# MilchRatchet/Luminary

Hardware: AMD Instinct MI355X
Metric: Mrays/s at 1920x1080, 8 bounces (higher is better)
Workload: dtype f32

## Files before the change

### include/lum_core.h

```cpp
#ifndef LUM_CORE_H
#define LUM_CORE_H

#include <stdint.h>

#ifdef __cplusplus
extern "C" {
#endif

typedef struct LumContext LumContext;

typedef struct LumDeviceSceneView {
  uint32_t num_meshes;
  uint32_t num_instances;
  uint32_t num_materials;
  uint32_t num_lights;
  const uint32_t* mesh_tri_offset;
  const float* vertices;
  const uint32_t* tri_tex;
  const uint32_t* instance_mesh_ids;
  const float* instance_transforms;
  const uint16_t* materials;
  const uint8_t* light_tree_root;
  const uint8_t* light_tree_nodes;
  const uint32_t* light_tri_handles;
// ... 146 lines not shown
typedef struct LumDenoiseParams {
  uint32_t iterations;
  float sigma_luminance;
  float sigma_normal;
  float sigma_depth;
  uint32_t uniform_samples;
} LumDenoiseParams;
void lumc_denoise_default_params(LumDenoiseParams* params);
int lumc_render_guides(LumContext* ctx, uint32_t num_samples, void* stream);
int lumc_download_guides(LumContext* ctx, float* albedo, float* normal, float* depth);
int lumc_has_guides(const LumContext* ctx);
int lumc_denoise(LumContext* ctx, const LumDenoiseParams* params, float* d_image, void* stream);
int lumc_denoise_host(LumContext* ctx, const LumDenoiseParams* params, float* image);
int lumc_set_denoise_form(LumContext* ctx, int lds);
int lumc_download_result_image(LumContext* ctx, float* result);
const float* lumc_result_image(LumContext* ctx);

int lumc_trace_closest(LumContext* ctx, uint32_t num_rays, const float* d_origins, const float* d_dirs, const uint32_t* d_ignore, uint32_t* d_out, void* stream);
int lumc_pixel_query(LumContext* ctx, uint32_t x, uint32_t y, uint32_t sample_id, uint32_t out[6]);
int lumc_trace_closest_host(LumContext* ctx, uint32_t num_rays, const float* origins, const float* dirs, const uint32_t* ignore, uint32_t* out);

int lumc_trace_visibility(LumContext* ctx, uint32_t num_rays, const float* d_origins, const float* d_dirs, const float* d_dist, const uint32_t* d_ids, const uint32_t* d_order,
                          float* d_out, void* stream);
int lumc_trace_visibility_host(LumContext* ctx, uint32_t num_rays, const float* origins, const float* dirs, const float* dist, const uint32_t* ids, const uint32_t* order, float* out);
int lumc_light_query_host(LumContext* ctx, uint32_t num_rays, const float* origins, const float* dirs, const uint32_t* self, const float* randoms, uint32_t* out_ids,
                          uint32_t* out_num_hits);
#define LUMC_LIGHT_PROBE_VERTEX_WORDS 20
#define LUMC_LIGHT_PROBE_WORDS 154
enum { LUMC_LIGHT_PROBE_GENERAL = 0, LUMC_LIGHT_PROBE_PLAIN = 1, LUMC_LIGHT_PROBE_UNSTAGED = 2 };
enum { LUMC_LIGHT_PROBE_NO_PICK = 0, LUMC_LIGHT_PROBE_SELF = 1, LUMC_LIGHT_PROBE_REFUSED = 2, LUMC_LIGHT_PROBE_MISSED = 3, LUMC_LIGHT_PROBE_EVALUATED = 4 };
int lumc_light_sample_probe_host(LumContext* ctx, uint32_t num_vertices, const uint32_t* vertices, uint32_t first_sample, uint32_t samples, int form, uint32_t* out);

#define LUMC_LENS_MAX_INTERFACES 24
typedef struct LumLensInterface { float radius, vertex, cylindrical_radius; } LumLensInterface;
typedef struct LumLensMedium { float design_ior, abbe, cylindrical_radius; } LumLensMedium;
typedef struct LumPhysicalCamera {
  float aperture_point, aperture_radius, exit_pupil_point, exit_pupil_radius, image_plane_distance, sensor_width;
  uint32_t allow_reflections;
  uint32_t num_interfaces;
  LumLensInterface interfaces[LUMC_LENS_MAX_INTERFACES];
  LumLensMedium media[LUMC_LENS_MAX_INTERFACES + 1];
} LumPhysicalCamera;
int lumc_set_physical_camera(LumContext* ctx, const LumPhysicalCamera* camera);
int lumc_camera_rays(LumContext* ctx, const uint32_t* pixels, uint32_t n, uint32_t first_sample, uint32_t samples, float* out_origin, float* out_dir, float* out_weight);

int lumc_set_bvh_builder(LumContext* ctx, int builder);

unsigned int lumc_lds_stack_bytes(void);

#define LUMC_COMM_ID_BYTES 128
int lumc_device_count(void);
uint32_t lumc_tile_lattice_step(uint32_t world);
uint32_t lumc_tile_owner(uint32_t tile_x, uint32_t tile_y, uint32_t tiles_x, uint32_t world);
int lumc_tile_pixels(uint32_t width, uint32_t height, uint32_t rank, uint32_t world, uint32_t tile, uint32_t* out, uint32_t* count);
int lumc_comm_unique_id(uint8_t id[LUMC_COMM_ID_BYTES]);
int lumc_comm_init_rank(LumContext* ctx, int world, int rank, const uint8_t id[LUMC_COMM_ID_BYTES]);
int lumc_comm_init_all(LumContext** ctxs, int n);
void lumc_comm_destroy(LumContext* ctx);
int lumc_frame_assemble(LumContext* ctx, uint32_t frame_pixels, int root, void* stream, float** d_frame_out);
int lumc_frame_assemble_all(LumContext** ctxs, int n, uint32_t frame_pixels, int root, float** d_frame_root);
int lumc_frame_gather(LumContext* ctx, uint32_t width, uint32_t height, int root, void* stream, float** d_frame_out);
int lumc_frame_gather_all(LumContext** ctxs, int n, uint32_t width, uint32_t height, int root, float** d_frame_root);
int lumc_frame_download(LumContext* ctx, uint32_t frame_pixels, float* first_moment, float* second_moment);
uint32_t lumc_frame_plane_stride(const LumContext* ctx);
int lumc_use_assembled_frame(LumContext* ctx, int on);
int lumc_accumulators_from_frame(LumContext* dst, LumContext* src);
int lumc_comm_count(const LumContext* ctx);
int lumc_device_name(int ordinal, char* out, size_t size);

int lumc_set_ray_sorting(LumContext* ctx, int mode);
int lumc_get_ray_sorting(const LumContext* ctx);

enum { LUMC_FLAVOUR_EXACT = 0, LUMC_FLAVOUR_FAST = 1 };
int lumc_set_flavour(LumContext* ctx, int flavour);
int lumc_get_flavour(const LumContext* ctx);
int lumc_set_ambient_reuse(LumContext* ctx, int mode);
int lumc_get_ambient_reuse(const LumContext* ctx);
int lumc_set_single_level(LumContext* ctx, int mode);
int lumc_get_single_level(const LumContext* ctx);
int lumc_set_plain_form(LumContext* ctx, int mode);
int lumc_get_plain_form(const LumContext* ctx);
int lumc_set_overlap_light_query(LumContext* ctx, int mode);
int lumc_get_overlap_light_query(const LumContext* ctx);
int lumc_overlap_registers_fit(uint32_t ray_kernel_regs, uint32_t light_query_regs);
int lumc_set_fused_resolve(LumContext* ctx, int on);
int lumc_set_sobol_table(LumContext* ctx, int on);
double lumc_bvh_build_seconds(const LumContext* ctx);
int lumc_bvh_meshes_by_builder(const LumContext* ctx, uint32_t out[2]);
int lumc_bvh_stats(LumContext* ctx, uint64_t out[4]);
uint32_t lumc_scene_view_sizeof(void);
int lumc_host_bvh_probe(const float* boxes, uint32_t count, uint32_t max_leaf, uint64_t out[6], double inner_area[3]);
uint32_t lumc_leaf_max_triangles(void);
typedef struct LumMeshRefitStats {
  uint64_t refits, rebuilds;
  uint32_t last_refits, last_rebuilds;
  double max_cost_growth;
  double seconds;
  double seconds_upload, seconds_refit, seconds_rebuild, seconds_assemble;
  double seconds_hash, seconds_download, seconds_lights;
} LumMeshRefitStats;
int lumc_set_mesh_refit(LumContext* ctx, uint32_t mode, float max_cost_growth);
int lumc_mesh_refit_stats(const LumContext* ctx, LumMeshRefitStats* out);
int lumc_bvh_refit_probe(const float* built_boxes, const float* refit_boxes, uint32_t count, uint32_t refit_count, int builder, int on_gpu, uint64_t sizes[3],
                         void* built_nodes, void* refit_nodes, void* host_refit_nodes, uint32_t* prims, double cost[3], uint64_t* valid);
int lumc_scene_tree_probe(const LumDeviceSceneView* scene, uint64_t sizes[4], void* nodes, void* tris, void* leaves, void* rows, uint32_t* mesh_root, float bounds[6]);
typedef struct LumInstanceUpdateStats {
  uint64_t device_updates, fallbacks, relayouts;
  uint32_t tlas_nodes, tlas_depth, tlas_capacity, hittable;
  double seconds;
  double seconds_relayout, seconds_upload, seconds_boxes, seconds_build, seconds_leaves;
} LumInstanceUpdateStats;
int lumc_set_instance_update(LumContext* ctx, uint32_t mode);
int lumc_instance_update_stats(const LumContext* ctx, LumInstanceUpdateStats* out);
int lumc_instance_boxes_probe(const LumDeviceSceneView* scene, const float* mesh_boxes, int on_gpu, void* rows, float* boxes, uint32_t* hittable);
int lumc_resident_tree_probe(LumContext* ctx, uint64_t sizes[5], void* top_nodes, void* leaves, uint32_t* mesh_root, uint64_t* mesh_hash);
int lumc_set_mesh_refit_in_place(LumContext* ctx, uint32_t on);
typedef struct LumResidentRefitStats {
  uint64_t updates, fallbacks;
  uint32_t last_meshes, last_launches;
  uint64_t last_bytes_downloaded;
  double seconds;
  double seconds_upload, seconds_hash, seconds_refit, seconds_cost, seconds_top_level;
} LumResidentRefitStats;
int lumc_resident_refit_stats(const LumContext* ctx, LumResidentRefitStats* out);
int lumc_resident_mesh_nodes_probe(LumContext* ctx, void* nodes);
typedef struct LumMeshSkinStats {
  uint64_t poses, rebuild_downloads;
  uint32_t last_meshes, last_launches;
  uint64_t last_bytes_uploaded;
  double seconds, seconds_upload, seconds_skin;
} LumMeshSkinStats;
int lumc_mesh_skin_bind(LumContext* ctx, uint32_t mesh, const float* rest_positions, const float* rest_normals, const uint16_t* bone_ids, const float* weights,
                        uint32_t triangle_count, uint32_t bone_count);
int lumc_mesh_skin_unbind(LumContext* ctx, uint32_t mesh);
int lumc_mesh_skin_pose(LumContext* ctx, uint32_t mesh, const float* bones, uint32_t bone_count);
int lumc_mesh_skin_stats(const LumContext* ctx, LumMeshSkinStats* out);
int lumc_mesh_vertices_probe(LumContext* ctx, uint32_t mesh, void* out);
int lumc_skin_host(const float* rest_positions, const float* rest_normals, const uint16_t* bone_ids, const float* weights, uint32_t triangle_count, const float* bones,
                   uint32_t bone_count, float* positions, float* normals, uint32_t* packed);
typedef struct LumMeshMorphStats {
  uint64_t applied, rebuild_downloads;
  uint32_t last_meshes, last_launches;
  uint64_t last_bytes_uploaded;
  double seconds, seconds_upload, seconds_morph;
} LumMeshMorphStats;
int lumc_mesh_morph_bind(LumContext* ctx, uint32_t mesh, const float* base_positions, const float* base_normals, uint32_t triangle_count, uint32_t target_count,
                         const uint32_t* offsets, const uint32_t* corners, const float* delta_positions, const float* delta_normals);
int lumc_mesh_morph_unbind(LumContext* ctx, uint32_t mesh);
int lumc_mesh_morph_weights(LumContext* ctx, uint32_t mesh, const float* weights, uint32_t target_count);
int lumc_mesh_morph_stats(const LumContext* ctx, LumMeshMorphStats* out);
int lumc_morph_host(const float* base_positions, const float* base_normals, uint32_t triangle_count, uint32_t target_count, const uint32_t* offsets, const uint32_t* corners,
                    const float* delta_positions, const float* delta_normals, const float* weights, const uint16_t* bone_ids, const float* skin_weights, const float* bones,
                    uint32_t bone_count, float* positions, float* normals, uint32_t* packed);
typedef struct LumShutterStats {
  uint64_t slices;
  uint32_t last_meshes, last_launches;
  uint64_t last_bytes_uploaded;
  double seconds;
} LumShutterStats;
int lumc_mesh_shutter_key(LumContext* ctx, uint32_t mesh, uint32_t which);
int lumc_mesh_shutter_drop(LumContext* ctx, uint32_t mesh);
int lumc_shutter_time(LumContext* ctx, float t);
int lumc_shutter_stats(const LumContext* ctx, LumShutterStats* out);
int lumc_shutter_host(const void* open_records, const void* close_records, uint32_t count, float t, void* out_records, uint32_t* flags);
int lumc_host_bvh_nodes_probe(const float* boxes, uint32_t count, uint32_t max_leaf, uint32_t max_depth, uint64_t sizes[3], void* nodes, uint32_t* prims);
typedef struct LumLightFragment { uint32_t instance, mesh, triangle, light_id, transform; float intensity, average_intensity; uint32_t reserved; } LumLightFragment;
// ... 39 lines not shown
```

### luminary_amd/core.py

```python
import ctypes as C

import numpy as np

from . import DeviceSceneView, _lib

DIRTY_CONSTANTS, DIRTY_MATERIALS, DIRTY_INSTANCES, DIRTY_LIGHTS, DIRTY_MESHES, DIRTY_TEXTURES, DIRTY_PARTICLES, DIRTY_ALL = 1, 2, 4, 8, 16, 32, 64, 127
DIRTY_MESH_POSITIONS = 128
DIRTY_INSTANCE_TRANSFORMS = 256
DIRTY_MESH_SKIN = 512
DIRTY_LIGHT_POSITIONS = 1024
DIRTY_MESH_SHUTTER = 2048
BVH_BUILDERS = {"sah": 0, "lbvh": 1, "ploc": 2, "sah_gpu": 3}
CNT_TRACE, CNT_SHADOW, CNT_LIGHT_BVH, CNT_VERTICES, CNT_NODES, CNT_TRIS, CNT_NODES_SHADOW, CNT_TRIS_SHADOW, CNT_NODES_LIGHT, CNT_TRIS_LIGHT, CNT_NODES_LDS, CNT_NODES_LDS_SHADOW, CNT_AMBIENT_DEFERRED, CNT_AMBIENT_FALLBACK = range(14)
CNT_COUNT = 16
KERNELS = ("generate", "trace", "shade", "shadow", "accumulate", "light_query", "resolve", "output", "sky", "sort", "volume")


class CoreError(RuntimeError):
    pass


class OutputParams(C.Structure):
    _fields_ = [("src_width", C.c_uint32), ("src_height", C.c_uint32), ("dst_width", C.c_uint32), ("dst_height", C.c_uint32),
                ("inv_sample_count", C.c_float), ("exposure", C.c_float), ("tonemap", C.c_uint32), ("filter", C.c_uint32), ("dithering", C.c_uint32),
# ... 323 lines not shown
        lib = _lib()
        n = C.c_uint32()
        if lib.lumc_tile_pixels(C.c_uint32(width), C.c_uint32(height), C.c_uint32(rank), C.c_uint32(world), C.c_uint32(tile), C.c_void_p(0), C.byref(n)):
            raise CoreError("lumc_tile_pixels: bad arguments")
        out = np.zeros(max(n.value, 1), dtype=np.uint32)
        lib.lumc_tile_pixels(C.c_uint32(width), C.c_uint32(height), C.c_uint32(rank), C.c_uint32(world), C.c_uint32(tile), out.ctypes.data_as(C.c_void_p), C.byref(n))
        return out[:n.value]

    @staticmethod
    def comm_unique_id():
        buf = (C.c_uint8 * 128)()
        if _lib().lumc_comm_unique_id(buf):
            raise CoreError("lumc_comm_unique_id failed")
        return bytes(buf)

    def comm_init_rank(self, world, rank, unique_id):
        buf = (C.c_uint8 * 128).from_buffer_copy(unique_id)
        self._call("lumc_comm_init_rank", C.c_int(world), C.c_int(rank), buf)

    def frame_assemble(self, frame_pixels, root=0, stream=0):
        ptr = C.c_void_p()
        self._call("lumc_frame_assemble", C.c_uint32(frame_pixels), C.c_int(root), C.c_void_p(stream), C.byref(ptr))
        return ptr.value

    def frame_gather(self, width, height, root=0, stream=0):
        ptr = C.c_void_p()
        self._call("lumc_frame_gather", C.c_uint32(width), C.c_uint32(height), C.c_int(root), C.c_void_p(stream), C.byref(ptr))
        return ptr.value

    def frame_download(self, frame_pixels):
        fm = np.zeros(3 * frame_pixels, dtype=np.float32)
        sm = np.zeros(frame_pixels, dtype=np.float32)
        self._call("lumc_frame_download", C.c_uint32(frame_pixels), fm.ctypes.data_as(C.c_void_p), sm.ctypes.data_as(C.c_void_p))
        return fm.reshape(3, -1), sm

    @property
    def ray_sorting(self):
        fn = self._lib.lumc_get_ray_sorting
        fn.restype = C.c_int
        return int(fn(self._ctx))

    def set_ray_sorting(self, mode):
        self._call("lumc_set_ray_sorting", C.c_int(mode))

    def set_fused_resolve(self, on):
        self._call("lumc_set_fused_resolve", C.c_int(int(on)))

    def set_sobol_table(self, on):
        self._call("lumc_set_sobol_table", C.c_int(1 if on else 0))

    def set_ambient_reuse(self, mode):
        self._call("lumc_set_ambient_reuse", C.c_int(mode))

    @property
    def ambient_reuse(self):
        fn = self._lib.lumc_get_ambient_reuse
        fn.restype = C.c_int
        return bool(fn(self._ctx))

    def set_single_level(self, mode):
        self._call("lumc_set_single_level", C.c_int(mode))

    def get_single_level(self):
        fn = self._lib.lumc_get_single_level
        fn.restype = C.c_int
        return int(fn(self._ctx))

    def set_plain_form(self, mode):
        self._call("lumc_set_plain_form", C.c_int(mode))

    def get_plain_form(self):
        fn = self._lib.lumc_get_plain_form
        fn.restype = C.c_int
        return int(fn(self._ctx))

    def set_overlap_light_query(self, mode):
        self._call("lumc_set_overlap_light_query", C.c_int(mode))

    def get_overlap_light_query(self):
        fn = self._lib.lumc_get_overlap_light_query
        fn.restype = C.c_int
        return int(fn(self._ctx))

    @staticmethod
    def overlap_registers_fit(ray_kernel_regs, light_query_regs):
        fn = _lib().lumc_overlap_registers_fit
        fn.restype = C.c_int
        return bool(fn(C.c_uint32(ray_kernel_regs), C.c_uint32(light_query_regs)))

    def set_physical_camera(self, camera):
        self._call("lumc_set_physical_camera", C.byref(camera) if camera is not None else C.c_void_p(0))

    def camera_rays(self, pixels, first_sample, samples):
        px = np.ascontiguousarray(pixels, dtype=np.uint32)
        n = px.size * samples
        o = np.zeros((n, 3), dtype=np.float32)
        d = np.zeros((n, 3), dtype=np.float32)
        w = np.zeros(n, dtype=np.float32)
        self._call("lumc_camera_rays", px.ctypes.data_as(C.c_void_p), C.c_uint32(px.size), C.c_uint32(first_sample), C.c_uint32(samples),
                   o.ctypes.data_as(C.c_void_p), d.ctypes.data_as(C.c_void_p), w.ctypes.data_as(C.c_void_p))
        return o, d, w

    def pixel_query(self, x, y, sample_id=0):
        out = (C.c_uint32 * 6)()
        self._call("lumc_pixel_query", C.c_uint32(x), C.c_uint32(y), C.c_uint32(sample_id), out)
        a = np.array(list(out), dtype=np.uint32)
        return int(a[0]), int(a[1]), float(a[2:3].view(np.float32)[0]), a[3:6].view(np.float32).copy()

    def set_flavour(self, name):
        self._call("lumc_set_flavour", C.c_int({"exact": 0, "fast": 1}[name]))

    def _call(self, name, *args):
        fn = getattr(self._lib, name)
        fn.restype = C.c_int
        if fn(self._ctx, *args) != 0:
            raise CoreError("%s failed: %s" % (name, self._lib.lumc_last_error(self._ctx).decode()))

    def close(self):
        if self._ctx:
            self._lib.lumc_context_destroy(self._ctx)
            self._ctx = C.c_void_p()

    def __del__(self):
        try:
            self.close()
        except Exception:
            pass

    def upload(self, view):
        self._view_keepalive = view
        self._call("lumc_scene_upload", C.byref(view))
        self.width, self.height = view.width, view.height

    def update(self, view, dirty):
        self._view_keepalive = view
        self._call("lumc_scene_update", C.byref(view), C.c_uint(dirty))
        self.width, self.height = view.width, view.height

    def generate_output(self, params, first_moment=None, want_float=False):
        out = np.zeros((params.dst_height, params.dst_width), dtype=np.uint32)
        planes = np.zeros(params.output_planes_shape(), dtype=np.float32) if want_float else None
        pl = planes.ctypes.data_as(C.c_void_p) if want_float else C.c_void_p(0)
        if isinstance(first_moment, np.ndarray):
            fm = np.ascontiguousarray(first_moment, dtype=np.float32)
            self._call("lumc_generate_output_from_host", C.byref(params), fm.ctypes.data_as(C.c_void_p), out.ctypes.data_as(C.c_void_p), pl)
        else:
            ptr = C.c_void_p(0) if first_moment is None else C.c_void_p(int(first_moment))
            self._call("lumc_generate_output_host", C.byref(params), ptr, out.ctypes.data_as(C.c_void_p), pl)
        return (out, planes) if want_float else out

    def download_luts(self):
        out = {"conductor": np.zeros(1024, np.uint16), "glossy": np.zeros(1024, np.uint16), "dielectric": np.zeros(32768, np.uint16),
               "dielectric_inv": np.zeros(32768, np.uint16)}
        self._call("lumc_download_luts", *[out[k].ctypes.data_as(C.c_void_p) for k in ("conductor", "glossy", "dielectric", "dielectric_inv")])
        return out

    def download_sky_luts(self):
        tm = np.zeros(2 * 64 * 256 * 4, dtype=np.float32)
        ms = np.zeros(2 * 32 * 32 * 4, dtype=np.float32)
        self._call("lumc_download_sky_luts", tm.ctypes.data_as(C.c_void_p), ms.ctypes.data_as(C.c_void_p))
        return tm, ms

    def cloud_noise_generate(self, seed):
        shape, detail, weather = np.zeros(128 ** 3, np.uint32), np.zeros(32 ** 3, np.uint32), np.zeros(1024 ** 2, np.uint32)
        self._call("lumc_cloud_noise_generate", C.c_uint32(seed), shape.ctypes.data_as(C.c_void_p), detail.ctypes.data_as(C.c_void_p),
                   weather.ctypes.data_as(C.c_void_p))
# ... 378 lines not shown
```

### luminary_amd/csrc/device/dev_scene.h

```cpp
#pragma once

#include <hip/hip_vector_types.h>
#include <stdint.h>

namespace lum {

struct alignas(128) Bvh4Node {
  float lo_x[4], lo_y[4], lo_z[4];
  float hi_x[4], hi_y[4], hi_z[4];
  uint32_t child[4];
  uint32_t pad[4];
};
static_assert(sizeof(Bvh4Node) == 128, "BVH4 node must be one cache line");

constexpr uint32_t kNodeBytes = 128u, kNodeShift = 7u;

constexpr uint32_t kBvhEmpty      = 0xFFFFFFFFu;
constexpr uint32_t kBvhLeafBit    = 0x80000000u;
#ifndef LUM_LEAF_MAX
#define LUM_LEAF_MAX 2
#endif
constexpr uint32_t kBvhLeafMaxTri = LUM_LEAF_MAX;
static_assert(LUM_LEAF_MAX >= 1 && LUM_LEAF_MAX <= 8, "a leaf's triangle count travels in 3 bits");

// ... 77 lines not shown
  uint32_t ocean_caustics_active, ocean_caustics_ris_sample_count;
  float ocean_caustics_domain_scale;
  uint32_t ocean_multiscattering, ocean_triangle_light_contribution;
  uint32_t cloud_active, cloud_atmosphere_scattering, cloud_steps, cloud_shadow_steps, cloud_octaves;
  float cloud_offset_x, cloud_offset_z, cloud_density, cloud_noise_shape_scale, cloud_noise_detail_scale, cloud_noise_weather_scale;
  float cloud_phase[4];
  float cloud_layers[3][10];
  const uint32_t* cloud_noise_shape;
  const uint32_t* cloud_noise_detail;
  const uint32_t* cloud_noise_weather;
  uint32_t particles_active, particles_count;
  float particles_scale, particles_speed;
  float particles_albedo[3], particles_direction[3], particles_phase[4];
  const float4* particle_normals;
  const Bvh4Node* particle_bvh_nodes;
  const BvhTri* particle_tris;
  const float4* particle_leaves;
  uint32_t particle_tlas_num_nodes, particle_num_leaves;
  const uint2* sobol_table;
  uint32_t sobol_first, sobol_count, sobol_stride;
  uint32_t traits;
};

struct PathQueue {
  float4* origin_t;
  float4* dir_slot;
  uint4* aux;
  uint4* hit_id;
  uint32_t* hit_scene_tri;
  uint32_t* parent;
};
constexpr uint32_t kParentDeferred = 0x80000000u, kParentMask = 0x7FFFFFFFu;

struct NeeQueue {
  float4* geo_color_light;
  float4* bsdf_ray_prob;
  float4* bsdf_weight_sum;
  uint4* ambient;
  uint4* sun;
  uint32_t* amb_path;
  float4* sun_water;
  float4* amb_t1;
  float4* amb_t2;
};

struct ShadowQueue {
  float4* origin_dist;
  float4* dir_out;
  uint4* ids;
  float4* vis;
  uint32_t* light_items;
  uint32_t capacity;
};

struct FusedResolve {
  PathQueue prev;
  NeeQueue nee_prev;
  ShadowQueue fallback;
  uint32_t* ended;
  const uint32_t* ended_prev;
};

constexpr uint32_t kVolumeShadowKinds = 19, kVolumeKindSun = 15, kVolumeKindAmbient = 16, kVolumeKindSun2 = 17, kVolumeKindAmbient2 = 18;
constexpr uint32_t kShadowKindAmbient2 = 4, kShadowKindSun2 = 5, kSurfaceShadowKindsWater = 6;
struct CloudQueue {
  uint32_t* items;
  float4* result;
  float* hit_dist;
  uint32_t capacity;
};
struct VolumeQueue {
  float4* bridge;
  uint4* sky;
  float4* weight;
  float4* sun_water;
  float4* amb_t1;
  float4* amb_t2;
  uint32_t* items;
};

struct PassParams {
  const uint32_t* pixels;
  uint32_t num_pixels, batch, first_sample;
};

constexpr uint32_t kAdaptiveStages = 4;
struct AdaptiveView {
  const uint32_t* stage_counts;
  const uint32_t* block_task_end;
  uint32_t blocks_x, blocks_y, num_blocks;
  uint32_t executions[kAdaptiveStages + 1];
  uint32_t stage_id;
};
struct AdaptivePass { uint32_t task_begin, task_end, block_begin, block_end, executions; };
constexpr uint32_t kGuidePlanes = 7;
constexpr uint32_t kGuideSumPlanes = 9;
struct DenoiseArgs {
  uint32_t width, height, step, uniform_samples;
  float sigma_luminance, sigma_normal, sigma_depth;
};

constexpr uint32_t kLensMaxInterfaces = 24;
struct LensInterface { float radius, vertex, cylindrical_radius; };
struct LensMedium { float design_ior, abbe, cylindrical_radius; };
struct DeviceLens {
  float aperture_point, aperture_radius, exit_pupil_point, exit_pupil_radius, image_plane_distance, sensor_width;
  uint32_t num_interfaces, pad;
  LensInterface iface[kLensMaxInterfaces];
  LensMedium medium[kLensMaxInterfaces + 1];
};
enum CameraKind : int { kCamThinLens = 0, kCamPhysical = 1, kCamPhysicalReflections = 2 };

enum PathState : uint32_t {
  kStDeltaPath = 1, kStCameraDirection = 2, kStVolumeScattered = 4, kStAllowEmission = 8, kStAllowAmbient = 16, kStUseIgnoreHandle = 32
};
enum SkyMode : uint32_t { kSkyDefault = 0, kSkyHdri = 1, kSkyConstantColor = 2 };

#ifndef LUM_CTL_LINE
#define LUM_CTL_LINE 32u
#endif
enum CtrlWord : uint32_t {
  kCtlPaths = 0, kCtlShadowItems = LUM_CTL_LINE, kCtlLightItems = 2u * LUM_CTL_LINE, kCtlSkyItems = 2u * LUM_CTL_LINE + 1u, kCtlTraceCursor = 3u * LUM_CTL_LINE,
  kCtlShadowCursor = 3u * LUM_CTL_LINE + 8u, kCtlStride = 4u * LUM_CTL_LINE,
  kCtlVolumeShift = 16u, kCtlVolumeShadowItems = kCtlShadowItems + kCtlVolumeShift, kCtlVolumeShadowCursor = kCtlShadowCursor + kCtlVolumeShift,
  kCtlVolumeItems = 2u * LUM_CTL_LINE + 2u,
  kCtlParticleCursor = LUM_CTL_LINE + 8u,
  kCtlCloudItems = 2u * LUM_CTL_LINE + 3u, kCtlCloudCursor = LUM_CTL_LINE + 24u,
  kCtlShadeCursor = 3u * LUM_CTL_LINE + 16u
};
static_assert(LUM_CTL_LINE >= 32u, "the fog's control words sit in the second half of the 32-word lines");

#ifndef LUM_LDS_STACK_BYTES
#define LUM_LDS_STACK_BYTES 98304u
#endif
#ifndef LUM_RAY_BLOCK_MAX
#define LUM_RAY_BLOCK_MAX 1024u
#endif
constexpr uint32_t kRayBlockMax = LUM_RAY_BLOCK_MAX;

enum Counter : uint32_t { kCntTrace = 0, kCntShadow, kCntLightBvh, kCntVertices, kCntNodes, kCntTris, kCntNodesShadow, kCntTrisShadow, kCntNodesLight, kCntTrisLight, kCntNodesLds,
                         kCntNodesLdsShadow,
                         kCntAmbientDeferred,
                         kCntAmbientFallback,
                         kCntSpare0, kCntSpare1, kCntCount };

}
```

### luminary_amd/csrc/device/dev_trace.h

```cpp
#pragma once

#include "dev_light.h"

LUM_NS_BEGIN

#ifndef LUM_TRACE_BLOCK
#define LUM_TRACE_BLOCK 1024
#endif
constexpr int kTraceBlock = LUM_TRACE_BLOCK;

constexpr uint32_t kHitSky        = 0xFFFFFFFEu;
constexpr uint32_t kLeaveInstance = 0xFFFFFFFDu;
constexpr uint32_t kTraversalDone = 0xFFFFFFFCu;
constexpr uint32_t kNoInstance    = 0xFFFFFFFFu;
constexpr int kStackSize = 128;
#ifndef LUM_CHUNK_MAX
#define LUM_CHUNK_MAX 256u
#endif
#ifndef LUM_VOTE_TRIS
#define LUM_VOTE_TRIS 1u
#define LUM_VOTE_NODES 2u
#endif
#ifndef LUM_REFILL
#define LUM_REFILL 40
// ... 20 lines not shown
#endif

LUM_DEV float safe_inv(float d) { return (fabsf(d) < 1e-30f) ? copysignf(1e30f, d) : __builtin_amdgcn_rcpf(d); }

LUM_DEV float vmax3(float a, float b, float c) { float r; asm("v_max3_f32 %0, %1, %2, %3" : "=v"(r) : "v"(a), "v"(b), "v"(c)); return r; }
LUM_DEV float vmin3(float a, float b, float c) { float r; asm("v_min3_f32 %0, %1, %2, %3" : "=v"(r) : "v"(a), "v"(b), "v"(c)); return r; }
LUM_DEV float vmax0(float a) { float r; asm("v_max_f32 %0, 0, %1" : "=v"(r) : "v"(a)); return r; }
LUM_DEV float vmin2(float a, float b) { float r; asm("v_min_f32 %0, %1, %2" : "=v"(r) : "v"(a), "v"(b)); return r; }

struct TRay {
  V3 o, d, inv, noi;
  uint32_t nx, ny, nz, fx, fy, fz;
  LUM_DEV void set(V3 origin, V3 dir) {
    o = origin; d = dir;
    inv = v3(safe_inv(dir.x), safe_inv(dir.y), safe_inv(dir.z));
    noi = v3(-(origin.x * inv.x), -(origin.y * inv.y), -(origin.z * inv.z));
    nx = (inv.x < 0.0f) ? 48u : 0u;  fx = 48u - nx;
    ny = (inv.y < 0.0f) ? 64u : 16u; fy = 80u - ny;
    nz = (inv.z < 0.0f) ? 80u : 32u; fz = 112u - nz;
  }
};

LUM_DEV float4 node_f4(const Bvh4Node* nodes, uint32_t byte_offset) {
  return *reinterpret_cast<const float4*>(reinterpret_cast<const char*>(nodes) + byte_offset);
}
LUM_DEV uint4 node_u4(const Bvh4Node* nodes, uint32_t byte_offset) {
  return *reinterpret_cast<const uint4*>(reinterpret_cast<const char*>(nodes) + byte_offset);
}

template <int kFarFirst = 0>
LUM_DEV float child_entry(float nx, float ny, float nz, float fx, float fy, float fz, const TRay& r, float tmax) {
  const float ax = __builtin_fmaf(nx, r.inv.x, r.noi.x), ay = __builtin_fmaf(ny, r.inv.y, r.noi.y), az = __builtin_fmaf(nz, r.inv.z, r.noi.z);
  const float bx = __builtin_fmaf(fx, r.inv.x, r.noi.x), by = __builtin_fmaf(fy, r.inv.y, r.noi.y), bz = __builtin_fmaf(fz, r.inv.z, r.noi.z);
  const float tn = vmax3(ax, ay, vmax0(az));
  const float tf = vmin3(bx, by, vmin2(bz, tmax));
  const bool far_first = kFarFirst == 1 || (kFarFirst == 2 && tmax >= 3.0e38f) || (kFarFirst == 3 && tmax < 3.0e38f);
  return (tn <= __builtin_fmaf(tf, 1.000004f, 1e-30f)) ? (far_first ? -tn : tn) : __builtin_inff();
}

LUM_DEV void cswap(float& ka, uint32_t& ca, float& kb, uint32_t& cb) {
  const bool s = kb < ka;
  const float k0 = s ? kb : ka, k1 = s ? ka : kb;
  const uint32_t c0 = s ? cb : ca, c1 = s ? ca : cb;
  ka = k0; kb = k1; ca = c0; cb = c1;
}

LUM_DEV bool within(float tnear, float tmax) { return tnear <= __builtin_fmaf(tmax, 1.000004f, 1e-30f); }

struct NodeSource { const Bvh4Node* global; const char* lds; uint32_t lds_count; };

template <bool kCull> struct StackEntry;
template <> struct StackEntry<true> {
  using E = uint2;
  static LUM_DEV E make(uint32_t node, float tnear) { return make_uint2(node, fbits(tnear)); }
  static LUM_DEV uint32_t node(E e) { return e.x; }
  static LUM_DEV bool reachable(E e, float tmax) { return bitsf(e.y) <= __builtin_fmaf(tmax, 1.000004f, 1e-30f); }
};
template <> struct StackEntry<false> {
  using E = uint32_t;
  static LUM_DEV E make(uint32_t node, float) { return node; }
  static LUM_DEV uint32_t node(E e) { return e; }
  static LUM_DEV bool reachable(E, float) { return true; }
};

template <typename E> struct StackWord;
template <> struct StackWord<uint32_t> {
  typedef uint32_t W;
  static LUM_DEV W pack(uint32_t e) { return e; }
  static LUM_DEV uint32_t unpack(W w) { return w; }
};
template <> struct StackWord<uint2> {
  typedef unsigned long long W;
  static LUM_DEV W pack(uint2 e) { return (W) e.x | ((W) e.y << 32); }
  static LUM_DEV uint2 unpack(W w) { return make_uint2((uint32_t) w, (uint32_t) (w >> 32)); }
};
template <typename E> struct TraversalStack {
  typedef typename StackWord<E>::W W;
  typedef __attribute__((address_space(5))) W* ScratchPtr;
  typedef __attribute__((address_space(3))) W* LdsPtr;
  ScratchPtr scratch; LdsPtr lds; int lds_entries;
  LUM_DEV void store(int i, E e) { if (i < lds_entries) lds[(uint32_t) i * (uint32_t) kTraceBlock] = StackWord<E>::pack(e); else scratch[i] = StackWord<E>::pack(e); }
  LUM_DEV E load(int i) const { if (i < lds_entries) return StackWord<E>::unpack(lds[(uint32_t) i * (uint32_t) kTraceBlock]); return StackWord<E>::unpack(scratch[i]); }
};
template <bool kOrdered, bool kCull, int kFarFirst = 0, typename S>
LUM_DEV uint32_t visit_node(const NodeSource& src, uint32_t cur, const TRay& r, float tmax, S& stk, int& sp,
                            typename StackEntry<kCull>::E& top, RayStats& st) {
  static_assert(!(kFarFirst && kCull), "the negated keys are not distances: only for queries that do not cull by them");
  using SE = StackEntry<kCull>;
  const uint32_t b = cur << 7;
  float4 nx, ny, nz, fx, fy, fz;
  uint4 ch;
  if (cur < src.lds_count) {
    const char* p = src.lds + b;
    nx = *reinterpret_cast<const float4*>(p + r.nx); ny = *reinterpret_cast<const float4*>(p + r.ny); nz = *reinterpret_cast<const float4*>(p + r.nz);
    fx = *reinterpret_cast<const float4*>(p + r.fx); fy = *reinterpret_cast<const float4*>(p + r.fy); fz = *reinterpret_cast<const float4*>(p + r.fz);
    ch = *reinterpret_cast<const uint4*>(p + 96u);
    st.lds_nodes++;
  }
  else {
    const Bvh4Node* __restrict__ nodes = src.global;
    nx = node_f4(nodes, b + r.nx); ny = node_f4(nodes, b + r.ny); nz = node_f4(nodes, b + r.nz);
    fx = node_f4(nodes, b + r.fx); fy = node_f4(nodes, b + r.fy); fz = node_f4(nodes, b + r.fz);
    ch = node_u4(nodes, b + 96u);
  }
  float k0 = child_entry<kFarFirst>(nx.x, ny.x, nz.x, fx.x, fy.x, fz.x, r, tmax);
  float k1 = child_entry<kFarFirst>(nx.y, ny.y, nz.y, fx.y, fy.y, fz.y, r, tmax);
  float k2 = child_entry<kFarFirst>(nx.z, ny.z, nz.z, fx.z, fy.z, fz.z, r, tmax);
  float k3 = child_entry<kFarFirst>(nx.w, ny.w, nz.w, fx.w, fy.w, fz.w, r, tmax);
  uint32_t c0 = ch.x, c1 = ch.y, c2 = ch.z, c3 = ch.w;
  if (kOrdered) {
    cswap(k0, c0, k1, c1); cswap(k2, c2, k3, c3); cswap(k0, c0, k2, c2); cswap(k1, c1, k3, c3); cswap(k1, c1, k2, c2);
  }
  const float inf = __builtin_inff();
  if (k1 < inf) {
    if (k2 < inf) {
      if (k3 < inf) { stk.store(sp, top); sp++; top = SE::make(c3, k3); }
      stk.store(sp, top); sp++; top = SE::make(c2, k2);
    }
    stk.store(sp, top); sp++; top = SE::make(c1, k1);
  }
  return (k0 < inf) ? c0 : kBvhEmpty;
}

template <typename S>
LUM_DEV uint2 stack_pop(const S& stk, int& sp, uint2& top) {
  const uint2 e = top;
  if (sp > 0) { sp--; top = stk.load(sp); }
  else top = make_uint2(kTraversalDone, 0u);
  return e;
}
template <typename S, typename E>
LUM_DEV void stack_push(S& stk, int& sp, E& top, E e) { stk.store(sp, top); sp++; top = e; }

LUM_DEV float4 tri_f4(const BvhTri* tris, uint32_t index, uint32_t word) { return reinterpret_cast<const float4*>(tris + index)[word]; }

struct LeafTris {
  float4 a[kBvhLeafMaxTri], b[kBvhLeafMaxTri], c[kBvhLeafMaxTri];
  template <bool kAllSlots>
  LUM_DEV void load(const BvhTri* __restrict__ tris, uint32_t first, uint32_t count) {
#pragma unroll
    for (uint32_t j = 0; j < kBvhLeafMaxTri; j++) {
      if (kAllSlots) {
        const uint32_t t = first + min(j, count - 1u);
        a[j] = tri_f4(tris, t, 0); b[j] = tri_f4(tris, t, 1); c[j] = tri_f4(tris, t, 2);
      }
      else if (j < count) { a[j] = tri_f4(tris, first + j, 0); b[j] = tri_f4(tris, first + j, 1); c[j] = tri_f4(tris, first + j, 2); }
    }
  }
};

template <bool kSingleLevel> struct OneInstance {};
template <> struct OneInstance<true> { float4 r0, r1, r2; uint32_t inst, root; };
LUM_DEV uint32_t instance_of(const OneInstance<false>&, uint32_t entered) { return entered; }
LUM_DEV uint32_t instance_of(const OneInstance<true>& one, uint32_t) { return one.inst; }

template <class Q, bool kSingleLevel = false>
LUM_DEV void trace_items(const DeviceScene& sc, uint32_t n, uint32_t* __restrict__ cursor, Q& q, RayStats& st, uint32_t& rays, uint32_t lds_count) {
  if (n == 0u) return;
  using SE = StackEntry<Q::kCull>;
  using E = typename SE::E;
  E stack_in_scratch[kStackSize];
  int sp = 0;
  TRay r;
  V3 wo = v3(0.0f, 0.0f, 0.0f), wd = v3(0.0f, 0.0f, 1.0f);
  float tmax = 0.0f;
  uint32_t cur = kTraversalDone, inst = kNoInstance, idx = 0;
  r.set(wo, wd);
  bool more = true;
  const uint32_t lane = threadIdx.x & 63u;
  const unsigned long long below = (1ull << lane) - 1ull;
  extern __shared__ float4 lds_top[];
  {
    const float4* __restrict__ g = reinterpret_cast<const float4*>(sc.bvh_nodes);
    for (uint32_t i = threadIdx.x; i < lds_count * (kNodeBytes / 16u); i += blockDim.x) lds_top[i] = g[i];
    __syncthreads();
  }
  __shared__ float4 lds_leaves[kSingleLevel ? 1u : 4u * LUM_LDS_INSTANCES];
  const uint32_t staged_leaves = kSingleLevel ? 0u : min(sc.tlas_num_leaves, (uint32_t) LUM_LDS_INSTANCES);
  if constexpr (!kSingleLevel) {
    for (uint32_t i = threadIdx.x; i < 4u * staged_leaves; i += blockDim.x) lds_leaves[i] = sc.tlas_leaves[i];
    __syncthreads();
  }
  [[maybe_unused]] OneInstance<kSingleLevel> one;
  if constexpr (kSingleLevel) {
    const float4* __restrict__ leaf = sc.tlas_leaves;
    const float4 meta = leaf[3];
    one.r0 = leaf[0]; one.r1 = leaf[1]; one.r2 = leaf[2]; one.inst = fbits(meta.x); one.root = fbits(meta.y);
  }
  const NodeSource nodes{sc.bvh_nodes, reinterpret_cast<const char*>(lds_top), lds_count};
  typedef typename TraversalStack<E>::W StackW;
  static_assert(sizeof(StackW) == sizeof(E), "a stack entry is one machine word");
  TraversalStack<E> stk{(typename TraversalStack<E>::ScratchPtr) reinterpret_cast<StackW*>(stack_in_scratch),
                        (typename TraversalStack<E>::LdsPtr) (reinterpret_cast<StackW*>(reinterpret_cast<char*>(lds_top) + lds_count * kNodeBytes) + threadIdx.x),
                        (int) (LUM_LDS_STACK_BYTES / (kRayBlockMax * (uint32_t) sizeof(E)))};

  E top = SE::make(kTraversalDone, 0.0f);
#ifdef LUM_PHASE_STATS
  uint32_t phase_[8] = {0, 0, 0, 0, 0, 0, 0, 0};
  unsigned long long ptime_[12] = {0, 0, 0, 0, 0, 0, 0, 0, 0, 0, 0, 0};
  const unsigned long long t_kernel_ = __builtin_readcyclecounter();
#endif
  auto pop = [&]() {
    LUM_PHASE(6); LUM_PHASE_LANES(7);
    bool left_instance = false, again;
    E e;
    if constexpr (kSingleLevel) {
      do {
        e = top;
        const bool done = SE::node(e) == kTraversalDone;
        if (!done) { sp--; top = stk.load(sp); }
        again = !done && !SE::reachable(e, tmax);
      } while (again);
      cur = SE::node(e);
      (void) left_instance;
      return;
    }
    do {
      e = top;
      const bool done = SE::node(e) == kTraversalDone, leave = SE::node(e) == kLeaveInstance;
      if (!done) { sp--; top = stk.load(sp); }
      left_instance |= leave;
      again = !done && (leave || !SE::reachable(e, tmax));
    } while (again);
    cur = SE::node(e);
    if (left_instance) { inst = kNoInstance; r.set(wo, wd); }
  };

  const uint32_t waves = gridDim.x * (blockDim.x / 64u);
  uint32_t chunk = n / (waves * 2u);
  chunk = (min(max(chunk, 64u), LUM_CHUNK_MAX) + 63u) & ~63u;
  uint32_t chunk_next = 0, chunk_end = 0;

  while (true) {
    const unsigned long long idle = __ballot(cur == kTraversalDone);
#ifdef LUM_PHASE_STATS
    const unsigned long long t_refill_ = __builtin_readcyclecounter();
    const bool refilling_ = idle != 0ull && more;
#endif
    if (idle != 0ull && more) {
      if (chunk_next >= chunk_end) {
        uint32_t base = 0;
        if (lane == 0) base = atomicAdd(cursor, chunk);
        base = __builtin_amdgcn_readfirstlane(base);
        chunk_next = base;
        chunk_end = min(base + chunk, n);
        more = base < n;
      }
      if (more) {
        const uint32_t avail = chunk_end - chunk_next, want = (uint32_t) __popcll(idle);
        const uint32_t rank = (uint32_t) __popcll(idle & below);
        if (cur == kTraversalDone && rank < avail) {
          idx = chunk_next + rank;
          if (q.load(sc, idx, wo, wd, tmax)) {
            rays++;
            const uint32_t e = 0x7F800000u;
            const bool finite = (fbits(wo.x) & e) != e && (fbits(wo.y) & e) != e && (fbits(wo.z) & e) != e && (fbits(wd.x) & e) != e && (fbits(wd.y) & e) != e &&
                                (fbits(wd.z) & e) != e;
            if constexpr (kSingleLevel) {
              if (finite) {
                const float4 r0 = one.r0, r1 = one.r1, r2 = one.r2;
                const float px = wo.x - r0.w, py = wo.y - r1.w, pz = wo.z - r2.w;
                const V3 oo = v3(mat_row_apply(r0.x, r0.y, r0.z, px, py, pz), mat_row_apply(r1.x, r1.y, r1.z, px, py, pz), mat_row_apply(r2.x, r2.y, r2.z, px, py, pz));
                const V3 od = v3(mat_row_apply(r0.x, r0.y, r0.z, wd.x, wd.y, wd.z), mat_row_apply(r1.x, r1.y, r1.z, wd.x, wd.y, wd.z),
                                 mat_row_apply(r2.x, r2.y, r2.z, wd.x, wd.y, wd.z));
                r.set(oo, od); cur = one.root; sp = 0; top = SE::make(kTraversalDone, 0.0f);
              }
              else q.finish(sc, idx);
            }
            else {
              if (finite) { r.set(wo, wd); cur = 0; sp = 0; top = SE::make(kTraversalDone, 0.0f); inst = kNoInstance; }
              else q.finish(sc, idx);
            }
          }
        }
        chunk_next += min(want, avail);
      }
    }
#ifdef LUM_PHASE_STATS
    if (refilling_) { ptime_[8] += __builtin_readcyclecounter() - t_refill_; ptime_[9]++; }
#endif
    if (__ballot(cur != kTraversalDone) == 0ull) break;
    LUM_PHASE(5);

    while (true) {
      const bool live = cur != kTraversalDone;
      const bool at_leaf = live && (cur & kBvhLeafBit);
      const bool want_tris = at_leaf && (kSingleLevel || inst != kNoInstance), want_enter = !kSingleLevel && at_leaf && inst == kNoInstance;
      const uint32_t n_live = (uint32_t) __popcll(__ballot(live)), n_tris = (uint32_t) __popcll(__ballot(want_tris)),
                     n_enter = kSingleLevel ? 0u : (uint32_t) __popcll(__ballot(want_enter));
      if (n_live == 0u) break;
      const uint32_t n_nodes = n_live - n_tris - n_enter;
      const bool run_tris = n_tris * LUM_VOTE_TRIS >= max(n_nodes, n_enter) * LUM_VOTE_NODES;
      const bool run_enter = !kSingleLevel && !run_tris && n_enter >= n_nodes;
      const bool do_tris = run_tris && want_tris, do_enter = run_enter && want_enter, do_node = !run_tris && !run_enter && live && !at_leaf;
      LUM_TIME_BEGIN();
#ifdef LUM_PHASE_STATS
      const bool memory_node_ = __ballot(do_node && cur >= lds_count) != 0ull;
#endif
      {
        if (do_tris) {
          LUM_PHASE(3); LUM_PHASE_LANES(4);
          if (q.on_tris(sc, instance_of(one, inst), cur & 0x0FFFFFFFu, ((cur >> 28) & 0x7u) + 1u, r.o, r.d, tmax, st)) cur = kTraversalDone;
          else pop();
          if (cur == kTraversalDone) q.finish(sc, idx);
        }
      }
      if constexpr (!kSingleLevel) {
        if (do_enter) {
          LUM_PHASE(1); LUM_PHASE_LANES(2);
          const uint32_t leaf_index = cur & 0x0FFFFFFFu;
          float4 r0, r1, r2, meta;
          if (leaf_index < staged_leaves) { const float4* leaf = lds_leaves + 4u * leaf_index; r0 = leaf[0]; r1 = leaf[1]; r2 = leaf[2]; meta = leaf[3]; }
          else { const float4* __restrict__ leaf = sc.tlas_leaves + 4u * leaf_index; r0 = leaf[0]; r1 = leaf[1]; r2 = leaf[2]; meta = leaf[3]; }
          inst = fbits(meta.x);
          const float px = wo.x - r0.w, py = wo.y - r1.w, pz = wo.z - r2.w;
          const V3 oo = v3(mat_row_apply(r0.x, r0.y, r0.z, px, py, pz), mat_row_apply(r1.x, r1.y, r1.z, px, py, pz), mat_row_apply(r2.x, r2.y, r2.z, px, py, pz));
          const V3 od = v3(mat_row_apply(r0.x, r0.y, r0.z, wd.x, wd.y, wd.z), mat_row_apply(r1.x, r1.y, r1.z, wd.x, wd.y, wd.z),
                           mat_row_apply(r2.x, r2.y, r2.z, wd.x, wd.y, wd.z));
          r.set(oo, od);
          stack_push(stk, sp, top, SE::make(kLeaveInstance, 0.0f));
          cur = fbits(meta.y);
        }
      }
      {
        if (do_node) {
          LUM_PHASE(0);
          st.nodes++;
          cur = visit_node<Q::kOrdered, Q::kCull, Q::kFarFirst>(nodes, cur, r, tmax, stk, sp, top, st);
          if (cur == kBvhEmpty) {
            pop();
            if (cur == kTraversalDone) q.finish(sc, idx);
          }
        }
      }
#ifdef LUM_PHASE_STATS
      {
        asm volatile("s_waitcnt vmcnt(0) lgkmcnt(0)" ::: "memory");
        const int kind = run_tris ? 4 : (run_enter ? 6 : (memory_node_ ? 0 : 2));
        LUM_TIME_END(kind);
      }
#endif
      if (more && n_live < LUM_REFILL) break;
    }
  }
#ifdef LUM_PHASE_STATS
  ptime_[10] = __builtin_readcyclecounter() - t_kernel_; ptime_[11] = 1;
  for (int k = 0; k < 8; k++) if (phase_[k]) atomicAdd(&g_phase[k], (unsigned long long) phase_[k]);
  if ((threadIdx.x & 63u) == 0u) for (int k = 0; k < 12; k++) if (ptime_[k]) atomicAdd(&g_phase_time[k], ptime_[k]);
#endif
}

struct Hit { uint32_t instance_id, tri_id; float t; uint32_t scene_tri; };

struct ClosestState {
  static constexpr bool kOrdered = true;
  static constexpr int kFarFirst = 0;
  static constexpr bool kCull = true;
  static constexpr uint32_t kOpaqueBit = 0x80000000u;
  bool use_ignore, cutout;
  uint32_t ign_inst, ign_tri;
  Hit best;
  LUM_DEV void begin(bool ignore, uint32_t inst, uint32_t tri) { use_ignore = ignore; cutout = false; ign_inst = inst; ign_tri = tri; best = Hit{kHitSky, 0u, kFltMax, 0u}; }
  LUM_DEV bool on_tris(const DeviceScene& sc, uint32_t inst, uint32_t first, uint32_t count, V3 o, V3 d, float& tmax, RayStats& st) {
    LeafTris lt;
    lt.load<false>(sc.blas_tris, first, count);
#pragma unroll
    for (uint32_t j = 0; j < kBvhLeafMaxTri; j++) {
      if (j >= count) break;
      const float4 a = lt.a[j], b = lt.b[j], c = lt.c[j];
      const uint32_t id = fbits(a.w);
      st.tris++;
      if (use_ignore && inst == ign_inst && id == ign_tri) continue;
      F2 uv;
      const float t = intersect_triangle(v3(a.x, a.y, a.z), v3(b.x, b.y, b.z), v3(c.x, c.y, c.z), o, d, uv);
      if (t < best.t || (t == best.t && t != kFltMax && (inst < best.instance_id || (inst == best.instance_id && id < best.tri_id)))) {
        if (fbits(c.w) < sc.num_textures &&
            texture_load(sc, fbits(c.w), triangle_uv(sc.tri_tex[fbits(b.w)], uv), true, make_float4(0.0f, 0.0f, 0.0f, 1.0f)).w == 0.0f) {
          cutout = true;
          continue;
        }
        best.instance_id = inst; best.tri_id = id; best.t = t; best.scene_tri = fbits(b.w) | (fbits(c.w) == kBvhTriOpaque ? kOpaqueBit : 0u); tmax = t;
      }
    }
    return false;
  }
  LUM_DEV Hit result() const { return (best.t == kFltMax) ? Hit{kHitSky, 0u, kFltMax, 0u} : Hit{best.instance_id, best.tri_id, best.t, best.scene_tri & ~kOpaqueBit}; }
};

struct ShadowState {
  static constexpr bool kOrdered = true;
#ifndef LUM_SHADOW_ORDER
#define LUM_SHADOW_ORDER 1
#endif
  static constexpr int kFarFirst = LUM_SHADOW_ORDER;
  static constexpr bool kCull = false;
  uint32_t tgt_inst, tgt_tri, self_inst, self_tri;
  float dist;
#if LUM_FAST
  using Acc = float;
#else
  using Acc = double;
#endif
  Acc tr, tg, tb;
  bool blocked;
  LUM_DEV void begin(uint4 ids, float d) { tgt_inst = ids.x; tgt_tri = ids.y; self_inst = ids.z; self_tri = ids.w; dist = (d > kFltMax) ? kFltMax : d; tr = tg = tb = (Acc) 1.0; blocked = false; }
  LUM_DEV bool on_tris(const DeviceScene& sc, uint32_t inst, uint32_t first, uint32_t count, V3 o, V3 d, float&, RayStats& st) {
    LeafTris lt;
    lt.load<true>(sc.blas_tris, first, count);
#pragma unroll
    for (uint32_t j = 0; j < kBvhLeafMaxTri; j++) {
      if (j >= count) break;
      const float4 a = lt.a[j], b = lt.b[j], c = lt.c[j];
      const uint32_t id = fbits(a.w);
      st.tris++;
      if ((inst == tgt_inst && id == tgt_tri) || (inst == self_inst && id == self_tri)) continue;
      F2 uv;
      const float t = intersect_triangle(v3(a.x, a.y, a.z), v3(b.x, b.y, b.z), v3(c.x, c.y, c.z), o, d, uv);
      if (!(t > kEps && t < dist)) continue;
      if (fbits(c.w) == kBvhTriOpaque) { blocked = true; return true; }
      const uint4 tt = sc.tri_tex[fbits(b.w)];
      const Material m = load_material(sc, tt.w & 0xFFFFu);
      Col albedo = m.albedo;
      float alpha = m.alpha;
      if (m.albedo_tex != kTextureNone) {
        const float4 af = (m.albedo_tex < sc.num_textures) ? texture_load(sc, m.albedo_tex, triangle_uv(tt, uv), true, make_float4(0.0f, 0.0f, 0.0f, 0.0f))
// ... 105 lines not shown
```

### luminary_amd/csrc/device/kernels.h

```cpp
#pragma once

#include "kernel_shadow.h"
#include "dev_sky.h"
#include "dev_volume.h"
#include "dev_particle.h"
#include "dev_water.h"
#include "dev_cloud_march.h"
#include "dev_adaptive.h"
#include "dev_camera.h"
#include "dev_wave.h"

LUM_NS_BEGIN

#ifndef LUM_SHADE_WAVES
#define LUM_SHADE_WAVES 3
#endif
#ifndef LUM_CLOUD_WAVES
#define LUM_CLOUD_WAVES 4
#endif
#ifndef LUM_FEATURE_WAVES
#define LUM_FEATURE_WAVES 3
#endif
#ifndef LUM_VOLUME_WAVES
#define LUM_VOLUME_WAVES 4
#endif
#ifndef LUM_SHADE_WAVES_CONSTANT_SKY
#define LUM_SHADE_WAVES_CONSTANT_SKY 3
#endif

LUM_DEV uint32_t initial_medium(const DeviceScene& sc, V3 origin) {
  return medium_ior_modify(0u, (sc.ocean_active && origin.y < sc.ocean_height) ? sc.ocean_refractive_index : 1.0f, true);
}
LUM_DEV uint32_t initial_volumes(const DeviceScene& sc, V3 origin, uint32_t sample_id) {
  uint32_t w = sample_id;
  if (sc.fog_active) w = volume_stack_modify(w, kVolumeFog, true);
  if (sc.ocean_active && ocean_is_underwater(sc, origin)) w = volume_stack_modify(w, kVolumeOcean, true);
  return w;
}

template <int kCam>
LUM_DEV void generate_path(const DeviceScene& sc, const DeviceLens& lens, const PathQueue& q, uint32_t* count, bool active, uint32_t x, uint32_t y,
                           uint32_t sample_id, uint32_t slot) {
  const uint32_t lane = threadIdx.x & 63u;
  const unsigned long long below = (1ull << lane) - 1ull;
  V3 o, d;
  float w = 1.0f;
  if (kCam != kCamThinLens && active) {
    const Sampler smp{sc.bluenoise_2d, x, y, sample_id, 0};
    w = camera_sample<kCam>(sc, lens, smp, o, d);
  }
  const bool valid = active && w > 0.0f;
  const unsigned long long ballot = __ballot(valid);
  if (ballot) {
    uint32_t base = 0;
    if (lane == (uint32_t) __builtin_ctzll(ballot)) base = atomicAdd(count, (uint32_t) __popcll(ballot));
    base = __shfl(base, __builtin_ctzll(ballot));
    if (valid) {
      const uint32_t i = base + (uint32_t) __popcll(ballot & below);
      if (kCam == kCamThinLens) {
        const Sampler smp{sc.bluenoise_2d, x, y, sample_id, 0};
        camera_ray(sc, smp, o, d);
      }
      const U2 rec = record_pack(splat(w));
      q.origin_t[i] = make_float4(o.x, o.y, o.z, kFltMax);
      q.dir_slot[i] = make_float4(d.x, d.y, d.z, bitsf(slot));
      q.aux[i]      = make_uint4(rec.x, rec.y, initial_medium(sc, o), kStDeltaPath | kStCameraDirection | kStAllowEmission | kStAllowAmbient);
      q.hit_id[i]   = make_uint4(0u, 0u, x | (y << 16), initial_volumes(sc, o, sample_id));
    }
  }
}

template <int kCam>
__global__ __launch_bounds__(kBlock) void k_generate(DeviceScene sc, PassParams pp, PathQueue q, float4* results, uint32_t* count, DeviceLens lens_arg) {
  const uint32_t total = pp.num_pixels * pp.batch;
  if constexpr (kCam == kCamThinLens) {
    for (uint32_t i = blockIdx.x * kBlock + threadIdx.x; i < total; i += gridDim.x * kBlock) {
      const uint32_t b = i / pp.num_pixels, p = i - b * pp.num_pixels;
      const uint32_t index = pp.pixels ? pp.pixels[p] : p;
      const uint32_t y = index / sc.width, x = index - y * sc.width;
      const Sampler smp{sc.bluenoise_2d, x, y, pp.first_sample + b, 0};
      V3 o, d;
      camera_ray(sc, smp, o, d);
      const U2 rec = record_pack(splat(1.0f));
      q.origin_t[i] = make_float4(o.x, o.y, o.z, kFltMax);
      q.dir_slot[i] = make_float4(d.x, d.y, d.z, bitsf(i));
      q.aux[i]      = make_uint4(rec.x, rec.y, initial_medium(sc, o), kStDeltaPath | kStCameraDirection | kStAllowEmission | kStAllowAmbient);
      q.hit_id[i]   = make_uint4(0u, 0u, x | (y << 16), initial_volumes(sc, o, pp.first_sample + b));
      results[i]    = make_float4(0.0f, 0.0f, 0.0f, 0.0f);
    }
    if (blockIdx.x == 0 && threadIdx.x == 0) *count = total;
  }
  else {
    __shared__ DeviceLens lds_lens;
    const DeviceLens& lens = stage_lens<kCam>(lens_arg, &lds_lens);
    const uint32_t rounds = (total + gridDim.x * kBlock - 1u) / (gridDim.x * kBlock);
    for (uint32_t round = 0; round < rounds; round++) {
      const uint32_t i = (round * gridDim.x + blockIdx.x) * kBlock + threadIdx.x;
      const bool active = i < total;
      uint32_t x = 0, y = 0, b = 0;
      if (active) {
        b = i / pp.num_pixels;
        const uint32_t p = i - b * pp.num_pixels;
        const uint32_t index = pp.pixels ? pp.pixels[p] : p;
        y = index / sc.width; x = index - y * sc.width;
        results[i] = make_float4(0.0f, 0.0f, 0.0f, 0.0f);
      }
      generate_path<kCam>(sc, lens, q, count, active, x, y, pp.first_sample + b, i);
    }
  }
}


template <int kCam>
__global__ __launch_bounds__(256) void k_generate_adaptive(DeviceScene sc, AdaptiveView a, AdaptivePass pass, PathQueue q, float4* results, uint32_t* count,
                                                          DeviceLens lens_arg) {
  __shared__ DeviceLens lds_lens;
  const DeviceLens& lens = stage_lens<kCam>(lens_arg, &lds_lens);
  const uint32_t pass_tasks = pass.task_end - pass.task_begin;
  const uint32_t rounds = (pass_tasks + gridDim.x * 256u - 1u) / (gridDim.x * 256u);
  for (uint32_t round = 0; round < rounds; round++) {
    const uint32_t slot = (round * gridDim.x + blockIdx.x) * 256u + threadIdx.x;
    const uint32_t t = pass.task_begin + slot;
    bool valid = false;
    uint32_t x = 0, y = 0, sample_id = 0;
    if (slot < pass_tasks) {
      uint32_t lo = pass.block_begin, hi = pass.block_end - 1u;
      while (lo < hi) {
        const uint32_t mid = (lo + hi) >> 1;
        if (t < a.block_task_end[mid] * pass.executions) hi = mid; else lo = mid + 1u;
      }
      const uint32_t block = lo;
      const uint32_t base = block ? a.block_task_end[block - 1u] * pass.executions : 0u;
      const uint32_t packed = a.stage_counts[block];
      const uint32_t per_pixel = adaptive_stage_count(packed, a.stage_id) * pass.executions;
      const uint32_t local = t - base;
      const uint32_t local_pixel = local / per_pixel, local_sample = local - local_pixel * per_pixel;
      const uint32_t by = block / a.blocks_x, bx = block - by * a.blocks_x;
      x = (bx << kAdaptiveBlockLog) + (local_pixel & 3u);
      y = (by << kAdaptiveBlockLog) + (local_pixel >> kAdaptiveBlockLog);
      sample_id = adaptive_pixel_samples(a, packed) + local_sample;
      valid = x < sc.width && y < sc.height && sample_id < kMaxGlobalSamples;
      results[slot] = make_float4(0.0f, 0.0f, 0.0f, 0.0f);
    }
    generate_path<kCam>(sc, lens, q, count, valid, x, y, sample_id, slot);
  }
}

template <int kCam>
__global__ __launch_bounds__(kBlock) void k_camera_rays(DeviceScene sc, DeviceLens lens_arg, const uint32_t* pixels, uint32_t n, uint32_t first_sample, uint32_t samples,
                                                        float* out_origin, float* out_dir, float* out_weight) {
  __shared__ DeviceLens lds_lens;
  const DeviceLens& lens = stage_lens<kCam>(lens_arg, &lds_lens);
  const uint32_t total = n * samples;
  for (uint32_t i = blockIdx.x * kBlock + threadIdx.x; i < total; i += gridDim.x * kBlock) {
    const uint32_t b = i / n, index = pixels[i - b * n];
    const uint32_t y = index / sc.width, x = index - y * sc.width;
    const Sampler smp{sc.bluenoise_2d, x, y, first_sample + b, 0};
    V3 o, d;
    const float w = camera_sample<kCam>(sc, lens, smp, o, d);
    out_origin[3 * i] = o.x; out_origin[3 * i + 1] = o.y; out_origin[3 * i + 2] = o.z;
    out_dir[3 * i] = d.x; out_dir[3 * i + 1] = d.y; out_dir[3 * i + 2] = d.z;
    out_weight[i] = w;
  }
}

constexpr uint32_t kNoAmbientPath = 0xFFFFFFFFu;
constexpr bool kReuseProves = !LUM_FAST;
constexpr uint32_t kHitTriOpaque = 0x80000000u, kHitTriCutout = 0x40000000u, kHitTriBeyondEps = 0x20000000u, kHitTriHit = 0x10000000u, kHitTriMask = 0x0FFFFFFFu;

struct TraceQuery : ClosestState {
  PathQueue q;
  const uint32_t* order;
  uint32_t item;
  LUM_DEV bool load(const DeviceScene&, uint32_t j, V3& o, V3& d, float& tmax) {
    const uint32_t i = order ? order[j] : j;
    item = i;
    const float4 o4 = ld_stream(&q.origin_t[i]), d4 = ld_stream(&q.dir_slot[i]);
    const uint32_t state = q.aux[i].w;
    const uint2 ign = *reinterpret_cast<const uint2*>(&q.hit_id[i]);
    begin((state & kStUseIgnoreHandle) != 0, ign.x, ign.y);
    o = v3(o4.x, o4.y, o4.z); d = v3(d4.x, d4.y, d4.z); tmax = kFltMax;
    return true;
  }
  LUM_DEV void finish(const DeviceScene&, uint32_t) {
    const uint32_t i = item;
    const Hit h = result();
    reinterpret_cast<float*>(&q.origin_t[i])[3] = h.t;
    *reinterpret_cast<uint2*>(&q.hit_id[i]) = make_uint2(h.instance_id, h.tri_id);
    static_assert(kOpaqueBit == kHitTriOpaque, "the opaque bit is stored where ClosestState keeps it");
    q.hit_scene_tri[i] = ((best.t == kFltMax) ? 0u : (best.scene_tri | kHitTriHit | (best.t > kEps ? kHitTriBeyondEps : 0u))) | (cutout ? kHitTriCutout : 0u);
  }
};

__global__ LUM_TRACE_BOUNDS void k_trace(DeviceScene sc, PathQueue q, const uint32_t* order, uint32_t* ctrl, uint64_t* counters, uint32_t lds_nodes) {
  RayStats st{0, 0, 0};
  uint32_t rays = 0;
  TraceQuery tq;
  tq.q = q;
  tq.order = order;
  tq.item = 0;
  trace_items(sc, ctrl[kCtlPaths], ctrl + kCtlTraceCursor, tq, st, rays, lds_nodes);
  flush_stats(counters, st, rays, kCntTrace, kCntNodes, kCntTris, kCntNodesLds);
}
template <bool kSingleLevel>
__global__ LUM_TRACE_BOUNDS void k_trace(DeviceScene sc, PathQueue q, const uint32_t* order, uint32_t* ctrl, uint64_t* counters, uint32_t lds_nodes) {
  static_assert(kSingleLevel, "the two-level form is the plain kernel of this name");
  RayStats st{0, 0, 0};
  uint32_t rays = 0;
  TraceQuery tq;
  tq.q = q;
  tq.order = order;
  tq.item = 0;
  trace_items<TraceQuery, true>(sc, ctrl[kCtlPaths], ctrl + kCtlTraceCursor, tq, st, rays, lds_nodes);
  flush_stats(counters, st, rays, kCntTrace, kCntNodes, kCntTris, kCntNodesLds);
}

template <bool kPlain = false>
LUM_DEV GeoContext build_context(const DeviceScene& sc, V3 hit_origin, V3 ray_world, uint32_t state, uint32_t inst, uint32_t tri, uint32_t tbase, uint32_t medium) {
  const Transform tf = load_transform(sc, inst);
  const float4 a = sc.vertices[3 * tbase], b = sc.vertices[3 * tbase + 1], c = sc.vertices[3 * tbase + 2];
  const uint4 tt = sc.tri_tex[tbase];
  V3 position = xf_point_inv(tf, hit_origin);
  const V3 ray = xf_rot_inv(tf, ray_world);
  const V3 p0 = v3(a.x, a.y, a.z);
  const V3 e1 = v3(b.x, b.y, b.z) - p0, e2 = v3(c.x, c.y, c.z) - p0;
  V3 face = normalize(cross(e1, e2));
  const F2 co = barycentric_in_triangle(p0, e1, e2, position);
  position = p0 + (e1 * co.x + e2 * co.y);
  position = xf_point(tf, position);
  const Material mat = load_material(sc, tt.w & 0xFFFFu);
  const F2 tex_coords = triangle_uv(tt, co);
  const V3 n0 = normal_unpack(fbits(a.w)), n1 = normal_unpack(fbits(b.w)), n2 = normal_unpack(fbits(c.w));
  const bool inside = dot(face, ray) > 0.0f;
  if (inside) face = face * -1.0f;
  V3 normal = lerp_normals(n0, n1 - n0, n2 - n0, co, face);
  if (mat.normal_tex != kTextureNone) {
    const bool valid = mat.normal_tex < sc.num_textures;
    const float4 nf = texture_load(sc, mat.normal_tex, tex_coords, false, make_float4(0.0f, 0.0f, 1.0f, 0.0f));
    V3 mn = v3(nf.x, nf.y, nf.z);
    if ((mat.flags & kDMatNormalMapCompressed) && valid) mn = mn * 2.0f - v3(1.0f, 1.0f, 1.0f);
    mn = normalize(mn);
    normal = qapply(qinv(rotation_to_z(normal)), mn);
  }
  normal = adapt_normal(ray * -1.0f, normal, face);
  Col albedo = mat.albedo;
  float alpha = mat.alpha;
  if (mat.albedo_tex != kTextureNone) {
    const float4 af = texture_load(sc, mat.albedo_tex, tex_coords, true, make_float4(0.9f, 0.9f, 0.9f, 1.0f));
    albedo = col(af.x, af.y, af.z);
    alpha = af.w;
  }
  const bool emissive_side = !inside || (mat.flags & kDMatBidirectionalEmission);
  const bool emits = (mat.flags & kDMatEmission) && emissive_side && ((state & kStAllowEmission) != 0);
  Col emission = emits ? mat.emission : col(0.0f, 0.0f, 0.0f);
  if (emits && mat.luminance_tex != kTextureNone) {
    const float4 lf = texture_load(sc, mat.luminance_tex, tex_coords, true, make_float4(0.0f, 0.0f, 0.0f, 0.0f));
    emission = col(lf.x, lf.y, lf.z) * (alpha * mat.emission_scale);
  }
  float roughness = mat.roughness;
  if (mat.roughness_tex != kTextureNone) roughness = texture_load(sc, mat.roughness_tex, tex_coords, true, make_float4(0.5f, 0.0f, 0.0f, 0.0f)).x;
  if (mat.flags & kDMatRoughnessAsSmoothness) roughness = 1.0f - roughness;
  roughness = fmaxf(roughness, 2e-2f);
  if ((state & kStDeltaPath) == 0) roughness = fmaxf(roughness, mat.roughness_clamp);
  uint32_t flags = kPlain ? 0u : mat.flags & kDMatSubstrateMask;
  if (mat.metallic_tex == kTextureNone && (mat.flags & kDMatMetallic)) flags |= kMatMetallic;
  if (mat.flags & kDMatColoredTransparency) flags |= kMatColoredTransparency;
  if (inside) flags |= kMatRefractionInside;
  const float other_ior = medium_ior_peek(medium, inside);
  const float ior_in = inside ? mat.refraction_index : other_ior;
  const float ior_out = inside ? other_ior : mat.refraction_index;
  if (((flags & kMatSubstrateMask) == kMatTranslucent) && (fabsf(1.0f - ior_in / ior_out) < 1e-4f)) {
    if ((flags & kMatColoredTransparency) == 0) albedo = col(lerpf(1.0f, albedo.r, alpha), lerpf(1.0f, albedo.g, alpha), lerpf(1.0f, albedo.b, alpha));
    alpha = 0.0f;
    flags |= kMatColoredTransparency;
  }
  GeoContext g;
  g.instance_id = inst; g.tri_id = tri;
  g.normal = xf_rot(tf, normal);
  g.face_normal_packed = normal_pack(face);
  g.position = position;
  g.V = ray_world * -1.0f;
  g.state = state;
  g.params.flags = flags;
  g.params.set(albedo, alpha, roughness, emission, ior_in / ior_out);
  return g;
}

LUM_DEV void add_to_result(float4* results, uint32_t slot, Col v) {
  if (!any_positive(v)) return;
  float4 r = results[slot];
  r.x += v.r; r.y += v.g; r.z += v.b;
  results[slot] = r;
}

struct ResolveRecords { uint4 aux; uint32_t slot; float4 cl, lc; uint4 amb; };
LUM_DEV ResolveRecords load_resolve_records(const PathQueue& in, const NeeQueue& nee, uint32_t i) {
// ... 1040 lines not shown
}

__global__ __launch_bounds__(kBlock) void k_volume_bounce(DeviceScene sc, PathQueue in, PathQueue out, VolumeQueue vq, uint32_t* ctrl, uint32_t depth_const) {
  const uint32_t n = ctrl[kCtlVolumeItems];
  uint32_t* count_out = ctrl + kCtlStride + kCtlPaths;
  const uint32_t lane = threadIdx.x & 63;
  const unsigned long long below = (1ull << lane) - 1ull;
  const uint32_t rounds = (n + gridDim.x * kBlock - 1) / (gridDim.x * kBlock);
  constexpr uint32_t kReserveRounds = 8;
  uint32_t reserved_base = 0;
  for (uint32_t round = 0; round < rounds; round++) {
    const uint32_t k = (round * gridDim.x + blockIdx.x) * kBlock + threadIdx.x;
    const bool valid = k < n;
    if (round % kReserveRounds == 0) {
      uint32_t count = 0;
      const uint32_t first = (round * gridDim.x + blockIdx.x) * kBlock + (threadIdx.x & ~63u);
      for (uint32_t r = 0; r < kReserveRounds && round + r < rounds; r++) {
        const uint32_t lo = first + r * gridDim.x * kBlock;
        count += (lo < n) ? min(64u, n - lo) : 0u;
      }
      uint32_t base = 0;
      if (lane == 0 && count) base = atomicAdd(count_out, count);
      reserved_base = __builtin_amdgcn_readfirstlane(base);
    }
    float4 n_o, n_d; uint4 n_aux, n_hid;
    if (valid) {
      const uint32_t i = vq.items[k];
      const float4 o4 = in.origin_t[i], d4 = in.dir_slot[i];
      const uint4 aux = in.aux[i], hid = in.hit_id[i];
      const Sampler smp{sc.bluenoise_2d, hid.z & 0xFFFFu, hid.z >> 16, path_sample_id(hid.w), depth_const};
      const V3 ray = v3(d4.x, d4.y, d4.z);
      const V3 origin = v3(o4.x, o4.y, o4.z) + ray * o4.w;
      const VolContext ctx = volume_context(sc, volume_stack_peek(hid.w, false), origin, ray, aux.w, 0.0f);
      const V3 bounce = volume_bsdf_sample(sc, ctx, smp, kRndVolGiResampling, kRndVolGiDiffuse);
      uint32_t state = aux.w & ~(kStDeltaPath | kStCameraDirection | kStAllowEmission | kStUseIgnoreHandle);
      if (sc.sky_mode != kSkyDefault) state &= ~kStAllowAmbient; else state |= kStAllowAmbient;
      state |= kStVolumeScattered;
      n_o = make_float4(origin.x, origin.y, origin.z, kFltMax);
      n_d = make_float4(bounce.x, bounce.y, bounce.z, d4.w);
      n_aux = make_uint4(aux.x, aux.y, aux.z, state);
      n_hid = make_uint4(0u, 0u, hid.z, hid.w);
    }
    const unsigned long long b = __ballot(valid);
    if (valid) {
      const uint32_t j = reserved_base + (uint32_t) __popcll(b & below);
      out.origin_t[j] = n_o; out.dir_slot[j] = n_d; out.aux[j] = n_aux; out.hit_id[j] = n_hid;
    }
    reserved_base += (uint32_t) __popcll(b);
  }
}

struct RaysQuery : ClosestState {
  const float* origins; const float* dirs; const uint32_t* ignore; uint32_t* out;
  LUM_DEV bool load(const DeviceScene&, uint32_t i, V3& o, V3& d, float& tmax) {
    const bool ign = ignore != nullptr && ignore[2 * i] != 0xFFFFFFFFu;
    begin(ign, ign ? ignore[2 * i] : 0u, ign ? ignore[2 * i + 1] : 0u);
    o = v3(origins[3 * i], origins[3 * i + 1], origins[3 * i + 2]); d = v3(dirs[3 * i], dirs[3 * i + 1], dirs[3 * i + 2]); tmax = kFltMax;
    return true;
  }
  LUM_DEV void finish(const DeviceScene&, uint32_t i) {
    const Hit h = result();
    out[3 * i] = h.instance_id; out[3 * i + 1] = h.tri_id; out[3 * i + 2] = fbits(h.t);
  }
};

__global__ LUM_TRACE_BOUNDS void k_trace_rays(DeviceScene sc, uint32_t n, const float* origins, const float* dirs, const uint32_t* ignore,
                                                           uint32_t* out, uint32_t* cursor, uint64_t* counters, uint32_t lds_nodes) {
  RayStats st{0, 0, 0};
  uint32_t rays = 0;
  RaysQuery q;
  q.origins = origins; q.dirs = dirs; q.ignore = ignore; q.out = out;
  trace_items(sc, n, cursor, q, st, rays, lds_nodes);
  flush_stats(counters, st, rays, kCntTrace, kCntNodes, kCntTris, kCntNodesLds);
}
template <bool kSingleLevel>
__global__ LUM_TRACE_BOUNDS void k_trace_rays(DeviceScene sc, uint32_t n, const float* origins, const float* dirs, const uint32_t* ignore,
                                                           uint32_t* out, uint32_t* cursor, uint64_t* counters, uint32_t lds_nodes) {
  static_assert(kSingleLevel, "the two-level form is the plain kernel of this name");
  RayStats st{0, 0, 0};
  uint32_t rays = 0;
  RaysQuery q;
  q.origins = origins; q.dirs = dirs; q.ignore = ignore; q.out = out;
  trace_items<RaysQuery, true>(sc, n, cursor, q, st, rays, lds_nodes);
  flush_stats(counters, st, rays, kCntTrace, kCntNodes, kCntTris, kCntNodesLds);
}

__global__ __launch_bounds__(kBlock) void k_light_query_probe(DeviceScene sc, uint32_t n, const float* origins, const float* dirs, const uint32_t* self, const float* randoms,
                                                              uint32_t* out_ids, uint32_t* out_num_hits) {
  const uint32_t i = blockIdx.x * kBlock + threadIdx.x;
  if (i >= n) return;
  RayStats st{0, 0, 0};
  uint32_t num_hits = 0;
  const uint32_t id = light_query(sc, v3(origins[3 * i], origins[3 * i + 1], origins[3 * i + 2]), v3(dirs[3 * i], dirs[3 * i + 1], dirs[3 * i + 2]), self[2 * i], self[2 * i + 1],
                                  randoms[i], num_hits, st);
  out_ids[i] = id; out_num_hits[i] = num_hits;
}

constexpr uint32_t kLightProbeVertexWords = 20, kLightProbeLaneWords = 17, kLightProbeHeadWords = 18;
constexpr uint32_t kLightProbeWords = kLightProbeHeadWords + kLightTreeOutputs * kLightProbeLaneWords;
enum LightProbeStatus : uint32_t { kLightProbeNoPick = 0, kLightProbeSelf = 1, kLightProbeRefused = 2, kLightProbeMissed = 3, kLightProbeEvaluated = 4 };
template <bool kPlain>
__global__ __launch_bounds__(kBlock) void k_light_sample_probe(DeviceScene sc, uint32_t n, uint32_t samples, uint32_t first_sample, uint32_t stage, const uint32_t* vertices,
                                                               uint32_t* out) {
  StagedLights staged_lights{nullptr, nullptr, 0u};
#if LUM_LDS_LIGHTS
  {
    __shared__ LdsF4 lds_light_table[4u * LUM_LDS_LIGHTS];
    __shared__ unsigned long long lds_light_handles[LUM_LDS_LIGHTS];
    const uint32_t staged = (kPlain || stage) ? min(sc.num_lights, (uint32_t) LUM_LDS_LIGHTS) : 0u;
    for (uint32_t k = threadIdx.x; k < 4u * staged; k += kBlock) { const float4 v = sc.light_tri_table[k]; const LdsF4 t = {v.x, v.y, v.z, v.w}; lds_light_table[k] = t; }
    for (uint32_t k = threadIdx.x; k < staged; k += kBlock) { const uint2 h = sc.light_tri_handles[k]; lds_light_handles[k] = (unsigned long long) h.x | ((unsigned long long) h.y << 32); }
    __syncthreads();
    staged_lights.table = (const __attribute__((address_space(3))) LdsF4*) lds_light_table;
    staged_lights.handles = (const __attribute__((address_space(3))) unsigned long long*) lds_light_handles;
    staged_lights.count = staged;
  }
#endif
  const uint32_t i = blockIdx.x * kBlock + threadIdx.x;
  if (i >= n) return;
  const uint32_t* vw = vertices + (size_t) (i / samples) * kLightProbeVertexWords;
  uint32_t* o = out + (size_t) i * kLightProbeWords;
  GeoContext g;
  g.instance_id = vw[16]; g.tri_id = vw[17];
  g.position = v3(bitsf(vw[0]), bitsf(vw[1]), bitsf(vw[2]));
  g.normal = normalize(v3(bitsf(vw[3]), bitsf(vw[4]), bitsf(vw[5])));
  g.V = normalize(v3(bitsf(vw[6]), bitsf(vw[7]), bitsf(vw[8])));
  g.face_normal_packed = normal_pack(g.normal);
  g.state = 0;
  g.params.flags = vw[15];
  g.params.set(col(bitsf(vw[9]), bitsf(vw[10]), bitsf(vw[11])), bitsf(vw[12]), bitsf(vw[13]), splat(0.0f), bitsf(vw[14]));
  const SamplerT<false> smp{sc.bluenoise_2d, vw[18], vw[19], first_sample + i % samples, 0u};
  ShadeClock clock;
  clock.start();
  const LightSample ls = sample_light<kPlain>(sc, g, smp, clock, staged_lights);
  o[0] = ls.light_id; o[1] = fbits(ls.ray.x); o[2] = fbits(ls.ray.y); o[3] = fbits(ls.ray.z);
  o[4] = fbits(ls.color.r); o[5] = fbits(ls.color.g); o[6] = fbits(ls.color.b); o[7] = fbits(ls.dist); o[8] = fbits(ls.root_sum);
  const TreeWork work = tree_prepass(sc, g, smp);
  const Energy energy = energy_terms(sc, g.params, world_ndotv(g));
#pragma unroll
  for (uint32_t l = 0; l < kLightTreeOutputs; l++) o[9 + l] = work.cont[l];
  o[17] = fbits(work.root_sum);
#if LUM_FAST
  const V3 view_local = normalize(qapply(rotation_to_z(g.normal), g.V));
#endif
#pragma nounroll
  for (uint32_t lane = 0; lane < kLightTreeOutputs; lane++) {
    uint32_t* w = o + kLightProbeHeadWords + lane * kLightProbeLaneWords;
    const TreePick pick = tree_postpass<kPlain>(sc, g, smp, lane, work);
    w[0] = pick.light_id; w[1] = fbits(pick.weight); w[2] = kLightProbeNoPick;
    if (pick.light_id == kLightIdInvalid) continue;
#if LUM_LDS_LIGHTS
    uint2 handle;
    const TableLight entry = load_tri_light_table<kPlain>(sc, staged_lights, pick.light_id, handle);
#else
    const uint2 handle = sc.light_tri_handles[pick.light_id];
    const TableLight entry = load_tri_light_table(sc, pick.light_id);
#endif
    const TriLight& tl = entry.tri;
    w[2] = kLightProbeSelf;
    if (handle.x == g.instance_id && handle.y == g.tri_id) continue;
    V3 ray; float sa;
    const F2 pair = smp.next2(kRndLightGeoRay + lane);
    w[2] = kLightProbeRefused;
    if (!sample_tri_solid_angle(g.position, tl, pair, ray, sa)) continue;
    w[3] = fbits(ray.x); w[4] = fbits(ray.y); w[5] = fbits(ray.z); w[6] = fbits(sa);
    F2 uv;
// ... 33 lines not shown
```

### luminary_amd/csrc/device/kernels_shared.h

```cpp
#pragma once

#include "dev_camera.h"
#include "dev_wave.h"
#include "dev_output.h"
#include "dev_adaptive.h"

LUM_NS_BEGIN

__global__ __launch_bounds__(256) void k_final_image(OutputParams p, const float* __restrict__ input, float* __restrict__ frame_output) {
  const uint32_t ui = p.undersampling_stage, uo = max(ui, p.supersampling);
  const uint32_t output_scale = 1u << (uo - ui);
  const uint32_t out_w = p.src_width >> uo, out_h = p.src_height >> uo, in_w = p.src_width >> ui, in_h = p.src_height >> ui;
  const uint32_t n = out_w * out_h, n_in = in_w * in_h;
  const float norm = 1.0f / (output_scale * output_scale);
  for (uint32_t i = blockIdx.x * 256 + threadIdx.x; i < n; i += gridDim.x * 256) {
    const uint32_t y = i / out_w, x = i - y * out_w;
    const uint32_t source_x = x * output_scale, source_y = y * output_scale;
    Col color = splat(0.0f);
    for (uint32_t yi = 0; yi < output_scale; yi++) {
      for (uint32_t xi = 0; xi < output_scale; xi++) {
        const uint32_t px_x = min(source_x + xi, in_w - 1), px_y = min(source_y + yi, in_h - 1);
        const uint32_t index = px_x + px_y * in_w;
        Col px = col(input[index] * p.inv_sample_count, input[n_in + index] * p.inv_sample_count, input[2 * n_in + index] * p.inv_sample_count);
        color = color + display_transform(p, px, px_x, px_y);
// ... 175 lines not shown
    if (x >= width || y >= height) continue;
    const uint32_t p = x + y * width;
    const uint32_t packed = a.stage_counts[block];
    const uint32_t per_pixel = adaptive_stage_count(packed, a.stage_id) * pass.executions;
    const uint32_t first_id = adaptive_pixel_samples(a, packed);
    const uint32_t block_begin = block ? a.block_task_end[block - 1u] : 0u;
    if (a.block_task_end[block] == block_begin) continue;
    const uint32_t base = block_begin * pass.executions - pass.task_begin + local * per_pixel;
    float r = first_moment[p], g = first_moment[num_pixels + p], b = first_moment[2 * num_pixels + p];
    float s = second_moment[p];
    for (uint32_t k = 0; k < per_pixel; k++) {
      if (first_id + k >= kMaxGlobalSamples) break;
      const float4 v = results[base + k];
      r += v.x; g += v.y; b += v.z;
      s += luminance(col(v.x * v.x, v.y * v.y, v.z * v.z));
    }
    first_moment[p] = r; first_moment[num_pixels + p] = g; first_moment[2 * num_pixels + p] = b;
    second_moment[p] = s;
  }
}

__global__ __launch_bounds__(256) void k_generate_result(AdaptiveView a, ResultParams rp, OutputParams op, const float* __restrict__ fm, const float* __restrict__ sm,
                                                        float* __restrict__ frame_result) {
  const uint32_t n = rp.width * rp.height;
  for (uint32_t index = blockIdx.x * 256u + threadIdx.x; index < n; index += gridDim.x * 256u) {
    const uint32_t y = index / rp.width, x = index - y * rp.width;
    const uint32_t samples = result_pixel_samples(a, rp, x, y);
    const float normalization = 1.0f / (float) samples;
    Col result;
    switch (rp.mode) {
      default:
      case 0: {
        if (rp.local_error_minimization) {
          Col center_mean;
          const float center_variance = adaptive_pixel_variance(fm, sm, n, index, normalization, center_mean);
          const float center_error = center_variance * normalization;
          const uint32_t xi_start = max(x, 1u) - 1u, xi_end = min(x, rp.width - 1u) + 1u;
          const uint32_t yi_start = max(y, 1u) - 1u, yi_end = min(y, rp.height - 1u) + 1u;
          Col neighbour_mean = splat(0.0f);
          float neighbour_error = 0.0f;
          for (uint32_t yi = yi_start; yi <= yi_end; yi++) {
            for (uint32_t xi = xi_start; xi <= xi_end; xi++) {
              if (xi == x && yi == y) continue;
              Col m = splat(0.0f);
              float variance = 0.0f, norm = 0.0f;
              const uint32_t ns = (xi < rp.width && yi < rp.height) ? result_pixel_samples(a, rp, xi, yi) : result_pixel_samples(a, rp, min(xi, rp.width - 1u), min(yi, rp.height - 1u));
              norm = 1.0f / (float) ns;
              if (xi < rp.width && yi < rp.height) variance = adaptive_pixel_variance(fm, sm, n, xi + yi * rp.width, norm, m);
              neighbour_mean = neighbour_mean + m;
              neighbour_error += variance * norm;
            }
          }
          const float neighbour_norm = 1.0f / (float) ((xi_end - xi_start + 1u) * (yi_end - yi_start + 1u) - 1u);
          neighbour_mean = neighbour_mean * neighbour_norm;
          neighbour_error *= neighbour_norm;
          const float t = remap01(center_error, 0.0f, 8.0f * neighbour_error);
          result = col(lerpf(center_mean.r, neighbour_mean.r, t), lerpf(center_mean.g, neighbour_mean.g, t), lerpf(center_mean.b, neighbour_mean.b, t));
        }
        else result = col(fm[index] * normalization, fm[n + index] * normalization, fm[2 * n + index] * normalization);
      } break;
      case 1: {
        Col mean;
        result = splat(128.0f * adaptive_pixel_variance(fm, sm, n, index, normalization, mean));
      } break;
      case 2: {
        Col mean;
        const float variance = adaptive_pixel_variance(fm, sm, n, index, normalization, mean);
        const float compression = adaptive_tonemap_compression(op, mean, rp.exposure);
        const float mse = sqrtf(variance * normalization) * compression;
        const float value = 1024.0f * mse;
        result = col(saturate(2.0f * value), saturate(2.0f * (value - 0.5f)),
                     saturate((value > 0.5f) ? 4.0f * (0.25f - fabsf(value - 1.0f)) : 4.0f * (0.25f - fabsf(value - 0.25f))));
      } break;
      case 3: {
        uint32_t per_pixel = 1;
        if (a.stage_counts && a.stage_id > 0) per_pixel = adaptive_stage_count(a.stage_counts[adaptive_block_of(a, x, y)], a.stage_id);
        result = splat((float) per_pixel / (float) kAdaptiveMaxRate);
      } break;
    }
    frame_result[index] = result.r; frame_result[n + index] = result.g; frame_result[2 * n + index] = result.b;
  }
}

__global__ __launch_bounds__(kBlock) void k_accumulate(const float4* results, uint32_t num_pixels, uint32_t batch, float* first_moment, float* second_moment) {
  for (uint32_t p = blockIdx.x * kBlock + threadIdx.x; p < num_pixels; p += gridDim.x * kBlock) {
    float r = first_moment[p], g = first_moment[num_pixels + p], b = first_moment[2 * num_pixels + p];
    float s = second_moment ? second_moment[p] : 0.0f;
    for (uint32_t k = 0; k < batch; k++) {
      const float4 v = results[k * num_pixels + p];
      r += v.x; g += v.y; b += v.z;
      s += luminance(col(v.x * v.x, v.y * v.y, v.z * v.z));
    }
    first_moment[p] = r; first_moment[num_pixels + p] = g; first_moment[2 * num_pixels + p] = b;
    if (second_moment) second_moment[p] = s;
  }
}

__global__ __launch_bounds__(kBlock) void k_accumulate_scatter(const float4* results, const uint32_t* pixels, uint32_t count, uint32_t frame_pixels, float* first_moment,
                                                               float* second_moment) {
  for (uint32_t p = blockIdx.x * kBlock + threadIdx.x; p < count; p += gridDim.x * kBlock) {
    const uint32_t index = pixels[p];
    const float4 v = results[p];
    first_moment[index] += v.x; first_moment[frame_pixels + index] += v.y; first_moment[2 * frame_pixels + index] += v.z;
    if (second_moment) second_moment[index] += luminance(col(v.x * v.x, v.y * v.y, v.z * v.z));
  }
}

__global__ __launch_bounds__(256) void k_visibility_pack(uint32_t n, const float* origins, const float* dirs, const float* dist, const uint32_t* ids, ShadowQueue sq) {
  const uint32_t i = blockIdx.x * 256u + threadIdx.x;
  if (i >= n) return;
  sq.origin_dist[i] = make_float4(origins[3 * i], origins[3 * i + 1], origins[3 * i + 2], dist[i]);
  sq.dir_out[i] = make_float4(dirs[3 * i], dirs[3 * i + 1], dirs[3 * i + 2], bitsf(i));
  sq.ids[i] = make_uint4(ids[4 * i], ids[4 * i + 1], ids[4 * i + 2], ids[4 * i + 3]);
}
__global__ __launch_bounds__(256) void k_visibility_unpack(uint32_t n, const float4* vis, float* out) {
  const uint32_t i = blockIdx.x * 256u + threadIdx.x;
  if (i >= n) return;
  const float4 v = vis[i];
  out[3 * i] = v.x; out[3 * i + 1] = v.y; out[3 * i + 2] = v.z;
}

__global__ void k_pixel_ray(DeviceScene sc, DeviceLens lens, int cam, uint32_t x, uint32_t y, uint32_t sample_id, float* origin, float* dir, uint32_t* valid) {
  if (blockIdx.x != 0 || threadIdx.x != 0) return;
  const Sampler smp{sc.bluenoise_2d, x, y, sample_id, 0};
  V3 o, d;
  float w = 1.0f;
  if (cam == kCamThinLens) camera_ray(sc, smp, o, d);
  else if (cam == kCamPhysical) w = camera_sample<kCamPhysical>(sc, lens, smp, o, d);
  else w = camera_sample<kCamPhysicalReflections>(sc, lens, smp, o, d);
  origin[0] = o.x; origin[1] = o.y; origin[2] = o.z;
  dir[0] = d.x; dir[1] = d.y; dir[2] = d.z;
  valid[0] = w > 0.0f ? 1u : 0u;
}

LUM_NS_END
```

### luminary_amd/csrc/device/wavefront_table.h

```cpp
#pragma once

#include <hip/hip_runtime.h>

#include "dev_scene.h"

namespace lum {

inline bool single_level_scene(const DeviceScene& sc) { return sc.tlas_num_nodes == 1u && sc.tlas_num_leaves == 2u; }

inline bool plain_scene(const DeviceScene& sc) {
  return (sc.traits & kTraitsPlain) == kTraitsPlain && sc.num_lights <= (uint32_t) LUM_LDS_LIGHTS && !sc.ocean_active &&
         (sc.sky_mode == kSkyConstantColor || sc.sky_mode == kSkyHdri);
}

struct WavefrontKernels {
  const char* flavour;
  uint32_t trace_block;
  int (*set_ray_kernel_lds)(size_t bytes);
  int (*init_sampler_seeds)();
  void (*sobol_table)(hipStream_t s, uint2* table, uint32_t first_sample, uint32_t count, uint32_t stride, uint32_t dims);
  void (*generate)(uint32_t grid, hipStream_t s, const DeviceScene& sc, const PassParams& pp, const PathQueue& q, float4* results, uint32_t* count, const DeviceLens& lens,
                   int cam);
  void (*generate_adaptive)(uint32_t grid, hipStream_t s, const DeviceScene& sc, const AdaptiveView& a, const AdaptivePass& pass, const PathQueue& q, float4* results,
                            uint32_t* count, const DeviceLens& lens, int cam);
  void (*trace)(uint32_t grid, size_t lds, hipStream_t s, const DeviceScene& sc, const PathQueue& q, const uint32_t* order, uint32_t* ctrl, uint64_t* counters,
                uint32_t lds_nodes, bool single_level);
  void (*sky_inscattering)(uint32_t grid, hipStream_t s, const DeviceScene& sc, const PathQueue& in, float4* results, const uint32_t* ctrl, uint32_t depth_const);
  void (*shade)(uint32_t grid, hipStream_t s, const DeviceScene& sc, const PathQueue& in, const PathQueue& out, const NeeQueue& nee, const ShadowQueue& sq, float4* results,
                uint32_t* ctrl, uint32_t depth_const, uint64_t* counters, uint32_t ambient_reuse, const FusedResolve* fused_dev, uint32_t fused_flags,
                bool plain_form);
  void (*shade_debug)(uint32_t grid, hipStream_t s, const DeviceScene& sc, const PathQueue& in, float4* results, const uint32_t* ctrl);
  void (*sky)(uint32_t grid, hipStream_t s, const DeviceScene& sc, const PathQueue& in, const ShadowQueue& sq, float4* results, const uint32_t* ctrl, uint32_t depth_const);
  void (*light_query)(uint32_t grid, hipStream_t s, const DeviceScene& sc, const PathQueue& in, const NeeQueue& nee, const ShadowQueue& sq, uint32_t* ctrl, uint32_t depth_const,
                      uint64_t* counters);
  void (*shadow_rays)(uint32_t grid, size_t lds, hipStream_t s, const DeviceScene& sc, const ShadowQueue& sq, const uint32_t* order, uint32_t* ctrl, uint64_t* counters,
                      uint32_t lds_nodes, bool single_level);
  void (*resolve)(uint32_t grid, hipStream_t s, const DeviceScene& sc, const PathQueue& in, const NeeQueue& nee, const ShadowQueue& sq, float4* results, const uint32_t* ctrl);
  void (*resolve_reuse)(uint32_t grid, hipStream_t s, const DeviceScene& sc, const PathQueue& in, const PathQueue& next, const NeeQueue& nee, const ShadowQueue& sq, float4* results,
                        uint32_t* ctrl, uint64_t* counters);
  void (*resolve_listed)(uint32_t grid, hipStream_t s, const DeviceScene& sc, const PathQueue& in, const NeeQueue& nee, const ShadowQueue& sq, float4* results, const uint32_t* ctrl);
  void (*resolve_ended)(uint32_t grid, hipStream_t s, const DeviceScene& sc, const PathQueue& in, const NeeQueue& nee, const ShadowQueue& sq, float4* results, const uint32_t* ctrl,
                        const uint32_t* list);
  bool fused_resolve;
  void (*volume_inscatter)(uint32_t grid, hipStream_t s, const DeviceScene& sc, const PathQueue& in, const VolumeQueue& vq, const ShadowQueue& sq, uint32_t* ctrl,
                           uint32_t depth_const);
  void (*volume_resolve)(uint32_t grid, hipStream_t s, const DeviceScene& sc, const PathQueue& in, const VolumeQueue& vq, const ShadowQueue& sq, float4* results,
                         const uint32_t* ctrl);
  void (*volume_events)(uint32_t grid, hipStream_t s, const DeviceScene& sc, const PathQueue& in, const VolumeQueue& vq, float4* results, uint32_t* ctrl, uint32_t depth_const);
  void (*volume_bounce)(uint32_t grid, hipStream_t s, const DeviceScene& sc, const PathQueue& in, const PathQueue& out, const VolumeQueue& vq, uint32_t* ctrl,
                        uint32_t depth_const);
  void (*trace_particles)(uint32_t grid, size_t lds, hipStream_t s, const DeviceScene& particle_tree, const PathQueue& q, uint32_t* ctrl, uint32_t lds_nodes);
  void (*particle_shade)(uint32_t grid, hipStream_t s, const DeviceScene& sc, const PathQueue& in, const PathQueue& out, const NeeQueue& nee, const ShadowQueue& sq,
                         uint32_t* ctrl, uint32_t depth_const);
  void (*trace_ocean)(uint32_t grid, hipStream_t s, const DeviceScene& sc, const PathQueue& q, const uint32_t* ctrl);
  void (*ocean_shade)(uint32_t grid, hipStream_t s, const DeviceScene& sc, const PathQueue& in, const PathQueue& out, const NeeQueue& nee, const ShadowQueue& sq, uint32_t* ctrl,
                      uint32_t depth_const);
  void (*clouds_list)(uint32_t grid, hipStream_t s, const DeviceScene& sc, const PathQueue& in, const CloudQueue& cq, uint32_t* ctrl);
  void (*clouds_march)(uint32_t grid, hipStream_t s, const DeviceScene& sc, const PathQueue& in, const CloudQueue& cq, uint32_t* ctrl, uint32_t depth_const);
  void (*clouds)(uint32_t grid, hipStream_t s, const DeviceScene& sc, const PathQueue& in, const CloudQueue& cq, float4* results, const uint32_t* ctrl, uint32_t depth_const);
  void (*trace_rays)(uint32_t grid, size_t lds, hipStream_t s, const DeviceScene& sc, uint32_t n, const float* origins, const float* dirs, const uint32_t* ignore, uint32_t* out,
                     uint32_t* cursor, uint64_t* counters, uint32_t lds_nodes, bool single_level);
  void (*camera_rays)(uint32_t grid, hipStream_t s, const DeviceScene& sc, const DeviceLens& lens, int cam, const uint32_t* pixels, uint32_t n, uint32_t first_sample,
                      uint32_t samples, float* origin, float* dir, float* weight);
  void (*guide)(uint32_t grid, hipStream_t s, const DeviceScene& sc, const PathQueue& in, const uint32_t* ctrl, float* planes, uint32_t n);
  void (*guide_normalise)(uint32_t grid, hipStream_t s, float* planes, uint32_t n, uint32_t samples);
  void (*denoise_prepare)(uint32_t grid, hipStream_t s, const AdaptiveView& a, const DenoiseArgs& p, const float* fm, const float* sm, const float* image, const float* guides,
                          float4* rec_a, uint4* rec_b);
  void (*denoise_atrous)(hipStream_t s, const DenoiseArgs& p, const float4* a_in, const uint4* rec_b, float4* a_out, bool lds);
  void (*denoise_finish)(uint32_t grid, hipStream_t s, const DenoiseArgs& p, const float4* rec_a, const float* guides, float* image);
  void (*light_query_probe)(hipStream_t s, const DeviceScene& sc, uint32_t n, const float* origins, const float* dirs, const uint32_t* self, const float* randoms, uint32_t* out_ids,
                            uint32_t* out_num_hits);
};
struct WavefrontProbes {
  void (*light_sample_probe)(hipStream_t s, const DeviceScene& sc, uint32_t n_vertices, uint32_t samples, uint32_t first_sample, uint32_t form, const uint32_t* vertices,
                             uint32_t* out);
};
constexpr uint32_t kLightSampleProbeVertexWords = 20, kLightSampleProbeWords = 154;

const WavefrontKernels* wavefront_kernels_exact();
const WavefrontKernels* wavefront_kernels_fast();
const WavefrontProbes* wavefront_probes_exact();
const WavefrontProbes* wavefront_probes_fast();
int ray_kernel_registers_exact(bool single_level, uint32_t* trace_regs, uint32_t* light_query_regs);
int ray_kernel_registers_fast(bool single_level, uint32_t* trace_regs, uint32_t* light_query_regs);

}
```

### luminary_amd/csrc/device/wavefront_table_impl.h

```cpp
#pragma once

#include "dev_adaptive.h"
#include "dev_denoise.h"
#include "wavefront_table.h"

LUM_NS_BEGIN
namespace table {

typedef void (*TraceKernel)(DeviceScene, PathQueue, const uint32_t*, uint32_t*, uint64_t*, uint32_t);
typedef void (*ShadowKernel)(DeviceScene, ShadowQueue, const uint32_t*, uint32_t*, uint64_t*, uint32_t);
typedef void (*TraceRaysKernel)(DeviceScene, uint32_t, const float*, const float*, const uint32_t*, uint32_t*, uint32_t*, uint64_t*, uint32_t);
static TraceKernel trace_kernel(bool single) { return single ? k_trace<true> : static_cast<TraceKernel>(k_trace); }
static ShadowKernel shadow_kernel(bool single) { return single ? k_shadow_rays<true> : static_cast<ShadowKernel>(k_shadow_rays); }
static TraceRaysKernel trace_rays_kernel(bool single) { return single ? k_trace_rays<true> : static_cast<TraceRaysKernel>(k_trace_rays); }

static int set_ray_kernel_lds(size_t bytes) {
  hipError_t e = hipSuccess;
  for (int single = 0; single < 2 && e == hipSuccess; single++) {
    e = hipFuncSetAttribute((const void*) trace_kernel(single != 0), hipFuncAttributeMaxDynamicSharedMemorySize, (int) bytes);
    if (e == hipSuccess) e = hipFuncSetAttribute((const void*) shadow_kernel(single != 0), hipFuncAttributeMaxDynamicSharedMemorySize, (int) bytes);
    if (e == hipSuccess) e = hipFuncSetAttribute((const void*) trace_rays_kernel(single != 0), hipFuncAttributeMaxDynamicSharedMemorySize, (int) bytes);
  }
  if (e == hipSuccess) e = hipFuncSetAttribute((const void*) k_trace_particles, hipFuncAttributeMaxDynamicSharedMemorySize, (int) bytes);
  return (int) e;
}
static int ray_kernel_registers(bool single_level, uint32_t* trace_regs, uint32_t* light_query_regs) {
  hipFuncAttributes a{};
  hipError_t e = hipFuncGetAttributes(&a, (const void*) trace_kernel(single_level));
  if (e != hipSuccess) return (int) e;
  *trace_regs = (uint32_t) a.numRegs;
  e = hipFuncGetAttributes(&a, (const void*) k_light_query);
  if (e == hipSuccess) *light_query_regs = (uint32_t) a.numRegs;
  return (int) e;
}
static int init_sampler_seeds() { return upload_sampler_seeds(); }
static void sobol_table(hipStream_t s, uint2* table, uint32_t first_sample, uint32_t count, uint32_t stride, uint32_t dims) {
  hipLaunchKernelGGL(k_sobol_table, dim3((dims * stride + 255u) / 256u), dim3(256), 0, s, table, first_sample, count, stride, dims);
}
static void generate(uint32_t grid, hipStream_t s, const DeviceScene& sc, const PassParams& pp, const PathQueue& q, float4* results, uint32_t* count, const DeviceLens& lens,
                     int cam) {
  auto* k = cam == kCamPhysical ? k_generate<kCamPhysical> : cam == kCamPhysicalReflections ? k_generate<kCamPhysicalReflections> : k_generate<kCamThinLens>;
  hipLaunchKernelGGL(k, dim3(grid), dim3(kBlock), 0, s, sc, pp, q, results, count, lens);
}
static void generate_adaptive(uint32_t grid, hipStream_t s, const DeviceScene& sc, const AdaptiveView& a, const AdaptivePass& pass, const PathQueue& q, float4* results,
                              uint32_t* count, const DeviceLens& lens, int cam) {
  auto* k = cam == kCamPhysical ? k_generate_adaptive<kCamPhysical> : cam == kCamPhysicalReflections ? k_generate_adaptive<kCamPhysicalReflections>
                                                                                                     : k_generate_adaptive<kCamThinLens>;
  hipLaunchKernelGGL(k, dim3(grid), dim3(kBlock), 0, s, sc, a, pass, q, results, count, lens);
}
static void camera_rays(uint32_t grid, hipStream_t s, const DeviceScene& sc, const DeviceLens& lens, int cam, const uint32_t* pixels, uint32_t n, uint32_t first_sample,
                        uint32_t samples, float* origin, float* dir, float* weight) {
  auto* k = cam == kCamPhysical ? k_camera_rays<kCamPhysical> : cam == kCamPhysicalReflections ? k_camera_rays<kCamPhysicalReflections> : k_camera_rays<kCamThinLens>;
  hipLaunchKernelGGL(k, dim3(grid), dim3(kBlock), 0, s, sc, lens, pixels, n, first_sample, samples, origin, dir, weight);
}
static void trace(uint32_t grid, size_t lds, hipStream_t s, const DeviceScene& sc, const PathQueue& q, const uint32_t* order, uint32_t* ctrl, uint64_t* counters,
                  uint32_t lds_nodes, bool single_level) {
  hipLaunchKernelGGL(trace_kernel(single_level && single_level_scene(sc)), dim3(grid), dim3(kTraceBlock), lds, s, sc, q, order, ctrl, counters, lds_nodes);
}
static void sky_inscattering(uint32_t grid, hipStream_t s, const DeviceScene& sc, const PathQueue& in, float4* results, const uint32_t* ctrl, uint32_t depth_const) {
  hipLaunchKernelGGL(k_sky_inscattering, dim3(grid), dim3(kBlock), 0, s, sc, in, results, ctrl, depth_const);
}
static void shade(uint32_t grid, hipStream_t s, const DeviceScene& sc, const PathQueue& in, const PathQueue& out, const NeeQueue& nee, const ShadowQueue& sq, float4* results,
                  uint32_t* ctrl, uint32_t depth_const, uint64_t* counters, uint32_t ambient_reuse, const FusedResolve* fused_dev, uint32_t fused_flags, bool plain_form) {
  auto* k = sc.sky_mode == kSkyDefault ? k_shade<kSkyDefault, false> : sc.sky_mode == kSkyHdri ? k_shade<kSkyHdri, false> : k_shade<kSkyConstantColor, false>;
  if (sc.ocean_active) k = sc.sky_mode == kSkyDefault ? k_shade<kSkyDefault, true> : sc.sky_mode == kSkyHdri ? k_shade<kSkyHdri, true> : k_shade<kSkyConstantColor, true>;
  if (sc.sobol_table) {
    k = sc.sky_mode == kSkyDefault ? k_shade<kSkyDefault, false, true> : sc.sky_mode == kSkyHdri ? k_shade<kSkyHdri, false, true> : k_shade<kSkyConstantColor, false, true>;
    if (sc.ocean_active) k = sc.sky_mode == kSkyDefault ? k_shade<kSkyDefault, true, true> : sc.sky_mode == kSkyHdri ? k_shade<kSkyHdri, true, true> : k_shade<kSkyConstantColor, true, true>;
  }
  if (plain_form && plain_scene(sc)) {
    if (sc.sobol_table) k = sc.sky_mode == kSkyHdri ? k_shade<kSkyHdri, false, true, true> : k_shade<kSkyConstantColor, false, true, true>;
    else k = sc.sky_mode == kSkyHdri ? k_shade<kSkyHdri, false, false, true> : k_shade<kSkyConstantColor, false, false, true>;
  }
  hipLaunchKernelGGL(k, dim3(grid), dim3(kBlock), 0, s, sc, in, out, nee, sq, results, ctrl, depth_const, counters, ambient_reuse, fused_dev, fused_flags);
}
static void shade_debug(uint32_t grid, hipStream_t s, const DeviceScene& sc, const PathQueue& in, float4* results, const uint32_t* ctrl) {
  hipLaunchKernelGGL(k_shade_debug, dim3(grid), dim3(kBlock), 0, s, sc, in, results, ctrl);
}
static void sky(uint32_t grid, hipStream_t s, const DeviceScene& sc, const PathQueue& in, const ShadowQueue& sq, float4* results, const uint32_t* ctrl, uint32_t depth_const) {
  hipLaunchKernelGGL(k_sky, dim3(grid), dim3(kBlock), 0, s, sc, in, sq, results, ctrl, depth_const);
}
static void light_query(uint32_t grid, hipStream_t s, const DeviceScene& sc, const PathQueue& in, const NeeQueue& nee, const ShadowQueue& sq, uint32_t* ctrl, uint32_t depth_const,
                        uint64_t* counters) {
  hipLaunchKernelGGL(k_light_query, dim3(grid), dim3(kBlock), 0, s, sc, in, nee, sq, ctrl, depth_const, counters);
}
static void shadow_rays(uint32_t grid, size_t lds, hipStream_t s, const DeviceScene& sc, const ShadowQueue& sq, const uint32_t* order, uint32_t* ctrl, uint64_t* counters,
                        uint32_t lds_nodes, bool single_level) {
  hipLaunchKernelGGL(shadow_kernel(single_level && single_level_scene(sc)), dim3(grid), dim3(kTraceBlock), lds, s, sc, sq, order, ctrl, counters, lds_nodes);
}
static void resolve(uint32_t grid, hipStream_t s, const DeviceScene& sc, const PathQueue& in, const NeeQueue& nee, const ShadowQueue& sq, float4* results, const uint32_t* ctrl) {
  hipLaunchKernelGGL(k_resolve, dim3(grid), dim3(kBlock), 0, s, sc, in, nee, sq, results, ctrl);
}
static void resolve_reuse(uint32_t grid, hipStream_t s, const DeviceScene& sc, const PathQueue& in, const PathQueue& next, const NeeQueue& nee, const ShadowQueue& sq, float4* results,
                          uint32_t* ctrl, uint64_t* counters) {
  hipLaunchKernelGGL(k_resolve_reuse, dim3(grid), dim3(kBlock), 0, s, sc, in, next, nee, sq, results, ctrl, counters);
}
static void resolve_listed(uint32_t grid, hipStream_t s, const DeviceScene& sc, const PathQueue& in, const NeeQueue& nee, const ShadowQueue& sq, float4* results, const uint32_t* ctrl) {
  hipLaunchKernelGGL(k_resolve_listed, dim3(grid), dim3(kBlock), 0, s, sc, in, nee, sq, results, ctrl);
}
static void resolve_ended(uint32_t grid, hipStream_t s, const DeviceScene& sc, const PathQueue& in, const NeeQueue& nee, const ShadowQueue& sq, float4* results, const uint32_t* ctrl,
                          const uint32_t* list) {
  hipLaunchKernelGGL(k_resolve_ended, dim3(grid), dim3(kBlock), 0, s, sc, in, nee, sq, results, ctrl, list);
}
static void volume_inscatter(uint32_t grid, hipStream_t s, const DeviceScene& sc, const PathQueue& in, const VolumeQueue& vq, const ShadowQueue& sq, uint32_t* ctrl,
                             uint32_t depth_const) {
  hipLaunchKernelGGL(k_volume_inscatter, dim3(grid), dim3(kBlock), 0, s, sc, in, vq, sq, ctrl, depth_const);
}
static void volume_resolve(uint32_t grid, hipStream_t s, const DeviceScene& sc, const PathQueue& in, const VolumeQueue& vq, const ShadowQueue& sq, float4* results,
                           const uint32_t* ctrl) {
  hipLaunchKernelGGL(k_volume_resolve, dim3(grid), dim3(kBlock), 0, s, sc, in, vq, sq, results, ctrl);
}
static void volume_events(uint32_t grid, hipStream_t s, const DeviceScene& sc, const PathQueue& in, const VolumeQueue& vq, float4* results, uint32_t* ctrl,
                          uint32_t depth_const) {
  hipLaunchKernelGGL(k_volume_events, dim3(grid), dim3(kBlock), 0, s, sc, in, vq, results, ctrl, depth_const);
}
static void volume_bounce(uint32_t grid, hipStream_t s, const DeviceScene& sc, const PathQueue& in, const PathQueue& out, const VolumeQueue& vq, uint32_t* ctrl,
                          uint32_t depth_const) {
  hipLaunchKernelGGL(k_volume_bounce, dim3(grid), dim3(kBlock), 0, s, sc, in, out, vq, ctrl, depth_const);
}
static void trace_particles(uint32_t grid, size_t lds, hipStream_t s, const DeviceScene& particle_tree, const PathQueue& q, uint32_t* ctrl, uint32_t lds_nodes) {
  hipLaunchKernelGGL(k_trace_particles, dim3(grid), dim3(kTraceBlock), lds, s, particle_tree, q, ctrl, lds_nodes);
}
static void particle_shade(uint32_t grid, hipStream_t s, const DeviceScene& sc, const PathQueue& in, const PathQueue& out, const NeeQueue& nee, const ShadowQueue& sq,
                           uint32_t* ctrl, uint32_t depth_const) {
  hipLaunchKernelGGL(k_particle_shade, dim3(grid), dim3(kBlock), 0, s, sc, in, out, nee, sq, ctrl, depth_const);
}
static void trace_ocean(uint32_t grid, hipStream_t s, const DeviceScene& sc, const PathQueue& q, const uint32_t* ctrl) {
  hipLaunchKernelGGL(k_trace_ocean, dim3(grid), dim3(kBlock), 0, s, sc, q, ctrl);
}
static void ocean_shade(uint32_t grid, hipStream_t s, const DeviceScene& sc, const PathQueue& in, const PathQueue& out, const NeeQueue& nee, const ShadowQueue& sq,
                        uint32_t* ctrl, uint32_t depth_const) {
  hipLaunchKernelGGL(k_ocean_shade, dim3(grid), dim3(kBlock), 0, s, sc, in, out, nee, sq, ctrl, depth_const);
}
static void clouds_list(uint32_t grid, hipStream_t s, const DeviceScene& sc, const PathQueue& in, const CloudQueue& cq, uint32_t* ctrl) {
  hipLaunchKernelGGL(k_clouds_list, dim3(grid), dim3(kBlock), 0, s, sc, in, cq, ctrl);
}
static void clouds_march(uint32_t grid, hipStream_t s, const DeviceScene& sc, const PathQueue& in, const CloudQueue& cq, uint32_t* ctrl, uint32_t depth_const) {
  hipLaunchKernelGGL(k_clouds_march, dim3(grid), dim3(kBlock), 0, s, sc, in, cq, ctrl, depth_const);
}
static void clouds(uint32_t grid, hipStream_t s, const DeviceScene& sc, const PathQueue& in, const CloudQueue& cq, float4* results, const uint32_t* ctrl, uint32_t depth_const) {
  hipLaunchKernelGGL(k_clouds, dim3(grid), dim3(kBlock), 0, s, sc, in, cq, results, ctrl, depth_const);
}
static void trace_rays(uint32_t grid, size_t lds, hipStream_t s, const DeviceScene& sc, uint32_t n, const float* origins, const float* dirs, const uint32_t* ignore, uint32_t* out,
                       uint32_t* cursor, uint64_t* counters, uint32_t lds_nodes, bool single_level) {
  hipLaunchKernelGGL(trace_rays_kernel(single_level && single_level_scene(sc)), dim3(grid), dim3(kTraceBlock), lds, s, sc, n, origins, dirs, ignore, out, cursor, counters,
                     lds_nodes);
}
static void guide(uint32_t grid, hipStream_t s, const DeviceScene& sc, const PathQueue& in, const uint32_t* ctrl, float* planes, uint32_t n) {
  hipLaunchKernelGGL(k_guide, dim3(grid), dim3(kBlock), 0, s, sc, in, ctrl, planes, n);
}
static void guide_normalise(uint32_t grid, hipStream_t s, float* planes, uint32_t n, uint32_t samples) {
  hipLaunchKernelGGL(k_guide_normalise, dim3(grid), dim3(256), 0, s, planes, n, samples);
}
static void denoise_prepare(uint32_t grid, hipStream_t s, const AdaptiveView& a, const DenoiseArgs& p, const float* fm, const float* sm, const float* image, const float* guides,
                            float4* rec_a, uint4* rec_b) {
  hipLaunchKernelGGL(k_denoise_prepare, dim3(grid), dim3(256), 0, s, a, p, fm, sm, image, guides, rec_a, rec_b);
}
static void denoise_atrous(hipStream_t s, const DenoiseArgs& p, const float4* a_in, const uint4* rec_b, float4* a_out, bool lds) {
  const dim3 grid((p.width + kDenoiseTileX - 1u) / kDenoiseTileX, (p.height + kDenoiseTileY - 1u) / kDenoiseTileY);
  if (lds && p.step <= kDenoiseMaxLdsStep) hipLaunchKernelGGL(k_denoise_atrous<true>, grid, dim3(256), 0, s, p, a_in, rec_b, a_out);
  else hipLaunchKernelGGL(k_denoise_atrous<false>, grid, dim3(256), 0, s, p, a_in, rec_b, a_out);
}
static void denoise_finish(uint32_t grid, hipStream_t s, const DenoiseArgs& p, const float4* rec_a, const float* guides, float* image) {
  hipLaunchKernelGGL(k_denoise_finish, dim3(grid), dim3(256), 0, s, p, rec_a, guides, image);
}
static void light_query_probe(hipStream_t s, const DeviceScene& sc, uint32_t n, const float* origins, const float* dirs, const uint32_t* self, const float* randoms, uint32_t* out_ids,
                              uint32_t* out_num_hits) {
  hipLaunchKernelGGL(k_light_query_probe, dim3((n + kBlock - 1) / kBlock), dim3(kBlock), 0, s, sc, n, origins, dirs, self, randoms, out_ids, out_num_hits);
}
static void light_sample_probe(hipStream_t s, const DeviceScene& sc, uint32_t n_vertices, uint32_t samples, uint32_t first_sample, uint32_t form, const uint32_t* vertices,
                               uint32_t* out) {
  static_assert(kLightProbeVertexWords == kLightSampleProbeVertexWords && kLightProbeWords == kLightSampleProbeWords, "the host layer sizes the probe's buffers by these");
  const uint32_t n = n_vertices * samples;
  if (form == 1u) hipLaunchKernelGGL(k_light_sample_probe<true>, dim3((n + kBlock - 1) / kBlock), dim3(kBlock), 0, s, sc, n, samples, first_sample, 1u, vertices, out);
  else hipLaunchKernelGGL(k_light_sample_probe<false>, dim3((n + kBlock - 1) / kBlock), dim3(kBlock), 0, s, sc, n, samples, first_sample, form == 2u ? 0u : 1u, vertices, out);
}

static constexpr WavefrontKernels make_table() {
  WavefrontKernels t{};
  t.flavour = LUM_FLAVOUR_NAME; t.trace_block = (uint32_t) kTraceBlock; t.set_ray_kernel_lds = set_ray_kernel_lds; t.init_sampler_seeds = init_sampler_seeds;
  t.sobol_table = sobol_table; t.generate = generate; t.generate_adaptive = generate_adaptive; t.trace = trace; t.sky_inscattering = sky_inscattering;
  t.shade = shade; t.shade_debug = shade_debug; t.sky = sky; t.light_query = light_query;
  t.shadow_rays = shadow_rays; t.resolve = resolve; t.resolve_reuse = resolve_reuse; t.resolve_listed = resolve_listed; t.resolve_ended = resolve_ended; t.fused_resolve = LUM_FAST != 0;
  t.volume_inscatter = volume_inscatter; t.volume_resolve = volume_resolve; t.volume_events = volume_events; t.volume_bounce = volume_bounce;
  t.trace_particles = trace_particles; t.particle_shade = particle_shade; t.trace_ocean = trace_ocean; t.ocean_shade = ocean_shade;
  t.clouds_list = clouds_list; t.clouds_march = clouds_march; t.clouds = clouds; t.trace_rays = trace_rays;
  t.camera_rays = camera_rays; t.guide = guide;
  t.guide_normalise = guide_normalise; t.denoise_prepare = denoise_prepare; t.denoise_atrous = denoise_atrous; t.denoise_finish = denoise_finish; t.light_query_probe = light_query_probe;
  return t;
}
static constexpr WavefrontKernels kTable = make_table();
static constexpr WavefrontProbes make_probes() {
  WavefrontProbes p{};
  p.light_sample_probe = light_sample_probe;
  return p;
}
static constexpr WavefrontProbes kProbes = make_probes();

}
LUM_NS_END

#ifdef LUM_PHASE_STATS
#if LUM_FAST
extern "C" int lumc_debug_phase_stats_fast(uint64_t out[16], int reset) {
  if (hipMemcpyFromSymbol(out, HIP_SYMBOL(g_phase), sizeof(uint64_t) * 16) != hipSuccess) return 1;
  if (reset) { const uint64_t zero[16] = {0}; if (hipMemcpyToSymbol(HIP_SYMBOL(g_phase), zero, sizeof(zero)) != hipSuccess) return 1; }
  return 0;
}
extern "C" int lumc_debug_phase_times_fast(uint64_t out[16], int reset) {
  if (hipMemcpyFromSymbol(out, HIP_SYMBOL(g_phase_time), sizeof(uint64_t) * 16) != hipSuccess) return 1;
  if (reset) { const uint64_t zero[16] = {0}; if (hipMemcpyToSymbol(HIP_SYMBOL(g_phase_time), zero, sizeof(zero)) != hipSuccess) return 1; }
  return 0;
}
extern "C" int lumc_debug_vis_stats_fast(uint64_t out[8], int reset) {
  if (hipMemcpyFromSymbol(out, HIP_SYMBOL(g_vis_stat), sizeof(uint64_t) * 8) != hipSuccess) return 1;
  if (reset) { const uint64_t zero[8] = {0}; if (hipMemcpyToSymbol(HIP_SYMBOL(g_vis_stat), zero, sizeof(zero)) != hipSuccess) return 1; }
  return 0;
}
extern "C" int lumc_debug_shade_times_fast(uint64_t out[16], int reset) {
  if (hipMemcpyFromSymbol(out, HIP_SYMBOL(g_shade_time), sizeof(uint64_t) * 16) != hipSuccess) return 1;
  if (reset) { const uint64_t zero[16] = {0}; if (hipMemcpyToSymbol(HIP_SYMBOL(g_shade_time), zero, sizeof(zero)) != hipSuccess) return 1; }
  return 0;
}
#else
extern "C" int lumc_debug_phase_stats(uint64_t out[16], int reset) {
  if (hipMemcpyFromSymbol(out, HIP_SYMBOL(g_phase), sizeof(uint64_t) * 16) != hipSuccess) return 1;
  if (reset) { const uint64_t zero[16] = {0}; if (hipMemcpyToSymbol(HIP_SYMBOL(g_phase), zero, sizeof(zero)) != hipSuccess) return 1; }
  return 0;
// ... 16 lines not shown
```

### luminary_amd/csrc/host/context.h

```cpp
#pragma once

#include <hip/hip_runtime.h>

#include <cstdio>
#include <map>
#include <memory>
#include <string>
#include <vector>

#include "../../../include/lum_core.h"
#include "../device/dev_scene.h"
#include "../device/wavefront_table.h"
#include "bvh_build.h"
#include "bvh_refit.h"
#include "device_buffer.h"
#include "instance_update.h"
#include "light_refit.h"
#include "mesh_deform.h"
#include "mesh_shutter.h"
#include "scene_arrays.h"
#include "work_layout.h"

using namespace lum;

typedef struct ncclComm* ncclComm_t;

struct MeshTree { Bvh4 bvh; bool built_on_gpu = false; };

struct MeshRefit {
  RefitPlan plan;
  std::shared_ptr<MeshTree> own;
  uint64_t fit_hash[2] = {0, 0};
  double built_cost = 0.0;
  bool stale = false;
  bool fit_to_pose = false;
};

struct LumContext {
  int device = 0;
  std::string error;
  const WavefrontKernels* wf = wavefront_kernels_fast();
  int camera = kCamThinLens;
  DeviceLens lens{};
  SceneArrays arrays;
  std::vector<std::shared_ptr<const MeshTree>> mesh_bvh;
  std::vector<Aabb> mesh_box;
  std::vector<MeshRefit> mesh_refit;
  std::vector<uint32_t> mesh_tri_offset;
  uint32_t refit_mode = 0;
  float refit_max_cost_growth = 0.0f;
  LumMeshRefitStats refit_stats{};
  InstanceUpdate instance_update;
  std::vector<uint32_t> instance_mesh_ids;
  std::vector<uint16_t> tri_material;
  std::vector<uint16_t> material_words;
  std::vector<uint32_t> light_handles;
  bool light_tree_flat = true;
  uint32_t instance_update_mode = 0;
  LumInstanceUpdateStats instance_stats{};
  uint32_t refit_in_place = 0;
  ResidentRefit resident_refit;
  uint32_t stale_meshes = 0;
  LumResidentRefitStats resident_stats{};
  std::map<uint32_t, MeshDeform> mesh_deform;
  DeviceBuffer<uint32_t> d_skin_flags;
  LumMeshSkinStats skin_stats{};
  LumMeshMorphStats morph_stats{};
  std::map<uint32_t, MeshShutter> mesh_shutter;
  DeviceBuffer<uint32_t> d_shutter_flags;
  LumShutterStats shutter_stats{};
  LightRefit light_refit;
  Bvh4 light_bvh;
  float light_refit_max_cost_growth = 0.0f;
  bool light_refit_needs_rebuild = false;
  bool lights_refitted = false;
  LumLightRefitStats light_refit_stats{};
  std::vector<uint32_t> sky_lut_key;
  DeviceBuffer<float> d_bridge_lut;
  std::vector<float> bridge_lut_host;
  DeviceBuffer<float4> d_sky_lut[2];
  DeviceScene scene{};
  bool has_scene = false;
  uint64_t bvh_stats[4] = {0, 0, 0, 0};
  int ambient_reuse = -1;
  int single_level = -1;
  int plain_form = -1;
  bool first_leaf_identity = false;
  int overlap_lq = -1;
  hipStream_t side_stream = nullptr;
  std::vector<hipEvent_t> overlap_events;
  bool overlap_fits[2][2] = {{false, false}, {false, false}};
  uint32_t shade_grid_rounds = 2;
  int fused_resolve = 1;
  struct Fused : FusedBuffers {
    DeviceBuffer<char> block;
    bool records_stale = false;
    uint32_t refused_capacity = 0;
  } fused;
  DeviceBuffer<uint2> d_sobol;
  int sobol_table = 1;
  int fused_ended = 1;
  int fused_ended_default = 1;
  int bvh_builder = 3;
  double bvh_build_seconds = 0.0;
  uint32_t bvh_meshes_by_builder[2] = {0, 0};
  uint32_t lds_nodes = 0;
  uint32_t trace_blocks = 256;
  DeviceBuffer<uint16_t> d_luts[4];
  DeviceBuffer<uint32_t> d_pixels;
  uint32_t num_pixels = 0;
  uint64_t pixels_hash = 0;
  DeviceBuffer<float> d_first_moment, d_second_moment;
  struct Work : WorkBuffers { DeviceBuffer<char> block; } work;
  uint32_t particle_lds_nodes = 0;
  DeviceBuffer<float> d_frame_output;
  DeviceBuffer<uint16_t> d_bluenoise_1d;
  DeviceBuffer<uint32_t> d_argb8;
  struct Adaptive {
    bool active = false;
    LumAdaptiveParams params{};
    uint32_t blocks_x = 0, blocks_y = 0, num_blocks = 0;
    uint32_t stage_id = 0;
    uint32_t executions[kAdaptiveStages + 1] = {0, 0, 0, 0, 0};
    DeviceBuffer<uint32_t> d_stage_counts, d_block_tasks, d_block_task_end;
    DeviceBuffer<float> d_block_variance;
    DeviceBuffer<float> d_partial;
    DeviceBuffer<char> d_scan_temp;
    size_t scan_temp_bytes = 0;
    std::vector<uint32_t> task_end;
    float variance_total = 0.0f;
    DeviceBuffer<uint8_t> d_block_mask;
    bool build_pending = false;
  } adaptive;
  DeviceBuffer<uint32_t> d_cloud_noise[3];
  bool cloud_noise_static = false;
  uint32_t cloud_noise_seed = 0;
  bool cloud_noise_weather_valid = false;
  DeviceBuffer<float4> d_sky_hdri;
  uint32_t sky_hdri_dim = 0;
  std::vector<DeviceBuffer<float>> bloom_mips;
  uint32_t bloom_width = 0, bloom_height = 0;
  DeviceBuffer<uint32_t> d_undersampling_pixels;
  std::vector<uint32_t> sky_hdri_key;
  DeviceBuffer<float> d_frame_result;
  DeviceBuffer<float> d_guides;
  bool guides_valid = false;
  DeviceBuffer<float4> d_denoise_rec[3];
  int denoise_lds = 1;
  struct RaySort {
    int mode = 0;
    PathQueue queue{};
    DeviceBuffer<float4> planes[4];
    int key = 0;
    DeviceBuffer<uint32_t> d_keys[2], d_vals[2];
    DeviceBuffer<char> d_temp;
    size_t temp_bytes = 0;
    float world_lo[3] = {0, 0, 0}, world_hi[3] = {1, 1, 1};
  } sort;
  bool sync_debug = false;
  struct Exchange {
    ncclComm_t comm = nullptr;
    int comm_rank = 0, comm_world = 1;
    DeviceBuffer<float> d_frame;
    uint32_t frame_pixels() const { return (uint32_t) (d_frame.count() / 4); }
    DeviceBuffer<float> d_gather_send, d_gather_recv;
    DeviceBuffer<uint32_t> d_gather_pixels;
    uint32_t gather_stride = 0, gather_key[3] = {0, 0, 0};
    bool use_frame = false;
  } exchange;
// ... 75 lines not shown
```

### luminary_amd/csrc/host/core.hip

```cpp
#include <hip/hip_runtime.h>

#include <algorithm>
#include <cmath>
#include <cstdio>
#include <cstdlib>
#include <cstring>
#include <string>
#include <vector>

#include "../../../include/lum_core.h"
#include "../device/kernels_shared.h"
#include <hipcub/hipcub.hpp>
#include "context.h"
#include "tiles.h"

static_assert(kLaunchBlock == (uint32_t) kBlock, "grid_for (context.h) counts the kernels' workgroups");

namespace {

void free_work(LumContext* ctx) {
  ctx->work = LumContext::Work{};
  ctx->fused = LumContext::Fused{};
  free_sort(ctx);
  ctx->d_sobol.reset();
// ... 29 lines not shown
  HIP_TRY(ctx, hipMemcpy(ctx->fused.records, by_depth, sizeof(by_depth), hipMemcpyHostToDevice));
  ctx->fused.records_stale = false;
  return 0;
}
int ensure_fused(LumContext* ctx, hipStream_t stream) {
  LumContext::Fused& f = ctx->fused;
  const uint32_t paths = ctx->work.capacity;
  if (f.block && f.capacity == paths) return f.records_stale ? upload_fused_records(ctx, stream) : 0;
  if (f.refused_capacity == paths) return 1;
  FusedBuffers sized;
  ArenaCarver size(nullptr);
  lay_out_fused(size, paths, ctx->work, sized);
  if (f.block.resize(size.used) != hipSuccess) { f.refused_capacity = paths; return 1; }
  ArenaCarver arena(f.block.get());
  lay_out_fused(arena, paths, ctx->work, f);
  ctx->work.queue[2] = f.queue;
  for (int k = 0; k < 3; k++) ctx->work.queue[k].parent = f.parent[k];
  return upload_fused_records(ctx, stream);
}

constexpr uint32_t kCtrlRows = 68;

inline uint32_t shade_grid(const LumContext* ctx, uint32_t n) {
  const uint32_t blocks = (n + kBlock - 1) / kBlock;
  const uint32_t resident = ctx->trace_blocks * 3u;
  const uint32_t rounds = ctx->shade_grid_rounds;
  const uint32_t cap = resident * (rounds ? rounds : 1u);
  return blocks < 1 ? 1 : std::min(blocks, cap);
}

int resolve_stamps(LumContext* ctx) {
  for (auto& st : ctx->stamps) {
    float ms = 0.0f;
    if (hipEventSynchronize(st.b) == hipSuccess && hipEventElapsedTime(&ms, st.a, st.b) == hipSuccess) {
      ctx->kernel_ms[st.kernel] += ms;
      ctx->kernel_launches[st.kernel]++;
    }
    (void) hipEventDestroy(st.a);
    (void) hipEventDestroy(st.b);
  }
  ctx->stamps.clear();
  return 0;
}

void prepare_overlap(LumContext* ctx) {
  int least = 0, greatest = 0;
  if (hipDeviceGetStreamPriorityRange(&least, &greatest) != hipSuccess) least = 0;
  if (hipStreamCreateWithPriority(&ctx->side_stream, hipStreamNonBlocking, least) != hipSuccess) ctx->side_stream = nullptr;
  for (int fast = 0; fast < 2; fast++)
    for (int single = 0; single < 2; single++) {
      uint32_t trace_regs = 0, light_query_regs = 0;
      const int e = fast ? ray_kernel_registers_fast(single != 0, &trace_regs, &light_query_regs) : ray_kernel_registers_exact(single != 0, &trace_regs, &light_query_regs);
      ctx->overlap_fits[fast][single] = e == 0 && overlap_registers_fit(trace_regs, light_query_regs);
    }
  (void) hipGetLastError();
}

int ensure_overlap_events(LumContext* ctx, uint32_t depths) {
  while (ctx->overlap_events.size() < 2u * (size_t) depths) {
    hipEvent_t e;
    HIP_TRY(ctx, hipEventCreateWithFlags(&e, hipEventDisableTiming));
    ctx->overlap_events.push_back(e);
  }
  return 0;
}

}

extern "C" {

int lumc_context_create(int device_ordinal, LumContext** out) {
  if (!out) return 1;
  *out = nullptr;
  LumContext* ctx = new LumContext();
  ctx->device = device_ordinal;
  if (const char* b = getenv("LUM_BVH_BUILDER")) ctx->bvh_builder = (std::strcmp(b, "lbvh") == 0) ? 1 : (std::strcmp(b, "ploc") == 0) ? 2 : (std::strcmp(b, "sah") == 0 || std::strcmp(b, "host") == 0) ? 0 : 3;
  if (const char* e = getenv("LUM_SORT")) ctx->sort.mode = atoi(e);
  if (const char* e = getenv("LUM_SYNC_DEBUG")) ctx->sync_debug = atoi(e) != 0;
  if (const char* e = getenv("LUM_SORT_KEY")) ctx->sort.key = atoi(e);
  if (const char* e = getenv("LUM_AMBIENT_REUSE")) ctx->ambient_reuse = atoi(e) != 0 ? 1 : 0;
  if (const char* e = getenv("LUM_SINGLE_LEVEL")) ctx->single_level = atoi(e) != 0 ? 1 : 0;
  if (const char* e = getenv("LUM_PLAIN_FORM")) ctx->plain_form = atoi(e) != 0 ? 1 : 0;
  if (const char* e = getenv("LUM_OVERLAP_LQ")) ctx->overlap_lq = atoi(e) != 0 ? 1 : 0;
  if (const char* e = getenv("LUM_FUSED_RESOLVE")) ctx->fused_resolve = atoi(e) != 0 ? 1 : 0;
  if (const char* e = getenv("LUM_SHADE_GRID")) ctx->shade_grid_rounds = (uint32_t) atoi(e);
  if (const char* e = getenv("LUM_SOBOL_TABLE_RT")) ctx->sobol_table = atoi(e) != 0 ? 1 : 0;
  if (const char* e = getenv("LUM_FUSED_ENDED")) ctx->fused_ended = ctx->fused_ended_default = atoi(e) != 0 ? 1 : 0;
  if (const char* e = getenv("LUM_DENOISE_LDS")) ctx->denoise_lds = atoi(e) != 0 ? 1 : 0;
  if (const char* f = getenv("LUM_FLAVOUR")) ctx->wf = (std::strcmp(f, "exact") == 0) ? wavefront_kernels_exact() : wavefront_kernels_fast();
  *out = ctx;
  int count = 0;
  HIP_TRY(ctx, hipGetDeviceCount(&count));
  if (device_ordinal < 0 || device_ordinal >= count) { ctx->error = "no such HIP device"; return 1; }
  HIP_TRY(ctx, hipSetDevice(device_ordinal));
  HIP_TRY(ctx, (hipError_t) wavefront_kernels_exact()->init_sampler_seeds());
  HIP_TRY(ctx, (hipError_t) wavefront_kernels_fast()->init_sampler_seeds());
  HIP_TRY(ctx, (hipError_t) exact::upload_sampler_seeds());
  HIP_TRY(ctx, (hipError_t) scene_device_init());
  HIP_TRY(ctx, ctx->d_ctrl.resize(kCtlStride * kCtrlRows));
  HIP_TRY(ctx, hipMemset(ctx->d_ctrl.get(), 0, sizeof(uint32_t) * kCtlStride * kCtrlRows));
  HIP_TRY(ctx, ctx->d_counters.resize(LUMC_CNT_COUNT));
  HIP_TRY(ctx, hipMemset(ctx->d_counters.get(), 0, sizeof(uint64_t) * LUMC_CNT_COUNT));
  prepare_overlap(ctx);
  return 0;
}

void lumc_context_destroy(LumContext* ctx) {
  if (!ctx) return;
  (void) hipSetDevice(ctx->device);
  (void) hipDeviceSynchronize();
  resolve_stamps(ctx);
  for (hipEvent_t e : ctx->overlap_events) (void) hipEventDestroy(e);
  if (ctx->side_stream) (void) hipStreamDestroy(ctx->side_stream);
  free_exchange(ctx);
  delete ctx;
}

const char* lumc_last_error(const LumContext* ctx) { return ctx ? ctx->error.c_str() : "null context"; }
uint32_t lumc_scene_view_sizeof(void) { return (uint32_t) sizeof(LumDeviceSceneView); }

uint64_t pixel_list_hash(const uint32_t* pixels, uint32_t n) {
  uint64_t h = 1469598103934665603ull;
  for (uint32_t i = 0; i < n; i++) { h ^= pixels ? pixels[i] : i; h *= 1099511628211ull; }
  return h;
}

int lumc_set_pixels(LumContext* ctx, const uint32_t* pixels, uint32_t num_pixels) {
  if (!ctx || !ctx->has_scene) { if (ctx) ctx->error = "lumc_set_pixels: no scene"; return 1; }
  HIP_TRY(ctx, hipSetDevice(ctx->device));
  if (!pixels) num_pixels = ctx->scene.width * ctx->scene.height;
  ctx->adaptive = LumContext::Adaptive();
  ctx->d_pixels.reset(); ctx->d_first_moment.reset(); ctx->d_second_moment.reset();
  ctx->num_pixels = num_pixels;
  ctx->pixels_hash = pixel_list_hash(pixels, num_pixels);
  if (num_pixels == 0) return 0;
  HIP_TRY(ctx, ctx->d_pixels.assign(pixels, num_pixels));
  HIP_TRY(ctx, ctx->d_first_moment.resize(3 * (size_t) num_pixels));
  HIP_TRY(ctx, ctx->d_second_moment.resize(num_pixels));
  return lumc_clear_accumulators(ctx);
}

int lumc_clear_accumulators(LumContext* ctx) {
  if (!ctx || !ctx->d_first_moment) return 1;
  HIP_TRY(ctx, hipMemset(ctx->d_first_moment.get(), 0, sizeof(float) * 3 * (size_t) ctx->num_pixels));
  HIP_TRY(ctx, hipMemset(ctx->d_second_moment.get(), 0, sizeof(float) * (size_t) ctx->num_pixels));
  return 0;
}

static void trace_particles(LumContext* ctx, hipStream_t stream, const PathQueue& q, uint32_t* ctrl, uint32_t N) {
  DeviceScene tree = ctx->scene;
  tree.bvh_nodes = tree.particle_bvh_nodes; tree.blas_tris = tree.particle_tris; tree.tlas_leaves = tree.particle_leaves; tree.tlas_num_nodes = tree.particle_tlas_num_nodes; tree.tlas_num_leaves = tree.particle_num_leaves;
  Launch l(ctx, stream, LUMC_KERNEL_TRACE);
  ctx->wf->trace_particles(grid_persistent(ctx, N), (size_t) ctx->particle_lds_nodes * kNodeBytes + LUM_LDS_STACK_BYTES, stream, tree, q, ctrl, ctx->particle_lds_nodes);
}

static bool ambient_reuse_active(const LumContext* ctx) {
  const DeviceScene& sc = ctx->scene;
  const bool wanted = ctx->ambient_reuse < 0 ? (ctx->wf == wavefront_kernels_fast()) : ctx->ambient_reuse != 0;
  return wanted && ctx->has_scene && sc.sky_mode != kSkyDefault && !sc.fog_active && !sc.ocean_active && !sc.particles_active && !sc.cloud_active &&
         !sc.sky_aerial_perspective && ctx->sort.mode == 0 && sc.shading_mode == 0u;
}

static void prepare_sobol_table(LumContext* ctx, hipStream_t stream, DeviceScene& sc, uint32_t first_sample, uint32_t sample_count) {
  sc.sobol_table = nullptr;
  if (!(ctx->sobol_table && sample_count > 0 && sample_count <= kSobolTableMaxSamples && sc.shading_mode == 0u)) return;
  const uint32_t stride = (sample_count + 15u) & ~15u, dims = (sc.max_ray_depth + 1u) * kRndTargetCount;
  const size_t entries = (size_t) stride * dims;
  if (ctx->d_sobol.count() < entries && ctx->d_sobol.resize(entries) != hipSuccess) (void) hipGetLastError();
  if (ctx->d_sobol) {
    ctx->wf->sobol_table(stream, ctx->d_sobol.get(), first_sample, sample_count, stride, dims);
    sc.sobol_table = ctx->d_sobol.get(); sc.sobol_first = first_sample; sc.sobol_count = sample_count; sc.sobol_stride = stride;
  }
}

static size_t ray_kernel_lds(const LumContext* ctx) { return (size_t) ctx->lds_nodes * kNodeBytes + LUM_LDS_STACK_BYTES; }
static bool render_volumes(const DeviceScene& sc) { return sc.fog_active || sc.ocean_active; }

static void first_hits(LumContext* ctx, hipStream_t stream, const DeviceScene& sc, uint32_t N) {
  const WavefrontKernels& wf = *ctx->wf;
  {
    Launch l(ctx, stream, LUMC_KERNEL_TRACE);
    wf.trace(grid_persistent(ctx, N), ray_kernel_lds(ctx), stream, sc, ctx->work.queue[0], nullptr, ctx->d_ctrl.get(), ctx->d_counters.get(), ctx->lds_nodes, single_level_allowed(ctx));
  }
  if (sc.particles_active) trace_particles(ctx, stream, ctx->work.queue[0], ctx->d_ctrl.get(), N);
  if (sc.ocean_active) {
    Launch l(ctx, stream, LUMC_KERNEL_TRACE);
    wf.trace_ocean(grid_for(N), stream, sc, ctx->work.queue[0], (const uint32_t*) ctx->d_ctrl.get());
  }
}

static void debug_pass(LumContext* ctx, hipStream_t stream, const DeviceScene& sc, uint32_t N) {
  const WavefrontKernels& wf = *ctx->wf;
  first_hits(ctx, stream, sc, N);
  if (render_volumes(sc)) {
    Launch l(ctx, stream, LUMC_KERNEL_VOLUME);
    wf.volume_events(grid_for(N), stream, sc, ctx->work.queue[0], ctx->work.volume, ctx->work.results, ctx->d_ctrl.get(), 0u);
  }
  if (sc.sky_aerial_perspective && sc.sky_mode != kSkyConstantColor) {
    Launch l(ctx, stream, LUMC_KERNEL_SKY);
    wf.sky_inscattering(grid_for(N), stream, sc, ctx->work.queue[0], ctx->work.results, (const uint32_t*) ctx->d_ctrl.get(), 0u);
  }
  Launch l(ctx, stream, LUMC_KERNEL_SHADE);
  wf.shade_debug(grid_for(N), stream, sc, ctx->work.queue[0], ctx->work.results, (const uint32_t*) ctx->d_ctrl.get());
}

enum ResolveScheme { kResolvePlain, kResolveReuse, kResolveFused };

static ResolveScheme wanted_scheme(const LumContext* ctx) {
  if (!ambient_reuse_active(ctx)) return kResolvePlain;
  return (ctx->wf->fused_resolve && ctx->fused_resolve != 0 && ctx->wf == wavefront_kernels_fast() && ctx->scene.max_ray_depth > 0) ? kResolveFused : kResolveReuse;
}

constexpr bool kOverlapAuto = true;
static bool overlap_allowed(const LumContext* ctx, ResolveScheme scheme) {
  const DeviceScene& sc = ctx->scene;
  const bool wanted = ctx->overlap_lq < 0 ? kOverlapAuto : ctx->overlap_lq != 0;
  if (!wanted || !ctx->has_scene || !ctx->side_stream || scheme == kResolveReuse || ctx->sort.mode != 0 || sc.shading_mode != 0u || sc.max_ray_depth == 0u) return false;
  if (sc.fog_active || sc.ocean_active || sc.particles_active || sc.cloud_active || sc.sky_aerial_perspective) return false;
  return ctx->overlap_fits[ctx->wf == wavefront_kernels_fast() ? 1 : 0][(single_level_allowed(ctx) && single_level_scene(sc)) ? 1 : 0];
}

struct DepthBuffers {
  PathQueue& cur;
  PathQueue& next;
  PathQueue& prev;
  NeeQueue& nee;
  NeeQueue& nee_before;
  uint32_t* ctrl;
  const FusedResolve* fused_records;
  uint32_t* ended;
  uint32_t depth, depth_const;
  bool last;
};

static DepthBuffers depth_buffers(LumContext* ctx, ResolveScheme scheme, uint32_t depth, uint32_t max_depth) {
  const bool fused = scheme == kResolveFused;
  const int cur = fused ? (int) (depth % 3u) : (int) (depth & 1u);
  const int next_q = fused ? (cur + 1) % 3 : (cur ^ 1), prev_q = fused ? (cur + 2) % 3 : (cur ^ 1);
  const bool second_set = fused && (depth & 1u);
  const uint32_t depth_const = (depth == max_depth && depth > 0) ? depth - 1 : depth;
  return DepthBuffers{ctx->work.queue[cur], ctx->work.queue[next_q], ctx->work.queue[prev_q], second_set ? ctx->fused.nee : ctx->work.nee, second_set ? ctx->work.nee : ctx->fused.nee,
                      ctx->d_ctrl.get() + kCtlStride * depth, fused ? ctx->fused.records + depth % 6u : nullptr, fused ? ctx->fused.ended[depth & 1u] : nullptr, depth, depth_const,
                      depth == max_depth};
}

static void trace_depth(LumContext* ctx, hipStream_t stream, const DeviceScene& sc, const DepthBuffers& d, const uint32_t* order, uint32_t N) {
  Launch l(ctx, stream, LUMC_KERNEL_TRACE);
  ctx->wf->trace(grid_persistent(ctx, N), ray_kernel_lds(ctx), stream, sc, d.cur, order, d.ctrl, ctx->d_counters.get(), ctx->lds_nodes, single_level_allowed(ctx));
}

static int closest_hits(LumContext* ctx, hipStream_t stream, const DeviceScene& sc, ResolveScheme scheme, const DepthBuffers& d, uint32_t N) {
  const WavefrontKernels& wf = *ctx->wf;
  const uint32_t* order = nullptr;
  if (ctx->sort.mode >= 1 && d.depth >= 1 && sort_closest_rays(ctx, stream, d.cur, d.ctrl, N, &order)) return 1;
  trace_depth(ctx, stream, sc, d, order, N);
  if (scheme == kResolveReuse && d.depth > 0) {
    uint32_t* prev = d.ctrl - kCtlStride;
    {
      Launch l(ctx, stream, LUMC_KERNEL_RESOLVE);
      wf.resolve_reuse(grid_for(N), stream, sc, d.prev, d.cur, d.nee, ctx->work.shadow, ctx->work.results, prev, ctx->d_counters.get());
    }
    {
      Launch l(ctx, stream, LUMC_KERNEL_SHADOW);
      wf.shadow_rays(ctx->trace_blocks, ray_kernel_lds(ctx), stream, sc, ctx->work.shadow, nullptr, prev + kCtlVolumeShift, ctx->d_counters.get(), ctx->lds_nodes, single_level_allowed(ctx));
    }
    Launch l(ctx, stream, LUMC_KERNEL_RESOLVE);
    wf.resolve_listed(std::min<uint32_t>(grid_for(N), 1024u), stream, sc, d.prev, d.nee, ctx->work.shadow, ctx->work.results, (const uint32_t*) prev);
  }
  return 0;
}

static void media_passes(LumContext* ctx, hipStream_t stream, const DeviceScene& sc, const DepthBuffers& d, uint32_t N) {
  const WavefrontKernels& wf = *ctx->wf;
  if (sc.particles_active) trace_particles(ctx, stream, d.cur, d.ctrl, N);
  if (sc.ocean_active) {
    Launch l(ctx, stream, LUMC_KERNEL_TRACE);
    wf.trace_ocean(grid_for(N), stream, sc, d.cur, (const uint32_t*) d.ctrl);
  }
  if (render_volumes(sc)) {
    {
      Launch l(ctx, stream, LUMC_KERNEL_VOLUME);
      wf.volume_inscatter(grid_for(N), stream, sc, d.cur, ctx->work.volume, ctx->work.shadow, d.ctrl, d.depth_const);
    }
    {
      Launch l(ctx, stream, LUMC_KERNEL_SHADOW);
      wf.shadow_rays(grid_persistent(ctx, N), ray_kernel_lds(ctx), stream, sc, ctx->work.shadow, nullptr, d.ctrl + kCtlVolumeShift, ctx->d_counters.get(), ctx->lds_nodes, single_level_allowed(ctx));
    }
    Launch l(ctx, stream, LUMC_KERNEL_VOLUME);
    wf.volume_resolve(grid_for(N), stream, sc, d.cur, ctx->work.volume, ctx->work.shadow, ctx->work.results, (const uint32_t*) d.ctrl);
    wf.volume_events(grid_for(N), stream, sc, d.cur, ctx->work.volume, ctx->work.results, d.ctrl, d.depth_const);
  }
  if (sc.cloud_active && sc.sky_mode == kSkyDefault && sc.cloud_noise_shape) {
    Launch l(ctx, stream, LUMC_KERNEL_SKY);
    wf.clouds_list(grid_for(N), stream, sc, d.cur, ctx->work.cloud, d.ctrl);
    wf.clouds_march(ctx->trace_blocks * 4u, stream, sc, d.cur, ctx->work.cloud, d.ctrl, d.depth_const);
    wf.clouds(grid_for(N), stream, sc, d.cur, ctx->work.cloud, ctx->work.results, (const uint32_t*) d.ctrl, d.depth_const);
  }
  if (sc.sky_aerial_perspective && sc.sky_mode != kSkyConstantColor) {
    Launch l(ctx, stream, LUMC_KERNEL_SKY);
    wf.sky_inscattering(grid_for(N), stream, sc, d.cur, ctx->work.results, (const uint32_t*) d.ctrl, d.depth_const);
  }
}

static void shade_depth(LumContext* ctx, hipStream_t stream, const DeviceScene& sc, ResolveScheme scheme, const DepthBuffers& d, uint32_t N) {
  const WavefrontKernels& wf = *ctx->wf;
  const bool fused = scheme == kResolveFused;
  {
    Launch l(ctx, stream, LUMC_KERNEL_SHADE);
    wf.shade(shade_grid(ctx, N), stream, sc, d.cur, d.next, d.nee, ctx->work.shadow, ctx->work.results, d.ctrl, d.depth_const, ctx->d_counters.get(),
             (scheme != kResolvePlain && !d.last) ? 1u : 0u, d.fused_records,
             fused ? ((d.depth > 0 ? 1u : 0u) | (!d.last ? 2u : 0u) | (ctx->fused_ended ? 4u : 0u)) : 0u, ctx->plain_form != 0);
  }
  if (fused && d.depth > 0) {
    {
      Launch l(ctx, stream, LUMC_KERNEL_SHADOW);
      wf.shadow_rays(ctx->trace_blocks, ray_kernel_lds(ctx), stream, sc, ctx->fused.fallback, nullptr, d.ctrl + kCtlVolumeShift, ctx->d_counters.get(), ctx->lds_nodes, single_level_allowed(ctx));
    }
    Launch l(ctx, stream, LUMC_KERNEL_RESOLVE);
    wf.resolve_listed(std::min<uint32_t>(grid_for(N), 1024u), stream, sc, d.prev, d.nee_before, ctx->fused.fallback, ctx->work.results, (const uint32_t*) d.ctrl);
  }
}

static void feature_shading(LumContext* ctx, hipStream_t stream, const DeviceScene& sc, const DepthBuffers& d, uint32_t N) {
  const WavefrontKernels& wf = *ctx->wf;
  if (sc.particles_active) {
    Launch l(ctx, stream, LUMC_KERNEL_SHADE);
    wf.particle_shade(grid_for(N), stream, sc, d.cur, d.next, d.nee, ctx->work.shadow, d.ctrl, d.depth_const);
  }
  if (sc.ocean_active) {
    Launch l(ctx, stream, LUMC_KERNEL_SHADE);
    wf.ocean_shade(grid_for(N), stream, sc, d.cur, d.next, d.nee, ctx->work.shadow, d.ctrl, d.depth_const);
  }
  if (sc.sky_mode == kSkyDefault) {
    Launch l(ctx, stream, LUMC_KERNEL_SKY);
    wf.sky(grid_for(N), stream, sc, d.cur, ctx->work.shadow, ctx->work.results, (const uint32_t*) d.ctrl, d.depth_const);
  }
}

static void light_queries(LumContext* ctx, hipStream_t stream, const DeviceScene& sc, const DepthBuffers& d, uint32_t N, bool beside_trace) {
  Launch l(ctx, stream, LUMC_KERNEL_LIGHT_QUERY);
  const uint32_t per_cu = beside_trace ? 1u : 4u;
  ctx->wf->light_query(std::min<uint32_t>(grid_for(N), ctx->trace_blocks * per_cu), stream, sc, d.cur, d.nee, ctx->work.shadow, d.ctrl, d.depth_const, ctx->d_counters.get());
}

static int visibility_and_resolve(LumContext* ctx, hipStream_t stream, const DeviceScene& sc, ResolveScheme scheme, const DepthBuffers& d, uint32_t N) {
  const WavefrontKernels& wf = *ctx->wf;
  const uint32_t* shadow_order = nullptr;
  if (ctx->sort.mode == 2) {
    shadow_order = sort_rays(ctx, stream, ctx->work.shadow.origin_dist, ctx->work.shadow.dir_out, d.ctrl + kCtlShadowItems,
                             (sc.ocean_active ? kSurfaceShadowKindsWater : 4u) * (ctx->work.shadow.capacity < N ? ctx->work.shadow.capacity : N));
    if (!shadow_order) { ctx->error = "ray sorting failed"; return 1; }
  }
  {
    Launch l(ctx, stream, LUMC_KERNEL_SHADOW);
    wf.shadow_rays(grid_persistent(ctx, N), ray_kernel_lds(ctx), stream, sc, ctx->work.shadow, shadow_order, d.ctrl, ctx->d_counters.get(), ctx->lds_nodes, single_level_allowed(ctx));
  }
  if (d.last || scheme == kResolvePlain) {
    Launch l(ctx, stream, LUMC_KERNEL_RESOLVE);
    wf.resolve(grid_for(N), stream, sc, d.cur, d.nee, ctx->work.shadow, ctx->work.results, (const uint32_t*) d.ctrl);
  }
  else if (scheme == kResolveFused) {
    if (!ctx->fused_ended) {
      Launch l(ctx, stream, LUMC_KERNEL_RESOLVE);
      wf.resolve_ended(std::min<uint32_t>(grid_for(N), 4096u), stream, sc, d.cur, d.nee, ctx->work.shadow, ctx->work.results, (const uint32_t*) d.ctrl, d.ended);
    }
  }
  return 0;
}

static void volume_bounce(LumContext* ctx, hipStream_t stream, const DeviceScene& sc, const DepthBuffers& d, uint32_t N) {
  if (render_volumes(sc) && !d.last) {
    Launch l(ctx, stream, LUMC_KERNEL_VOLUME);
    ctx->wf->volume_bounce(grid_for(N), stream, sc, d.cur, d.next, ctx->work.volume, d.ctrl, d.depth_const);
  }
}

static int wavefront_depths(LumContext* ctx, hipStream_t stream, uint32_t N, uint32_t first_sample = 0, uint32_t sample_count = 0) {
  DeviceScene sc = ctx->scene;
  const uint32_t max_depth = sc.max_ray_depth;
  prepare_sobol_table(ctx, stream, sc, first_sample, sample_count);
  if (sc.shading_mode != 0u) { debug_pass(ctx, stream, sc, N); return 0; }
  ResolveScheme scheme = wanted_scheme(ctx);
  if (scheme == kResolveFused && ensure_fused(ctx, stream) != 0) {
    (void) hipGetLastError();
    ctx->error.clear();
    scheme = kResolveReuse;
  }
  const bool overlap = overlap_allowed(ctx, scheme) && ensure_overlap_events(ctx, max_depth) == 0;
  hipStream_t side = ctx->side_stream;
  bool traced = false;
  for (uint32_t depth = 0; depth <= max_depth; depth++) {
    const DepthBuffers d = depth_buffers(ctx, scheme, depth, max_depth);
    if (!traced && closest_hits(ctx, stream, sc, scheme, d, N)) return 1;
    traced = false;
    media_passes(ctx, stream, sc, d, N);
    shade_depth(ctx, stream, sc, scheme, d, N);
    feature_shading(ctx, stream, sc, d, N);
    if (overlap && !d.last) {
      hipEvent_t shaded = ctx->overlap_events[2u * depth], queried = ctx->overlap_events[2u * depth + 1u];
      HIP_TRY(ctx, hipEventRecord(shaded, stream));
      HIP_TRY(ctx, hipStreamWaitEvent(side, shaded, 0));
      light_queries(ctx, side, sc, d, N, true);
      const hipError_t recorded = hipEventRecord(queried, side);
      if (recorded != hipSuccess) (void) hipStreamSynchronize(side);
      HIP_TRY(ctx, recorded);
      trace_depth(ctx, stream, sc, depth_buffers(ctx, scheme, depth + 1u, max_depth), nullptr, N);
      traced = true;
      HIP_TRY(ctx, hipStreamWaitEvent(stream, queried, 0));
    }
    else light_queries(ctx, stream, sc, d, N, false);
    if (visibility_and_resolve(ctx, stream, sc, scheme, d, N)) return 1;
    volume_bounce(ctx, stream, sc, d, N);
  }
  return 0;
}

int lumc_render(LumContext* ctx, uint32_t first_sample, uint32_t num_samples, uint32_t samples_per_pass, float* d_fm, float* d_sm, void* stream_) {
  if (!ctx || !ctx->has_scene) { if (ctx) ctx->error = "lumc_render: no scene"; return 1; }
  if (ctx->num_pixels == 0) return 0;
  hipStream_t stream = (hipStream_t) stream_;
  HIP_TRY(ctx, hipSetDevice(ctx->device));
  if (!d_fm) { d_fm = ctx->d_first_moment.get(); d_sm = ctx->d_second_moment.get(); }
  if (samples_per_pass == 0) samples_per_pass = 1;
  if (first_sample >= kMaxGlobalSamples) return 0;
  if (first_sample + (uint64_t) num_samples > kMaxGlobalSamples) num_samples = kMaxGlobalSamples - first_sample;
  const uint32_t P = ctx->num_pixels;
  const uint64_t want = (uint64_t) P * samples_per_pass;
  if (want > 0x7FFFFFFFull) { ctx->error = "pass too large"; return 1; }
  if (ensure_work(ctx, (uint32_t) want)) return 1;
  const DeviceScene& sc = ctx->scene;
  const uint32_t max_depth = sc.max_ray_depth;

  for (uint32_t done = 0; done < num_samples; done += samples_per_pass) {
    const uint32_t batch = std::min(samples_per_pass, num_samples - done);
    const uint32_t N = P * batch;
    PassParams pp{ctx->d_pixels.get(), P, batch, first_sample + done};
    HIP_TRY(ctx, hipMemsetAsync(ctx->d_ctrl.get(), 0, sizeof(uint32_t) * kCtlStride * (max_depth + 2), stream));
    {
      Launch l(ctx, stream, LUMC_KERNEL_GENERATE);
      ctx->wf->generate(grid_for(N), stream, sc, pp, ctx->work.queue[0], ctx->work.results, ctx->d_ctrl.get() + kCtlPaths, ctx->lens, ctx->camera);
    }
    if (wavefront_depths(ctx, stream, N, first_sample + done, batch)) return 1;
    {
      Launch l(ctx, stream, LUMC_KERNEL_ACCUMULATE);
      hipLaunchKernelGGL(k_accumulate, dim3(grid_for(P)), dim3(kBlock), 0, stream, (const float4*) ctx->work.results, P, batch, d_fm, d_sm);
    }
    HIP_TRY(ctx, hipGetLastError());
  }
  return 0;
}

int lumc_render_undersampled(LumContext* ctx, uint32_t stage, uint32_t iteration, void* stream_) {
  if (!ctx || !ctx->has_scene || !ctx->d_first_moment || ctx->d_pixels || ctx->num_pixels != ctx->scene.width * ctx->scene.height) {
    if (ctx) ctx->error = "lumc_render_undersampled: needs the full-frame accumulators";
    return 1;
  }
  if (stage == 0 || stage > 15 || iteration > 3) { ctx->error = "lumc_render_undersampled: stage in [1, 15], iteration in [0, 3]"; return 1; }
  hipStream_t stream = (hipStream_t) stream_;
  HIP_TRY(ctx, hipSetDevice(ctx->device));
  const DeviceScene& sc = ctx->scene;
  const std::vector<uint32_t> px = undersampling_pixels(sc.width, sc.height, stage, iteration);
  const uint32_t n = (uint32_t) px.size();
  if (n == 0) return 0;
  if (ctx->d_undersampling_pixels.count() < n) HIP_TRY(ctx, ctx->d_undersampling_pixels.resize(n));
  HIP_TRY(ctx, hipMemcpyAsync(ctx->d_undersampling_pixels.get(), px.data(), sizeof(uint32_t) * (size_t) n, hipMemcpyHostToDevice, stream));
  HIP_TRY(ctx, hipStreamSynchronize(stream));
  if (ensure_work(ctx, n)) return 1;
  PassParams pp{ctx->d_undersampling_pixels.get(), n, 1u, 0u};
  HIP_TRY(ctx, hipMemsetAsync(ctx->d_ctrl.get(), 0, sizeof(uint32_t) * kCtlStride * (sc.max_ray_depth + 2), stream));
  {
    Launch l(ctx, stream, LUMC_KERNEL_GENERATE);
    ctx->wf->generate(grid_for(n), stream, sc, pp, ctx->work.queue[0], ctx->work.results, ctx->d_ctrl.get() + kCtlPaths, ctx->lens, ctx->camera);
  }
  if (wavefront_depths(ctx, stream, n)) return 1;
  {
    Launch l(ctx, stream, LUMC_KERNEL_ACCUMULATE);
    hipLaunchKernelGGL(k_accumulate_scatter, dim3(grid_for(n)), dim3(kBlock), 0, stream, (const float4*) ctx->work.results, (const uint32_t*) ctx->d_undersampling_pixels.get(), n,
                       ctx->num_pixels, ctx->d_first_moment.get(), ctx->d_second_moment.get());
  }
  HIP_TRY(ctx, hipGetLastError());
  return 0;
}

namespace {

AdaptiveView adaptive_view(const LumContext* ctx) {
  const LumContext::Adaptive& a = ctx->adaptive;
  AdaptiveView v;
  v.stage_counts = a.d_stage_counts.get(); v.block_task_end = a.d_block_task_end.get();
  v.blocks_x = a.blocks_x; v.blocks_y = a.blocks_y; v.num_blocks = a.num_blocks;
  for (uint32_t s = 0; s <= kAdaptiveStages; s++) v.executions[s] = a.executions[s];
  v.stage_id = a.stage_id;
  return v;
}

OutputParams tone_params(const LumOutputParams* p) {
  OutputParams op;
  std::memset(&op, 0, sizeof(op));
  if (p) std::memcpy(&op, p, sizeof(op));
  return op;
}

int adaptive_compute_variance(LumContext* ctx, hipStream_t stream) {
  LumContext::Adaptive& a = ctx->adaptive;
  const DeviceScene& sc = ctx->scene;
  const AdaptiveView view = adaptive_view(ctx);
  const OutputParams op = tone_params(&a.params.tone);
  hipLaunchKernelGGL(k_adaptive_block_variance, dim3((a.num_blocks * 16 + 255) / 256), dim3(256), 0, stream, view, op, sc.width, sc.height, a.params.exposure,
                     (const float*) ctx->d_first_moment.get(), (const float*) ctx->d_second_moment.get(), a.d_block_variance.get());
  HIP_TRY(ctx, hipGetLastError());
  return 0;
}

int adaptive_task_prefix(LumContext* ctx, hipStream_t stream) {
  LumContext::Adaptive& a = ctx->adaptive;
  const uint32_t nb = a.num_blocks;
  HIP_TRY(ctx, hipcub::DeviceScan::InclusiveSum(a.d_scan_temp.get(), a.scan_temp_bytes, a.d_block_tasks.get(), a.d_block_task_end.get(), (int) nb, stream));
  a.task_end.resize(nb);
  HIP_TRY(ctx, hipMemcpyAsync(a.task_end.data(), a.d_block_task_end.get(), sizeof(uint32_t) * nb, hipMemcpyDeviceToHost, stream));
  HIP_TRY(ctx, hipStreamSynchronize(stream));
  return 0;
}

int adaptive_finish_build(LumContext* ctx, hipStream_t stream) {
  LumContext::Adaptive& a = ctx->adaptive;
  const uint32_t nb = a.num_blocks, chunks = (nb + kAdaptiveSumChunk - 1) / kAdaptiveSumChunk;
  hipLaunchKernelGGL(k_adaptive_sum_chunks, dim3((chunks + 63) / 64), dim3(64), 0, stream, (const float*) a.d_block_variance.get(), nb, a.d_partial.get());
  hipLaunchKernelGGL(k_adaptive_sum_total, dim3(1), dim3(1), 0, stream, (const float*) a.d_partial.get(), chunks, a.d_partial.get() + chunks);
// ... 462 lines not shown
  return 0;
}
int lumc_set_profiling(LumContext* ctx, int enabled) {
  if (!ctx) return 1;
  ctx->profiling = enabled != 0;
  for (int k = 0; k < LUMC_KERNEL_COUNT; k++) { ctx->kernel_ms[k] = 0.0; ctx->kernel_launches[k] = 0; }
  return 0;
}
int lumc_kernel_times(LumContext* ctx, double total_ms[LUMC_KERNEL_COUNT], uint32_t launches[LUMC_KERNEL_COUNT]) {
  if (!ctx) return 1;
  if (lumc_synchronize(ctx)) return 1;
  for (int k = 0; k < LUMC_KERNEL_COUNT; k++) { total_ms[k] = ctx->kernel_ms[k]; launches[k] = ctx->kernel_launches[k]; }
  return 0;
}

extern "C" const unsigned char lum_embedded_bluenoise_1d[];
extern "C" const unsigned char lum_embedded_bluenoise_1d_end[];

int lumc_generate_output(LumContext* ctx, const LumOutputParams* params, const float* d_first_moment, uint32_t* d_argb8, void* stream_) {
  if (!ctx || !params || !d_argb8) { if (ctx) ctx->error = "lumc_generate_output: null argument"; return 1; }
  static_assert(sizeof(LumOutputParams) == sizeof(OutputParams), "output parameter structs must match");
  HIP_TRY(ctx, hipSetDevice(ctx->device));
  hipStream_t stream = (hipStream_t) stream_;
  OutputParams p;
  std::memcpy(&p, params, sizeof(p));
  if (p.src_width == 0 || p.src_height == 0 || p.dst_width < 2 || p.dst_height < 2) { ctx->error = "lumc_generate_output: image sizes must be at least 2x2"; return 1; }
  if (p.supersampling > 3 || p.undersampling_stage > 15) { ctx->error = "lumc_generate_output: supersampling at most 3, undersampling stage at most 15"; return 1; }
  const uint32_t ns = p.src_width * p.src_height;
  const uint32_t uo = std::max(p.undersampling_stage, p.supersampling);
  const uint32_t n_out = (p.src_width >> uo) * (p.src_height >> uo);
  if (n_out == 0) { ctx->error = "lumc_generate_output: the frame is smaller than one output pixel"; return 1; }
  if (!d_first_moment) {
    if (p.undersampling_stage) { ctx->error = "lumc_generate_output: an undersampled image must be passed explicitly (lumc_result_image)"; return 1; }
    if (!ctx->d_first_moment || ctx->d_pixels || ctx->num_pixels != ns) { ctx->error = "lumc_generate_output: the context does not hold a full frame of this size"; return 1; }
    d_first_moment = ctx->d_first_moment.get();
  }
  if (!ctx->d_bluenoise_1d) {
    const size_t bytes = (size_t) (lum_embedded_bluenoise_1d_end - lum_embedded_bluenoise_1d);
    if (bytes != 65536 * sizeof(uint16_t)) { ctx->error = "embedded 1D blue-noise mask has the wrong size"; return 1; }
    HIP_TRY(ctx, ctx->d_bluenoise_1d.assign((const uint16_t*) lum_embedded_bluenoise_1d, 65536));
  }
  if (ctx->d_frame_output.count() < 3 * (size_t) ns) HIP_TRY(ctx, ctx->d_frame_output.resize(3 * (size_t) ns));
  {
    Launch l(ctx, stream, LUMC_KERNEL_OUTPUT);
    hipLaunchKernelGGL(k_final_image, dim3(grid_for(n_out)), dim3(256), 0, stream, p, d_first_moment, ctx->d_frame_output.get());
    hipLaunchKernelGGL(k_to_argb8, dim3(grid_for(p.dst_width * p.dst_height)), dim3(256), 0, stream, p, (const float*) ctx->d_frame_output.get(),
                       (const uint16_t*) ctx->d_bluenoise_1d.get(), d_argb8);
  }
  HIP_TRY(ctx, hipGetLastError());
  return 0;
}

int lumc_generate_output_host(LumContext* ctx, const LumOutputParams* params, const float* d_first_moment, uint32_t* argb8, float* frame_output) {
  if (!ctx || !params || !argb8) { if (ctx) ctx->error = "lumc_generate_output_host: null argument"; return 1; }
  HIP_TRY(ctx, hipSetDevice(ctx->device));
  const uint32_t n = params->dst_width * params->dst_height;
  if (ctx->d_argb8.count() < n) HIP_TRY(ctx, ctx->d_argb8.resize(n));
  if (lumc_generate_output(ctx, params, d_first_moment, ctx->d_argb8.get(), nullptr)) return 1;
  HIP_TRY(ctx, hipDeviceSynchronize());
  HIP_TRY(ctx, hipMemcpy(argb8, ctx->d_argb8.get(), sizeof(uint32_t) * (size_t) n, hipMemcpyDeviceToHost));
  if (frame_output) {
    const uint32_t uo = std::max(params->undersampling_stage, params->supersampling);
    HIP_TRY(ctx, hipMemcpy(frame_output, ctx->d_frame_output.get(), sizeof(float) * 3 * (size_t) (params->src_width >> uo) * (params->src_height >> uo), hipMemcpyDeviceToHost));
  }
  return 0;
}

int lumc_generate_output_from_host(LumContext* ctx, const LumOutputParams* params, const float* first_moment, uint32_t* argb8, float* frame_output) {
  if (!ctx || !params || !first_moment || !argb8) { if (ctx) ctx->error = "lumc_generate_output_from_host: null argument"; return 1; }
  HIP_TRY(ctx, hipSetDevice(ctx->device));
  DeviceBuffer<float> d;
  HIP_TRY(ctx, d.assign(first_moment, 3 * (size_t) (params->src_width >> params->undersampling_stage) * (params->src_height >> params->undersampling_stage)));
  return lumc_generate_output_host(ctx, params, d.get(), argb8, frame_output);
}

int lumc_trace_closest(LumContext* ctx, uint32_t n, const float* d_origins, const float* d_dirs, const uint32_t* d_ignore, uint32_t* d_out, void* stream_) {
  if (!ctx || !ctx->has_scene) { if (ctx) ctx->error = "lumc_trace_closest: no scene"; return 1; }
  if (n == 0) return 0;
  hipStream_t stream = (hipStream_t) stream_;
  uint32_t* cursor = ctx->d_ctrl.get() + kCtlStride * (kCtrlRows - 1);
  HIP_TRY(ctx, hipMemsetAsync(cursor, 0, sizeof(uint32_t), stream));
  Launch l(ctx, stream, LUMC_KERNEL_TRACE);
  ctx->wf->trace_rays(grid_persistent(ctx, n), ray_kernel_lds(ctx), stream, ctx->scene, n, d_origins, d_dirs, d_ignore, d_out, cursor, ctx->d_counters.get(),
                      ctx->lds_nodes, single_level_allowed(ctx));
  HIP_TRY(ctx, hipGetLastError());
  return 0;
}

int lumc_trace_closest_host(LumContext* ctx, uint32_t n, const float* origins, const float* dirs, const uint32_t* ignore, uint32_t* out) {
  if (!ctx || !ctx->has_scene) { if (ctx) ctx->error = "lumc_trace_closest_host: no scene"; return 1; }
  if (n == 0) return 0;
  DeviceBuffer<float> d_o, d_d;
  DeviceBuffer<uint32_t> d_i, d_out;
  HIP_TRY(ctx, d_o.assign(origins, 3 * (size_t) n));
  HIP_TRY(ctx, d_d.assign(dirs, 3 * (size_t) n));
  HIP_TRY(ctx, d_out.resize(3 * (size_t) n));
  HIP_TRY(ctx, d_i.assign(ignore, 2 * (size_t) n));
  if (lumc_trace_closest(ctx, n, d_o.get(), d_d.get(), d_i.get(), d_out.get(), nullptr)) return 1;
  HIP_TRY(ctx, hipMemcpy(out, d_out.get(), sizeof(uint32_t) * 3 * (size_t) n, hipMemcpyDeviceToHost));
  return 0;
}

int lumc_trace_visibility(LumContext* ctx, uint32_t n, const float* d_origins, const float* d_dirs, const float* d_dist, const uint32_t* d_ids, const uint32_t* d_order, float* d_out,
                          void* stream_) {
  if (!ctx || !ctx->has_scene) { if (ctx) ctx->error = "lumc_trace_visibility: no scene"; return 1; }
  if (n == 0) return 0;
  if (!d_origins || !d_dirs || !d_dist || !d_ids || !d_out) { ctx->error = "lumc_trace_visibility: null argument"; return 1; }
  hipStream_t stream = (hipStream_t) stream_;
  HIP_TRY(ctx, hipSetDevice(ctx->device));
  DeviceBuffer<float4> buffer;
  HIP_TRY(ctx, buffer.resize(4 * (size_t) n));
  float4* items = buffer.get();
  ShadowQueue sq{};
  sq.origin_dist = items; sq.dir_out = items + n; sq.ids = reinterpret_cast<uint4*>(items + 2 * (size_t) n); sq.vis = items + 3 * (size_t) n;
  sq.capacity = n;
  uint32_t* ctrl = ctx->d_ctrl.get() + kCtlStride * (kCtrlRows - 2);
  const uint32_t blocks = (n + 255u) / 256u;
  HIP_TRY(ctx, hipMemsetAsync(sq.vis, 0xFF, sizeof(float4) * (size_t) n, stream));
  HIP_TRY(ctx, hipMemsetD32Async((hipDeviceptr_t) (ctrl + kCtlShadowItems), (int) n, 1, stream));
  HIP_TRY(ctx, hipMemsetAsync(ctrl + kCtlShadowCursor, 0, sizeof(uint32_t), stream));
  hipLaunchKernelGGL(k_visibility_pack, dim3(blocks), dim3(256), 0, stream, n, d_origins, d_dirs, d_dist, d_ids, sq);
  {
    Launch l(ctx, stream, LUMC_KERNEL_SHADOW);
    ctx->wf->shadow_rays(grid_persistent(ctx, n), ray_kernel_lds(ctx), stream, ctx->scene, sq, d_order, ctrl, ctx->d_counters.get(), ctx->lds_nodes, single_level_allowed(ctx));
  }
  hipLaunchKernelGGL(k_visibility_unpack, dim3(blocks), dim3(256), 0, stream, n, sq.vis, d_out);
  HIP_TRY(ctx, hipGetLastError());
  HIP_TRY(ctx, hipStreamSynchronize(stream));
  return 0;
}

int lumc_trace_visibility_host(LumContext* ctx, uint32_t n, const float* origins, const float* dirs, const float* dist, const uint32_t* ids, const uint32_t* order, float* out) {
  if (!ctx || !ctx->has_scene) { if (ctx) ctx->error = "lumc_trace_visibility_host: no scene"; return 1; }
  if (n == 0) return 0;
  if (!origins || !dirs || !dist || !ids || !out) { ctx->error = "lumc_trace_visibility_host: null argument"; return 1; }
  if (order) {
    for (uint32_t i = 0; i < n; i++) if (order[i] >= n) { ctx->error = "lumc_trace_visibility_host: order entry out of range"; return 1; }
  }
  HIP_TRY(ctx, hipSetDevice(ctx->device));
  DeviceBuffer<float> d_o, d_d, d_t, d_out;
  DeviceBuffer<uint32_t> d_i, d_ord;
  HIP_TRY(ctx, d_o.assign(origins, 3 * (size_t) n));
  HIP_TRY(ctx, d_d.assign(dirs, 3 * (size_t) n));
  HIP_TRY(ctx, d_t.assign(dist, n));
  HIP_TRY(ctx, d_i.assign(ids, 4 * (size_t) n));
  HIP_TRY(ctx, d_ord.assign(order, n));
  HIP_TRY(ctx, d_out.resize(3 * (size_t) n));
  if (lumc_trace_visibility(ctx, n, d_o.get(), d_d.get(), d_t.get(), d_i.get(), d_ord.get(), d_out.get(), nullptr)) return 1;
  HIP_TRY(ctx, hipMemcpy(out, d_out.get(), sizeof(float) * 3 * (size_t) n, hipMemcpyDeviceToHost));
  return 0;
}

int lumc_light_query_host(LumContext* ctx, uint32_t n, const float* origins, const float* dirs, const uint32_t* self, const float* randoms, uint32_t* out_ids, uint32_t* out_num_hits) {
  if (!ctx || !ctx->has_scene) { if (ctx) ctx->error = "lumc_light_query_host: no scene"; return 1; }
  if (n == 0) return 0;
  if (!origins || !dirs || !self || !randoms || !out_ids || !out_num_hits) { ctx->error = "lumc_light_query_host: null argument"; return 1; }
  const DeviceScene& sc = ctx->scene;
  if (!sc.num_lights || !sc.light_nodes || !sc.light_tris || !sc.light_tri_handles) {
    for (uint32_t i = 0; i < n; i++) { out_ids[i] = 0xFFFFFFFFu; out_num_hits[i] = 0u; }
    return 0;
  }
  HIP_TRY(ctx, hipSetDevice(ctx->device));
  DeviceBuffer<float> d_o, d_d, d_r;
  DeviceBuffer<uint32_t> d_s, d_out;
  HIP_TRY(ctx, d_o.assign(origins, 3 * (size_t) n));
  HIP_TRY(ctx, d_d.assign(dirs, 3 * (size_t) n));
  HIP_TRY(ctx, d_s.assign(self, 2 * (size_t) n));
// ... 80 lines not shown
  l.image_plane_distance = c->image_plane_distance; l.sensor_width = c->sensor_width; l.num_interfaces = n;
  std::memcpy(l.iface, c->interfaces, sizeof(LensInterface) * n);
  std::memcpy(l.medium, c->media, sizeof(LensMedium) * (n + 1));
  ctx->lens = l;
  ctx->camera = c->allow_reflections ? kCamPhysicalReflections : kCamPhysical;
  return 0;
}

int lumc_camera_rays(LumContext* ctx, const uint32_t* pixels, uint32_t n, uint32_t first_sample, uint32_t samples, float* out_origin, float* out_dir, float* out_weight) {
  if (!ctx || !ctx->has_scene || !pixels || !out_origin || !out_dir || !out_weight) { if (ctx) ctx->error = "lumc_camera_rays: no scene or null argument"; return 1; }
  const uint64_t total = (uint64_t) n * samples;
  if (total == 0) return 0;
  if (total > 0x7FFFFFFFull) { ctx->error = "lumc_camera_rays: too many rays"; return 1; }
  for (uint32_t p = 0; p < n; p++)
    if (pixels[p] >= ctx->scene.width * ctx->scene.height) { ctx->error = "lumc_camera_rays: pixel outside the frame"; return 1; }
  HIP_TRY(ctx, hipSetDevice(ctx->device));
  DeviceBuffer<uint32_t> d_px;
  DeviceBuffer<float> rays;
  HIP_TRY(ctx, d_px.resize(n));
  HIP_TRY(ctx, rays.resize(7 * (size_t) total));
  HIP_TRY(ctx, hipMemcpy(d_px.get(), pixels, sizeof(uint32_t) * (size_t) n, hipMemcpyHostToDevice));
  float* d = rays.get();
  ctx->wf->camera_rays(grid_for((uint32_t) total), 0, ctx->scene, ctx->lens, ctx->camera, d_px.get(), n, first_sample, samples, d, d + 3 * total, d + 6 * total);
  HIP_TRY(ctx, hipGetLastError());
  HIP_TRY(ctx, hipDeviceSynchronize());
  HIP_TRY(ctx, hipMemcpy(out_origin, d, sizeof(float) * 3 * total, hipMemcpyDeviceToHost));
  HIP_TRY(ctx, hipMemcpy(out_dir, d + 3 * total, sizeof(float) * 3 * total, hipMemcpyDeviceToHost));
  HIP_TRY(ctx, hipMemcpy(out_weight, d + 6 * total, sizeof(float) * total, hipMemcpyDeviceToHost));
  return 0;
}

int lumc_device_name(int ordinal, char* out, size_t size) {
  if (!out || size == 0) return 1;
  hipDeviceProp_t prop;
  if (hipGetDeviceProperties(&prop, ordinal) != hipSuccess) { out[0] = 0; return 1; }
  std::snprintf(out, size, "%s", prop.name);
  return 0;
}

int lumc_set_flavour(LumContext* ctx, int flavour) {
  if (!ctx || flavour < 0 || flavour > 1) { if (ctx) ctx->error = "lumc_set_flavour: 0 (exact) or 1 (fast)"; return 1; }
  ctx->wf = flavour == LUMC_FLAVOUR_FAST ? wavefront_kernels_fast() : wavefront_kernels_exact();
  return 0;
}
int lumc_set_fused_resolve(LumContext* ctx, int on) {
  if (!ctx) return 1;
  ctx->fused_resolve = on != 0 ? 1 : 0;
  ctx->fused_ended = on == 2 ? 0 : ctx->fused_ended_default;
  return 0;
}
int lumc_set_sobol_table(LumContext* ctx, int on) {
  if (!ctx) return 1;
  ctx->sobol_table = on != 0 ? 1 : 0;
  return 0;
}
int lumc_set_ambient_reuse(LumContext* ctx, int mode) {
  if (!ctx || mode < -1 || mode > 1) { if (ctx) ctx->error = "lumc_set_ambient_reuse: -1 (by flavour), 0 (off) or 1 (on)"; return 1; }
  ctx->ambient_reuse = mode;
  return 0;
}
int lumc_get_ambient_reuse(const LumContext* ctx) { return (ctx && ambient_reuse_active(ctx)) ? 1 : 0; }

int lumc_set_single_level(LumContext* ctx, int mode) {
  if (!ctx || mode < -1 || mode > 1) { if (ctx) ctx->error = "lumc_set_single_level: -1 (auto), 0 (never) or 1 (when the scene is eligible)"; return 1; }
  ctx->single_level = mode;
  return 0;
}
int lumc_get_single_level(const LumContext* ctx) { return (ctx && ctx->has_scene && single_level_allowed(ctx) && single_level_scene(ctx->scene)) ? 1 : 0; }

int lumc_set_plain_form(LumContext* ctx, int mode) {
  if (!ctx || mode < -1 || mode > 1) { if (ctx) ctx->error = "lumc_set_plain_form: -1 (auto), 0 (never) or 1 (when the scene is eligible)"; return 1; }
  ctx->plain_form = mode;
  return 0;
}

int lumc_get_plain_form(const LumContext* ctx) { return (ctx && ctx->has_scene && ctx->plain_form != 0 && plain_scene(ctx->scene)) ? 1 : 0; }

int lumc_set_overlap_light_query(LumContext* ctx, int mode) {
  if (!ctx || mode < -1 || mode > 1) { if (ctx) ctx->error = "lumc_set_overlap_light_query: -1 (auto), 0 (never) or 1 (when the pass allows it)"; return 1; }
  ctx->overlap_lq = mode;
  return 0;
}
int lumc_get_overlap_light_query(const LumContext* ctx) { return (ctx && ctx->has_scene && overlap_allowed(ctx, wanted_scheme(ctx))) ? 1 : 0; }
int lumc_overlap_registers_fit(uint32_t ray_kernel_regs, uint32_t light_query_regs) { return overlap_registers_fit(ray_kernel_regs, light_query_regs) ? 1 : 0; }
int lumc_get_flavour(const LumContext* ctx) { return (ctx && ctx->wf == wavefront_kernels_exact()) ? LUMC_FLAVOUR_EXACT : LUMC_FLAVOUR_FAST; }

unsigned int lumc_lds_stack_bytes(void) { return LUM_LDS_STACK_BYTES; }

}
```

Baseline: 4247.

## Add pixel-major sample slots and wave-coherent first-hit traversal

Path slots are reordered so that all samples of a pixel are adjacent, and this pixel-major order is on by default. The accumulate kernel gains an LDS-tiled transpose path to read that layout. For primary rays on single-level scenes, a coherent traversal mode visits a node once for the whole wave when every live lane is at the same node with the same octant. It uses scalar constant-address loads for that node and refills only when the whole wave is idle. This aims to cut divergent node fetches for coherent camera rays, at the cost of extra ballots and possible idle lanes while the wave waits for a full refill.

```diff
diff --git a/include/lum_core.h b/include/lum_core.h
--- a/include/lum_core.h
+++ b/include/lum_core.h
@@ -252,6 +252,10 @@
 int lumc_get_plain_form(const LumContext* ctx);
 int lumc_set_overlap_light_query(LumContext* ctx, int mode);
 int lumc_get_overlap_light_query(const LumContext* ctx);
+int lumc_set_pixel_major(LumContext* ctx, int mode);
+int lumc_get_pixel_major(const LumContext* ctx);
+int lumc_set_coherent_first_hits(LumContext* ctx, int mode);
+int lumc_get_coherent_first_hits(const LumContext* ctx);
 int lumc_overlap_registers_fit(uint32_t ray_kernel_regs, uint32_t light_query_regs);
 int lumc_set_fused_resolve(LumContext* ctx, int on);
 int lumc_set_sobol_table(LumContext* ctx, int on);
diff --git a/luminary_amd/core.py b/luminary_amd/core.py
--- a/luminary_amd/core.py
+++ b/luminary_amd/core.py
@@ -429,6 +429,22 @@
         fn.restype = C.c_int
         return int(fn(self._ctx))
 
+    def set_pixel_major(self, mode):
+        self._call("lumc_set_pixel_major", C.c_int(mode))
+
+    def get_pixel_major(self):
+        fn = self._lib.lumc_get_pixel_major
+        fn.restype = C.c_int
+        return int(fn(self._ctx))
+
+    def set_coherent_first_hits(self, mode):
+        self._call("lumc_set_coherent_first_hits", C.c_int(mode))
+
+    def get_coherent_first_hits(self):
+        fn = self._lib.lumc_get_coherent_first_hits
+        fn.restype = C.c_int
+        return int(fn(self._ctx))
+
     @staticmethod
     def overlap_registers_fit(ray_kernel_regs, light_query_regs):
         fn = _lib().lumc_overlap_registers_fit
diff --git a/luminary_amd/csrc/device/dev_scene.h b/luminary_amd/csrc/device/dev_scene.h
--- a/luminary_amd/csrc/device/dev_scene.h
+++ b/luminary_amd/csrc/device/dev_scene.h
@@ -183,6 +183,7 @@
 struct PassParams {
   const uint32_t* pixels;
   uint32_t num_pixels, batch, first_sample;
+  uint32_t pixel_major;
 };
 
 constexpr uint32_t kAdaptiveStages = 4;
diff --git a/luminary_amd/csrc/device/dev_trace.h b/luminary_amd/csrc/device/dev_trace.h
--- a/luminary_amd/csrc/device/dev_trace.h
+++ b/luminary_amd/csrc/device/dev_trace.h
@@ -126,11 +126,33 @@
   LUM_DEV void store(int i, E e) { if (i < lds_entries) lds[(uint32_t) i * (uint32_t) kTraceBlock] = StackWord<E>::pack(e); else scratch[i] = StackWord<E>::pack(e); }
   LUM_DEV E load(int i) const { if (i < lds_entries) return StackWord<E>::unpack(lds[(uint32_t) i * (uint32_t) kTraceBlock]); return StackWord<E>::unpack(scratch[i]); }
 };
+template <bool kOrdered, bool kCull, int kFarFirst, typename S>
+LUM_DEV uint32_t enter_children(float4 nx, float4 ny, float4 nz, float4 fx, float4 fy, float4 fz, uint4 ch, const TRay& r, float tmax, S& stk, int& sp,
+                                typename StackEntry<kCull>::E& top) {
+  using SE = StackEntry<kCull>;
+  float k0 = child_entry<kFarFirst>(nx.x, ny.x, nz.x, fx.x, fy.x, fz.x, r, tmax);
+  float k1 = child_entry<kFarFirst>(nx.y, ny.y, nz.y, fx.y, fy.y, fz.y, r, tmax);
+  float k2 = child_entry<kFarFirst>(nx.z, ny.z, nz.z, fx.z, fy.z, fz.z, r, tmax);
+  float k3 = child_entry<kFarFirst>(nx.w, ny.w, nz.w, fx.w, fy.w, fz.w, r, tmax);
+  uint32_t c0 = ch.x, c1 = ch.y, c2 = ch.z, c3 = ch.w;
+  if (kOrdered) {
+    cswap(k0, c0, k1, c1); cswap(k2, c2, k3, c3); cswap(k0, c0, k2, c2); cswap(k1, c1, k3, c3); cswap(k1, c1, k2, c2);
+  }
+  const float inf = __builtin_inff();
+  if (k1 < inf) {
+    if (k2 < inf) {
+      if (k3 < inf) { stk.store(sp, top); sp++; top = SE::make(c3, k3); }
+      stk.store(sp, top); sp++; top = SE::make(c2, k2);
+    }
+    stk.store(sp, top); sp++; top = SE::make(c1, k1);
+  }
+  return (k0 < inf) ? c0 : kBvhEmpty;
+}
+
 template <bool kOrdered, bool kCull, int kFarFirst = 0, typename S>
 LUM_DEV uint32_t visit_node(const NodeSource& src, uint32_t cur, const TRay& r, float tmax, S& stk, int& sp,
                             typename StackEntry<kCull>::E& top, RayStats& st) {
   static_assert(!(kFarFirst && kCull), "the negated keys are not distances: only for queries that do not cull by them");
-  using SE = StackEntry<kCull>;
   const uint32_t b = cur << 7;
   float4 nx, ny, nz, fx, fy, fz;
   uint4 ch;
@@ -147,23 +169,39 @@
     fx = node_f4(nodes, b + r.fx); fy = node_f4(nodes, b + r.fy); fz = node_f4(nodes, b + r.fz);
     ch = node_u4(nodes, b + 96u);
   }
-  float k0 = child_entry<kFarFirst>(nx.x, ny.x, nz.x, fx.x, fy.x, fz.x, r, tmax);
-  float k1 = child_entry<kFarFirst>(nx.y, ny.y, nz.y, fx.y, fy.y, fz.y, r, tmax);
-  float k2 = child_entry<kFarFirst>(nx.z, ny.z, nz.z, fx.z, fy.z, fz.z, r, tmax);
-  float k3 = child_entry<kFarFirst>(nx.w, ny.w, nz.w, fx.w, fy.w, fz.w, r, tmax);
-  uint32_t c0 = ch.x, c1 = ch.y, c2 = ch.z, c3 = ch.w;
-  if (kOrdered) {
-    cswap(k0, c0, k1, c1); cswap(k2, c2, k3, c3); cswap(k0, c0, k2, c2); cswap(k1, c1, k3, c3); cswap(k1, c1, k2, c2);
-  }
-  const float inf = __builtin_inff();
-  if (k1 < inf) {
-    if (k2 < inf) {
-      if (k3 < inf) { stk.store(sp, top); sp++; top = SE::make(c3, k3); }
-      stk.store(sp, top); sp++; top = SE::make(c2, k2);
-    }
-    stk.store(sp, top); sp++; top = SE::make(c1, k1);
-  }
-  return (k0 < inf) ? c0 : kBvhEmpty;
+  return enter_children<kOrdered, kCull, kFarFirst>(nx, ny, nz, fx, fy, fz, ch, r, tmax, stk, sp, top);
+}
+
+typedef float NodePlanes __attribute__((ext_vector_type(4)));
+typedef uint32_t NodeChildren __attribute__((ext_vector_type(4)));
+template <bool kOrdered, bool kCull, int kFarFirst = 0, typename S>
+LUM_DEV uint32_t visit_node_uniform(const NodeSource& src, uint32_t cur, uint32_t octant, const TRay& r, float tmax, S& stk, int& sp, typename StackEntry<kCull>::E& top,
+                                    RayStats& st) {
+  const uint32_t b = cur << 7;
+  const uint32_t onx = octant & 0xFFu, ony = (octant >> 8) & 0xFFu, onz = octant >> 16;
+  const uint32_t ofx = 48u - onx, ofy = 80u - ony, ofz = 112u - onz;
+  float4 nx, ny, nz, fx, fy, fz;
+  uint4 ch;
+  if (cur < src.lds_count) {
+    const char* p = src.lds + b;
+    nx = *reinterpret_cast<const float4*>(p + onx); ny = *reinterpret_cast<const float4*>(p + ony); nz = *reinterpret_cast<const float4*>(p + onz);
+    fx = *reinterpret_cast<const float4*>(p + ofx); fy = *reinterpret_cast<const float4*>(p + ofy); fz = *reinterpret_cast<const float4*>(p + ofz);
+    ch = *reinterpret_cast<const uint4*>(p + 96u);
+    st.lds_nodes++;
+  }
+  else {
+    typedef const char __attribute__((address_space(4)))* ConstBytes;
+    typedef const NodePlanes __attribute__((address_space(4)))* ConstPlanes;
+    typedef const NodeChildren __attribute__((address_space(4)))* ConstChildren;
+    const ConstBytes p = (ConstBytes) src.global + b;
+    const NodePlanes anx = *(ConstPlanes) (p + onx), any = *(ConstPlanes) (p + ony), anz = *(ConstPlanes) (p + onz);
+    const NodePlanes afx = *(ConstPlanes) (p + ofx), afy = *(ConstPlanes) (p + ofy), afz = *(ConstPlanes) (p + ofz);
+    const NodeChildren ach = *(ConstChildren) (p + 96u);
+    nx = make_float4(anx.x, anx.y, anx.z, anx.w); ny = make_float4(any.x, any.y, any.z, any.w); nz = make_float4(anz.x, anz.y, anz.z, anz.w);
+    fx = make_float4(afx.x, afx.y, afx.z, afx.w); fy = make_float4(afy.x, afy.y, afy.z, afy.w); fz = make_float4(afz.x, afz.y, afz.z, afz.w);
+    ch = make_uint4(ach.x, ach.y, ach.z, ach.w);
+  }
+  return enter_children<kOrdered, kCull, kFarFirst>(nx, ny, nz, fx, fy, fz, ch, r, tmax, stk, sp, top);
 }
 
 template <typename S>
@@ -198,8 +236,15 @@
 LUM_DEV uint32_t instance_of(const OneInstance<false>&, uint32_t entered) { return entered; }
 LUM_DEV uint32_t instance_of(const OneInstance<true>& one, uint32_t) { return one.inst; }
 
-template <class Q, bool kSingleLevel = false>
+#ifndef LUM_COHERENT_REFILL
+#define LUM_COHERENT_REFILL 1
+#endif
+template <bool kCoherent> struct WaveOctant {};
+template <> struct WaveOctant<true> { uint32_t word; };
+
+template <class Q, bool kSingleLevel = false, bool kCoherent = false>
 LUM_DEV void trace_items(const DeviceScene& sc, uint32_t n, uint32_t* __restrict__ cursor, Q& q, RayStats& st, uint32_t& rays, uint32_t lds_count) {
+  static_assert(kSingleLevel || !kCoherent, "the coherent form is a single-level form");
   if (n == 0u) return;
   using SE = StackEntry<Q::kCull>;
   using E = typename SE::E;
@@ -226,6 +271,9 @@
     __syncthreads();
   }
   [[maybe_unused]] OneInstance<kSingleLevel> one;
+  [[maybe_unused]] WaveOctant<kCoherent> oct;
+  if constexpr (kCoherent) oct.word = 0u;
+  constexpr bool kWholeWaveRefill = kCoherent && LUM_COHERENT_REFILL != 0;
   if constexpr (kSingleLevel) {
     const float4* __restrict__ leaf = sc.tlas_leaves;
     const float4 meta = leaf[3];
@@ -279,9 +327,9 @@
     const unsigned long long idle = __ballot(cur == kTraversalDone);
 #ifdef LUM_PHASE_STATS
     const unsigned long long t_refill_ = __builtin_readcyclecounter();
-    const bool refilling_ = idle != 0ull && more;
-#endif
-    if (idle != 0ull && more) {
+    const bool refilling_ = (kWholeWaveRefill ? idle == ~0ull : idle != 0ull) && more;
+#endif
+    if ((kWholeWaveRefill ? idle == ~0ull : idle != 0ull) && more) {
       if (chunk_next >= chunk_end) {
         uint32_t base = 0;
         if (lane == 0) base = atomicAdd(cursor, chunk);
@@ -308,6 +356,7 @@
                 const V3 od = v3(mat_row_apply(r0.x, r0.y, r0.z, wd.x, wd.y, wd.z), mat_row_apply(r1.x, r1.y, r1.z, wd.x, wd.y, wd.z),
                                  mat_row_apply(r2.x, r2.y, r2.z, wd.x, wd.y, wd.z));
                 r.set(oo, od); cur = one.root; sp = 0; top = SE::make(kTraversalDone, 0.0f);
+                if constexpr (kCoherent) oct.word = r.nx | (r.ny << 8) | (r.nz << 16);
               }
               else q.finish(sc, idx);
             }
@@ -323,11 +372,38 @@
 #ifdef LUM_PHASE_STATS
     if (refilling_) { ptime_[8] += __builtin_readcyclecounter() - t_refill_; ptime_[9]++; }
 #endif
-    if (__ballot(cur != kTraversalDone) == 0ull) break;
+    if (__ballot(cur != kTraversalDone) == 0ull) {
+      if constexpr (kWholeWaveRefill) { if (more) continue; }
+      break;
+    }
     LUM_PHASE(5);
 
     while (true) {
       const bool live = cur != kTraversalDone;
+      if constexpr (kCoherent) {
+        const unsigned long long live_lanes = __ballot(live);
+        if (live_lanes == 0ull) break;
+        const int first = __builtin_ctzll(live_lanes);
+        const uint32_t cur0 = (uint32_t) __builtin_amdgcn_readlane((int) cur, first), oct0 = (uint32_t) __builtin_amdgcn_readlane((int) oct.word, first);
+        if (!(cur0 & kBvhLeafBit) && __ballot(live && (cur != cur0 || oct.word != oct0)) == 0ull) {
+          LUM_TIME_BEGIN();
+          if (live) {
+            LUM_PHASE(0);
+            st.nodes++;
+            cur = visit_node_uniform<Q::kOrdered, Q::kCull, Q::kFarFirst>(nodes, cur0, oct0, r, tmax, stk, sp, top, st);
+            if (cur == kBvhEmpty) {
+              pop();
+              if (cur == kTraversalDone) q.finish(sc, idx);
+            }
+          }
+#ifdef LUM_PHASE_STATS
+          asm volatile("s_waitcnt vmcnt(0) lgkmcnt(0)" ::: "memory");
+          LUM_TIME_END(cur0 >= lds_count ? 0 : 2);
+#endif
+          if constexpr (!kWholeWaveRefill) { if (more && (uint32_t) __popcll(live_lanes) < LUM_REFILL) break; }
+          continue;
+        }
+      }
       const bool at_leaf = live && (cur & kBvhLeafBit);
       const bool want_tris = at_leaf && (kSingleLevel || inst != kNoInstance), want_enter = !kSingleLevel && at_leaf && inst == kNoInstance;
       const uint32_t n_live = (uint32_t) __popcll(__ballot(live)), n_tris = (uint32_t) __popcll(__ballot(want_tris)),
@@ -384,7 +460,7 @@
         LUM_TIME_END(kind);
       }
 #endif
-      if (more && n_live < LUM_REFILL) break;
+      if constexpr (!kWholeWaveRefill) { if (more && n_live < LUM_REFILL) break; }
     }
   }
 #ifdef LUM_PHASE_STATS
diff --git a/luminary_amd/csrc/device/kernels.h b/luminary_amd/csrc/device/kernels.h
--- a/luminary_amd/csrc/device/kernels.h
+++ b/luminary_amd/csrc/device/kernels.h
@@ -70,12 +70,18 @@
   }
 }
 
+LUM_DEV void pass_slot_split(const PassParams& pp, uint32_t i, uint32_t& p, uint32_t& b) {
+  if (pp.pixel_major) { p = i / pp.batch; b = i - p * pp.batch; }
+  else { b = i / pp.num_pixels; p = i - b * pp.num_pixels; }
+}
+
 template <int kCam>
 __global__ __launch_bounds__(kBlock) void k_generate(DeviceScene sc, PassParams pp, PathQueue q, float4* results, uint32_t* count, DeviceLens lens_arg) {
   const uint32_t total = pp.num_pixels * pp.batch;
   if constexpr (kCam == kCamThinLens) {
     for (uint32_t i = blockIdx.x * kBlock + threadIdx.x; i < total; i += gridDim.x * kBlock) {
-      const uint32_t b = i / pp.num_pixels, p = i - b * pp.num_pixels;
+      uint32_t b, p;
+      pass_slot_split(pp, i, p, b);
       const uint32_t index = pp.pixels ? pp.pixels[p] : p;
       const uint32_t y = index / sc.width, x = index - y * sc.width;
       const Sampler smp{sc.bluenoise_2d, x, y, pp.first_sample + b, 0};
@@ -99,8 +105,8 @@
       const bool active = i < total;
       uint32_t x = 0, y = 0, b = 0;
       if (active) {
-        b = i / pp.num_pixels;
-        const uint32_t p = i - b * pp.num_pixels;
+        uint32_t p;
+        pass_slot_split(pp, i, p, b);
         const uint32_t index = pp.pixels ? pp.pixels[p] : p;
         y = index / sc.width; x = index - y * sc.width;
         results[i] = make_float4(0.0f, 0.0f, 0.0f, 0.0f);
@@ -212,6 +218,18 @@
   tq.order = order;
   tq.item = 0;
   trace_items<TraceQuery, true>(sc, ctrl[kCtlPaths], ctrl + kCtlTraceCursor, tq, st, rays, lds_nodes);
+  flush_stats(counters, st, rays, kCntTrace, kCntNodes, kCntTris, kCntNodesLds);
+}
+template <bool kSingleLevel, bool kCoherent>
+__global__ LUM_TRACE_BOUNDS void k_trace(DeviceScene sc, PathQueue q, const uint32_t* order, uint32_t* ctrl, uint64_t* counters, uint32_t lds_nodes) {
+  static_assert(kSingleLevel && kCoherent, "the other forms are the kernels of this name with fewer parameters");
+  RayStats st{0, 0, 0};
+  uint32_t rays = 0;
+  TraceQuery tq;
+  tq.q = q;
+  tq.order = order;
+  tq.item = 0;
+  trace_items<TraceQuery, true, true>(sc, ctrl[kCtlPaths], ctrl + kCtlTraceCursor, tq, st, rays, lds_nodes);
   flush_stats(counters, st, rays, kCntTrace, kCntNodes, kCntTris, kCntNodesLds);
 }
 
@@ -1418,6 +1436,17 @@
   RaysQuery q;
   q.origins = origins; q.dirs = dirs; q.ignore = ignore; q.out = out;
   trace_items<RaysQuery, true>(sc, n, cursor, q, st, rays, lds_nodes);
+  flush_stats(counters, st, rays, kCntTrace, kCntNodes, kCntTris, kCntNodesLds);
+}
+template <bool kSingleLevel, bool kCoherent>
+__global__ LUM_TRACE_BOUNDS void k_trace_rays(DeviceScene sc, uint32_t n, const float* origins, const float* dirs, const uint32_t* ignore,
+                                                           uint32_t* out, uint32_t* cursor, uint64_t* counters, uint32_t lds_nodes) {
+  static_assert(kSingleLevel && kCoherent, "the other forms are the kernels of this name with fewer parameters");
+  RayStats st{0, 0, 0};
+  uint32_t rays = 0;
+  RaysQuery q;
+  q.origins = origins; q.dirs = dirs; q.ignore = ignore; q.out = out;
+  trace_items<RaysQuery, true, true>(sc, n, cursor, q, st, rays, lds_nodes);
   flush_stats(counters, st, rays, kCntTrace, kCntNodes, kCntTris, kCntNodesLds);
 }
 
diff --git a/luminary_amd/csrc/device/kernels_shared.h b/luminary_amd/csrc/device/kernels_shared.h
--- a/luminary_amd/csrc/device/kernels_shared.h
+++ b/luminary_amd/csrc/device/kernels_shared.h
@@ -281,7 +281,48 @@
   }
 }
 
-__global__ __launch_bounds__(kBlock) void k_accumulate(const float4* results, uint32_t num_pixels, uint32_t batch, float* first_moment, float* second_moment) {
+constexpr uint32_t kAccTile = 8;
+constexpr uint32_t kAccTileBytes = kBlock * kAccTile * (uint32_t) sizeof(float4);
+LUM_DEV void accumulate_pixel_major(const float4* __restrict__ results, uint32_t num_pixels, uint32_t batch, float* first_moment, float* second_moment, float4* tiles) {
+  static_assert(kAccTile == 8u, "the swizzle and the shifts below are written for rows of eight");
+  const uint32_t lane = threadIdx.x & 63u;
+  float4* tile = tiles + (threadIdx.x >> 6) * (64u * kAccTile);
+  const uint32_t rounds = (num_pixels + gridDim.x * kBlock - 1u) / (gridDim.x * kBlock);
+  for (uint32_t round = 0; round < rounds; round++) {
+    const uint32_t p = (round * gridDim.x + blockIdx.x) * kBlock + threadIdx.x;
+    const uint32_t p0 = p - lane;
+    const bool active = p < num_pixels;
+    float r = 0.0f, g = 0.0f, b = 0.0f, s = 0.0f;
+    if (active) {
+      r = first_moment[p]; g = first_moment[num_pixels + p]; b = first_moment[2 * num_pixels + p];
+      s = second_moment ? second_moment[p] : 0.0f;
+    }
+    for (uint32_t k0 = 0; k0 < batch; k0 += kAccTile) {
+      const uint32_t kc = min(kAccTile, batch - k0);
+#pragma unroll
+      for (uint32_t j = 0; j < kAccTile; j++) {
+        const uint32_t e = j * 64u + lane, row = e >> 3, at = e & 7u;
+        if (p0 + row < num_pixels && at < kc) tile[row * kAccTile + (at ^ (row & 7u))] = results[(size_t) (p0 + row) * batch + k0 + at];
+      }
+      __syncthreads();
+      if (active) {
+        for (uint32_t k = 0; k < kc; k++) {
+          const float4 v = tile[lane * kAccTile + (k ^ (lane & 7u))];
+          r += v.x; g += v.y; b += v.z;
+          s += luminance(col(v.x * v.x, v.y * v.y, v.z * v.z));
+        }
+      }
+      __syncthreads();
+    }
+    if (active) {
+      first_moment[p] = r; first_moment[num_pixels + p] = g; first_moment[2 * num_pixels + p] = b;
+      if (second_moment) second_moment[p] = s;
+    }
+  }
+}
+__global__ __launch_bounds__(kBlock) void k_accumulate(const float4* results, uint32_t num_pixels, uint32_t batch, float* first_moment, float* second_moment, uint32_t pixel_major) {
+  extern __shared__ float4 accumulate_tiles[];
+  if (pixel_major) { accumulate_pixel_major(results, num_pixels, batch, first_moment, second_moment, accumulate_tiles); return; }
   for (uint32_t p = blockIdx.x * kBlock + threadIdx.x; p < num_pixels; p += gridDim.x * kBlock) {
     float r = first_moment[p], g = first_moment[num_pixels + p], b = first_moment[2 * num_pixels + p];
     float s = second_moment ? second_moment[p] : 0.0f;
diff --git a/luminary_amd/csrc/device/wavefront_table.h b/luminary_amd/csrc/device/wavefront_table.h
--- a/luminary_amd/csrc/device/wavefront_table.h
+++ b/luminary_amd/csrc/device/wavefront_table.h
@@ -24,7 +24,7 @@
   void (*generate_adaptive)(uint32_t grid, hipStream_t s, const DeviceScene& sc, const AdaptiveView& a, const AdaptivePass& pass, const PathQueue& q, float4* results,
                             uint32_t* count, const DeviceLens& lens, int cam);
   void (*trace)(uint32_t grid, size_t lds, hipStream_t s, const DeviceScene& sc, const PathQueue& q, const uint32_t* order, uint32_t* ctrl, uint64_t* counters,
-                uint32_t lds_nodes, bool single_level);
+                uint32_t lds_nodes, bool single_level, bool coherent);
   void (*sky_inscattering)(uint32_t grid, hipStream_t s, const DeviceScene& sc, const PathQueue& in, float4* results, const uint32_t* ctrl, uint32_t depth_const);
   void (*shade)(uint32_t grid, hipStream_t s, const DeviceScene& sc, const PathQueue& in, const PathQueue& out, const NeeQueue& nee, const ShadowQueue& sq, float4* results,
                 uint32_t* ctrl, uint32_t depth_const, uint64_t* counters, uint32_t ambient_reuse, const FusedResolve* fused_dev, uint32_t fused_flags,
@@ -59,7 +59,7 @@
   void (*clouds_march)(uint32_t grid, hipStream_t s, const DeviceScene& sc, const PathQueue& in, const CloudQueue& cq, uint32_t* ctrl, uint32_t depth_const);
   void (*clouds)(uint32_t grid, hipStream_t s, const DeviceScene& sc, const PathQueue& in, const CloudQueue& cq, float4* results, const uint32_t* ctrl, uint32_t depth_const);
   void (*trace_rays)(uint32_t grid, size_t lds, hipStream_t s, const DeviceScene& sc, uint32_t n, const float* origins, const float* dirs, const uint32_t* ignore, uint32_t* out,
-                     uint32_t* cursor, uint64_t* counters, uint32_t lds_nodes, bool single_level);
+                     uint32_t* cursor, uint64_t* counters, uint32_t lds_nodes, bool single_level, bool coherent);
   void (*camera_rays)(uint32_t grid, hipStream_t s, const DeviceScene& sc, const DeviceLens& lens, int cam, const uint32_t* pixels, uint32_t n, uint32_t first_sample,
                       uint32_t samples, float* origin, float* dir, float* weight);
   void (*guide)(uint32_t grid, hipStream_t s, const DeviceScene& sc, const PathQueue& in, const uint32_t* ctrl, float* planes, uint32_t n);
diff --git a/luminary_amd/csrc/device/wavefront_table_impl.h b/luminary_amd/csrc/device/wavefront_table_impl.h
--- a/luminary_amd/csrc/device/wavefront_table_impl.h
+++ b/luminary_amd/csrc/device/wavefront_table_impl.h
@@ -10,9 +10,11 @@
 typedef void (*TraceKernel)(DeviceScene, PathQueue, const uint32_t*, uint32_t*, uint64_t*, uint32_t);
 typedef void (*ShadowKernel)(DeviceScene, ShadowQueue, const uint32_t*, uint32_t*, uint64_t*, uint32_t);
 typedef void (*TraceRaysKernel)(DeviceScene, uint32_t, const float*, const float*, const uint32_t*, uint32_t*, uint32_t*, uint64_t*, uint32_t);
-static TraceKernel trace_kernel(bool single) { return single ? k_trace<true> : static_cast<TraceKernel>(k_trace); }
+static TraceKernel trace_kernel(bool single, bool coherent = false) { return single ? (coherent ? k_trace<true, true> : k_trace<true>) : static_cast<TraceKernel>(k_trace); }
 static ShadowKernel shadow_kernel(bool single) { return single ? k_shadow_rays<true> : static_cast<ShadowKernel>(k_shadow_rays); }
-static TraceRaysKernel trace_rays_kernel(bool single) { return single ? k_trace_rays<true> : static_cast<TraceRaysKernel>(k_trace_rays); }
+static TraceRaysKernel trace_rays_kernel(bool single, bool coherent = false) {
+  return single ? (coherent ? k_trace_rays<true, true> : k_trace_rays<true>) : static_cast<TraceRaysKernel>(k_trace_rays);
+}
 
 static int set_ray_kernel_lds(size_t bytes) {
   hipError_t e = hipSuccess;
@@ -21,6 +23,8 @@
     if (e == hipSuccess) e = hipFuncSetAttribute((const void*) shadow_kernel(single != 0), hipFuncAttributeMaxDynamicSharedMemorySize, (int) bytes);
     if (e == hipSuccess) e = hipFuncSetAttribute((const void*) trace_rays_kernel(single != 0), hipFuncAttributeMaxDynamicSharedMemorySize, (int) bytes);
   }
+  if (e == hipSuccess) e = hipFuncSetAttribute((const void*) trace_kernel(true, true), hipFuncAttributeMaxDynamicSharedMemorySize, (int) bytes);
+  if (e == hipSuccess) e = hipFuncSetAttribute((const void*) trace_rays_kernel(true, true), hipFuncAttributeMaxDynamicSharedMemorySize, (int) bytes);
   if (e == hipSuccess) e = hipFuncSetAttribute((const void*) k_trace_particles, hipFuncAttributeMaxDynamicSharedMemorySize, (int) bytes);
   return (int) e;
 }
@@ -54,8 +58,8 @@
   hipLaunchKernelGGL(k, dim3(grid), dim3(kBlock), 0, s, sc, lens, pixels, n, first_sample, samples, origin, dir, weight);
 }
 static void trace(uint32_t grid, size_t lds, hipStream_t s, const DeviceScene& sc, const PathQueue& q, const uint32_t* order, uint32_t* ctrl, uint64_t* counters,
-                  uint32_t lds_nodes, bool single_level) {
-  hipLaunchKernelGGL(trace_kernel(single_level && single_level_scene(sc)), dim3(grid), dim3(kTraceBlock), lds, s, sc, q, order, ctrl, counters, lds_nodes);
+                  uint32_t lds_nodes, bool single_level, bool coherent) {
+  hipLaunchKernelGGL(trace_kernel(single_level && single_level_scene(sc), coherent), dim3(grid), dim3(kTraceBlock), lds, s, sc, q, order, ctrl, counters, lds_nodes);
 }
 static void sky_inscattering(uint32_t grid, hipStream_t s, const DeviceScene& sc, const PathQueue& in, float4* results, const uint32_t* ctrl, uint32_t depth_const) {
   hipLaunchKernelGGL(k_sky_inscattering, dim3(grid), dim3(kBlock), 0, s, sc, in, results, ctrl, depth_const);
@@ -142,8 +146,8 @@
   hipLaunchKernelGGL(k_clouds, dim3(grid), dim3(kBlock), 0, s, sc, in, cq, results, ctrl, depth_const);
 }
 static void trace_rays(uint32_t grid, size_t lds, hipStream_t s, const DeviceScene& sc, uint32_t n, const float* origins, const float* dirs, const uint32_t* ignore, uint32_t* out,
-                       uint32_t* cursor, uint64_t* counters, uint32_t lds_nodes, bool single_level) {
-  hipLaunchKernelGGL(trace_rays_kernel(single_level && single_level_scene(sc)), dim3(grid), dim3(kTraceBlock), lds, s, sc, n, origins, dirs, ignore, out, cursor, counters,
+                       uint32_t* cursor, uint64_t* counters, uint32_t lds_nodes, bool single_level, bool coherent) {
+  hipLaunchKernelGGL(trace_rays_kernel(single_level && single_level_scene(sc), coherent), dim3(grid), dim3(kTraceBlock), lds, s, sc, n, origins, dirs, ignore, out, cursor, counters,
                      lds_nodes);
 }
 static void guide(uint32_t grid, hipStream_t s, const DeviceScene& sc, const PathQueue& in, const uint32_t* ctrl, float* planes, uint32_t n) {
diff --git a/luminary_amd/csrc/host/context.h b/luminary_amd/csrc/host/context.h
--- a/luminary_amd/csrc/host/context.h
+++ b/luminary_amd/csrc/host/context.h
@@ -85,6 +85,8 @@
   int ambient_reuse = -1;
   int single_level = -1;
   int plain_form = -1;
+  int pixel_major = -1;
+  int coherent_first_hits = -1;
   bool first_leaf_identity = false;
   int overlap_lq = -1;
   hipStream_t side_stream = nullptr;
diff --git a/luminary_amd/csrc/host/core.hip b/luminary_amd/csrc/host/core.hip
--- a/luminary_amd/csrc/host/core.hip
+++ b/luminary_amd/csrc/host/core.hip
@@ -135,6 +135,8 @@
   if (const char* e = getenv("LUM_SINGLE_LEVEL")) ctx->single_level = atoi(e) != 0 ? 1 : 0;
   if (const char* e = getenv("LUM_PLAIN_FORM")) ctx->plain_form = atoi(e) != 0 ? 1 : 0;
   if (const char* e = getenv("LUM_OVERLAP_LQ")) ctx->overlap_lq = atoi(e) != 0 ? 1 : 0;
+  if (const char* e = getenv("LUM_PIXEL_MAJOR")) ctx->pixel_major = atoi(e) != 0 ? 1 : 0;
+  if (const char* e = getenv("LUM_COHERENT_FIRST_HITS")) ctx->coherent_first_hits = atoi(e) != 0 ? 1 : 0;
   if (const char* e = getenv("LUM_FUSED_RESOLVE")) ctx->fused_resolve = atoi(e) != 0 ? 1 : 0;
   if (const char* e = getenv("LUM_SHADE_GRID")) ctx->shade_grid_rounds = (uint32_t) atoi(e);
   if (const char* e = getenv("LUM_SOBOL_TABLE_RT")) ctx->sobol_table = atoi(e) != 0 ? 1 : 0;
@@ -233,7 +235,7 @@
   const WavefrontKernels& wf = *ctx->wf;
   {
     Launch l(ctx, stream, LUMC_KERNEL_TRACE);
-    wf.trace(grid_persistent(ctx, N), ray_kernel_lds(ctx), stream, sc, ctx->work.queue[0], nullptr, ctx->d_ctrl.get(), ctx->d_counters.get(), ctx->lds_nodes, single_level_allowed(ctx));
+    wf.trace(grid_persistent(ctx, N), ray_kernel_lds(ctx), stream, sc, ctx->work.queue[0], nullptr, ctx->d_ctrl.get(), ctx->d_counters.get(), ctx->lds_nodes, single_level_allowed(ctx), false);
   }
   if (sc.particles_active) trace_particles(ctx, stream, ctx->work.queue[0], ctx->d_ctrl.get(), N);
   if (sc.ocean_active) {
@@ -297,16 +299,24 @@
                       depth == max_depth};
 }
 
-static void trace_depth(LumContext* ctx, hipStream_t stream, const DeviceScene& sc, const DepthBuffers& d, const uint32_t* order, uint32_t N) {
+static void trace_depth(LumContext* ctx, hipStream_t stream, const DeviceScene& sc, const DepthBuffers& d, const uint32_t* order, uint32_t N, bool coherent = false) {
   Launch l(ctx, stream, LUMC_KERNEL_TRACE);
-  ctx->wf->trace(grid_persistent(ctx, N), ray_kernel_lds(ctx), stream, sc, d.cur, order, d.ctrl, ctx->d_counters.get(), ctx->lds_nodes, single_level_allowed(ctx));
-}
-
-static int closest_hits(LumContext* ctx, hipStream_t stream, const DeviceScene& sc, ResolveScheme scheme, const DepthBuffers& d, uint32_t N) {
+  ctx->wf->trace(grid_persistent(ctx, N), ray_kernel_lds(ctx), stream, sc, d.cur, order, d.ctrl, ctx->d_counters.get(), ctx->lds_nodes, single_level_allowed(ctx), coherent);
+}
+
+constexpr bool kPixelMajorAuto = true, kCoherentAuto = true;
+static bool pixel_major_wanted(const LumContext* ctx) { return ctx->pixel_major < 0 ? kPixelMajorAuto : ctx->pixel_major != 0; }
+static bool coherent_eligible(const LumContext* ctx) { return ctx->has_scene && single_level_allowed(ctx) && single_level_scene(ctx->scene); }
+static bool coherent_forced(const LumContext* ctx) { return ctx->coherent_first_hits == 1 && coherent_eligible(ctx); }
+static bool coherent_first_hits(const LumContext* ctx, bool pixel_major) {
+  return coherent_forced(ctx) || (ctx->coherent_first_hits < 0 && kCoherentAuto && pixel_major && ctx->camera == kCamThinLens && coherent_eligible(ctx));
+}
+
+static int closest_hits(LumContext* ctx, hipStream_t stream, const DeviceScene& sc, ResolveScheme scheme, const DepthBuffers& d, uint32_t N, bool coherent_depth0 = false) {
   const WavefrontKernels& wf = *ctx->wf;
   const uint32_t* order = nullptr;
   if (ctx->sort.mode >= 1 && d.depth >= 1 && sort_closest_rays(ctx, stream, d.cur, d.ctrl, N, &order)) return 1;
-  trace_depth(ctx, stream, sc, d, order, N);
+  trace_depth(ctx, stream, sc, d, order, N, coherent_depth0 && d.depth == 0u && order == nullptr);
   if (scheme == kResolveReuse && d.depth > 0) {
     uint32_t* prev = d.ctrl - kCtlStride;
     {
@@ -428,7 +438,7 @@
   }
 }
 
-static int wavefront_depths(LumContext* ctx, hipStream_t stream, uint32_t N, uint32_t first_sample = 0, uint32_t sample_count = 0) {
+static int wavefront_depths(LumContext* ctx, hipStream_t stream, uint32_t N, uint32_t first_sample = 0, uint32_t sample_count = 0, bool coherent = false) {
   DeviceScene sc = ctx->scene;
   const uint32_t max_depth = sc.max_ray_depth;
   prepare_sobol_table(ctx, stream, sc, first_sample, sample_count);
@@ -444,7 +454,7 @@
   bool traced = false;
   for (uint32_t depth = 0; depth <= max_depth; depth++) {
     const DepthBuffers d = depth_buffers(ctx, scheme, depth, max_depth);
-    if (!traced && closest_hits(ctx, stream, sc, scheme, d, N)) return 1;
+    if (!traced && closest_hits(ctx, stream, sc, scheme, d, N, coherent)) return 1;
     traced = false;
     media_passes(ctx, stream, sc, d, N);
     shade_depth(ctx, stream, sc, scheme, d, N);
@@ -487,16 +497,17 @@
   for (uint32_t done = 0; done < num_samples; done += samples_per_pass) {
     const uint32_t batch = std::min(samples_per_pass, num_samples - done);
     const uint32_t N = P * batch;
-    PassParams pp{ctx->d_pixels.get(), P, batch, first_sample + done};
+    const bool pixel_major = pixel_major_wanted(ctx);
+    PassParams pp{ctx->d_pixels.get(), P, batch, first_sample + done, pixel_major ? 1u : 0u};
     HIP_TRY(ctx, hipMemsetAsync(ctx->d_ctrl.get(), 0, sizeof(uint32_t) * kCtlStride * (max_depth + 2), stream));
     {
       Launch l(ctx, stream, LUMC_KERNEL_GENERATE);
       ctx->wf->generate(grid_for(N), stream, sc, pp, ctx->work.queue[0], ctx->work.results, ctx->d_ctrl.get() + kCtlPaths, ctx->lens, ctx->camera);
     }
-    if (wavefront_depths(ctx, stream, N, first_sample + done, batch)) return 1;
+    if (wavefront_depths(ctx, stream, N, first_sample + done, batch, coherent_first_hits(ctx, pixel_major && batch % 64u == 0u))) return 1;
     {
       Launch l(ctx, stream, LUMC_KERNEL_ACCUMULATE);
-      hipLaunchKernelGGL(k_accumulate, dim3(grid_for(P)), dim3(kBlock), 0, stream, (const float4*) ctx->work.results, P, batch, d_fm, d_sm);
+      hipLaunchKernelGGL(k_accumulate, dim3(grid_for(P)), dim3(kBlock), pixel_major ? kAccTileBytes : 0u, stream, (const float4*) ctx->work.results, P, batch, d_fm, d_sm, pixel_major ? 1u : 0u);
     }
     HIP_TRY(ctx, hipGetLastError());
   }
@@ -1125,7 +1136,7 @@
   HIP_TRY(ctx, hipMemsetAsync(cursor, 0, sizeof(uint32_t), stream));
   Launch l(ctx, stream, LUMC_KERNEL_TRACE);
   ctx->wf->trace_rays(grid_persistent(ctx, n), ray_kernel_lds(ctx), stream, ctx->scene, n, d_origins, d_dirs, d_ignore, d_out, cursor, ctx->d_counters.get(),
-                      ctx->lds_nodes, single_level_allowed(ctx));
+                      ctx->lds_nodes, single_level_allowed(ctx), coherent_forced(ctx));
   HIP_TRY(ctx, hipGetLastError());
   return 0;
 }
@@ -1372,6 +1383,18 @@
   return 0;
 }
 int lumc_get_overlap_light_query(const LumContext* ctx) { return (ctx && ctx->has_scene && overlap_allowed(ctx, wanted_scheme(ctx))) ? 1 : 0; }
+int lumc_set_pixel_major(LumContext* ctx, int mode) {
+  if (!ctx || mode < -1 || mode > 1) { if (ctx) ctx->error = "lumc_set_pixel_major: -1 (auto), 0 (sample-major slots) or 1 (pixel-major slots)"; return 1; }
+  ctx->pixel_major = mode;
+  return 0;
+}
+int lumc_get_pixel_major(const LumContext* ctx) { return (ctx && pixel_major_wanted(ctx)) ? 1 : 0; }
+int lumc_set_coherent_first_hits(LumContext* ctx, int mode) {
+  if (!ctx || mode < -1 || mode > 1) { if (ctx) ctx->error = "lumc_set_coherent_first_hits: -1 (auto), 0 (never) or 1 (when the scene is eligible)"; return 1; }
+  ctx->coherent_first_hits = mode;
+  return 0;
+}
+int lumc_get_coherent_first_hits(const LumContext* ctx) { return (ctx && coherent_first_hits(ctx, pixel_major_wanted(ctx))) ? 1 : 0; }
 int lumc_overlap_registers_fit(uint32_t ray_kernel_regs, uint32_t light_query_regs) { return overlap_registers_fit(ray_kernel_regs, light_query_regs) ? 1 : 0; }
 int lumc_get_flavour(const LumContext* ctx) { return (ctx && ctx->wf == wavefront_kernels_exact()) ? LUMC_FLAVOUR_EXACT : LUMC_FLAVOUR_FAST; }
 
```

After: 4292 (median of 6 runs). 1.1% higher.
